# JubSteven/POEM-v2

Hardware: AMD Instinct MI355X
Metric: samples/sec (multi-view frames) POEM-medium 8-view (higher is better)
Workload: dtype f32

## Files before the change

### include/poem_hip.h

```cpp
#ifndef POEM_HIP_H
#define POEM_HIP_H

#include <stddef.h>
#include <stdint.h>

#ifdef __cplusplus
extern "C" {
#endif

#define POEM_OK 0
#define POEM_E_ARG (-1)
#define POEM_E_WORKSPACE (-2)
#define POEM_E_LAUNCH (-3)
#define POEM_E_UNSUPPORTED (-4)


#define POEM_ACT_NONE 0
#define POEM_ACT_RELU 1
#define POEM_ACT_GELU 2

typedef struct poem_config {
  int32_t embed;
  int32_t in_channels;
  int32_t nsample;
  int32_t nquery;
  int32_t heads;
  int32_t nblocks;
  int32_t knn;
  int32_t parametric;
  int32_t feat_h, feat_w;
  int32_t max_views;
  float radius;
  float ln_eps;
  int32_t pe_normalize;
  int32_t petr_embedding;
  int32_t depth_num;
  int32_t lid;
  int32_t reserved0;
  double depth_start, depth_end;
  double position_range[6];
} poem_config_t;

typedef struct poem_handle_s* poem_handle_t;

int poem_abi_version(void);
int poem_last_hip_error(void);
const char* poem_error_string(int code);

int poem_num_weight_tensors(const poem_config_t* cfg);
int64_t poem_weight_tensor_numel(const poem_config_t* cfg, int index);
size_t poem_packed_bytes(const poem_config_t* cfg);
int poem_create(const poem_config_t* cfg, const void* const* raw_host, int n, const float* bps, const float* anchor,
                const int32_t* anchor_idx, const float* template_xyz, void* packed, size_t packed_bytes,
                void* stream, poem_handle_t* out);
void poem_destroy(poem_handle_t h);

size_t poem_workspace_bytes(poem_handle_t h, int batch, int total_views);
int poem_graph_stats(poem_handle_t h, int64_t* out, int n);
int poem_head_forward(poem_handle_t h, const float* mlvl_feat, const float* cam_intr, const float* cam_extr,
                      const int32_t* view_offsets_host, int batch, const float* reference_joints, int img_w,
                      int img_h, float* out_xyz, float* pose_aa, float* betas, void* workspace,
                      size_t workspace_bytes, void* stream);
int poem_decoder_forward(poem_handle_t h, const float* query_xyz, const float* query_feat, const float* pt_xyz,
                         const float* pt_feats, int batch, float* out_xyz_norm, float* pose_aa, float* betas,
                         void* workspace, size_t workspace_bytes, void* stream);
int poem_set_overlap(poem_handle_t h, int enable);
int poem_set_chains(poem_handle_t h, int enable);
int poem_set_option(poem_handle_t h, const char* name, int value);
int poem_set_anchor_tables(poem_handle_t h, int enable);
#define POEM_PRECISION_FP32 0
#define POEM_PRECISION_SPLIT_F16X3 1
#define POEM_PRECISION_SPLIT_F16X3_ALL 2
int poem_set_precision(poem_handle_t h, int mode);
int poem_cross_attention_merged(const float* q, const float* k, const float* v, float* ctx, int batch, int nq, int nk, int embed,
                                int heads, void* scratch, size_t scratch_bytes, void* stream);
int poem_cross_attention_split_f16x3(const float* q, const float* k, const float* v, float* ctx, int batch, int nq, int nk,
                                     int embed, int heads, void* scratch, size_t scratch_bytes, void* stream);
int poem_pack_split_gemm(const float* w, int out_features, int in_features, void* image, float* scales, void* stream);
int poem_gemm_split(const float* x, int ldx, const void* image, const float* scales, const float* bias, const float* residual,
                    int ldr, float* y, int ldy, int m, int n, int k, int act, void* stream);
int poem_finalize_parametric(poem_handle_t h, const float* mano_verts, const float* mano_joints,
                             const float* reference_joints, int batch, float* out_xyz, void* stream);
int poem_profile_enable(poem_handle_t h, int max_launches);
int poem_profile_read(poem_handle_t h, int* launches, float* total_ms, int reset);
int poem_profile_read_anchored(poem_handle_t h, int* launches, float* total_ms);
#define POEM_PROF_VECATTN 0
#define POEM_PROF_VECATTN_ANCHORED 1
#define POEM_PROF_SAMPLING 2
int poem_profile_read_stage(poem_handle_t h, int stage, int* launches, float* total_ms);
int64_t poem_tap(poem_handle_t h, const char* name, void* dst, int64_t dst_elems, void* stream);
int poem_enable_taps(poem_handle_t h, int enable);

size_t poem_packed_linear_bytes(int out_features, int in_features);
int poem_pack_linear(const float* w, int out_features, int in_features, void* packed, void* stream);
int poem_gemm(const float* x, int ldx, const void* w_packed, const float* bias, const float* residual, int ldr,
              float* y, int ldy, int M, int N, int K, int act, void* stream);
#define POEM_LAYOUT_RM 0
#define POEM_LAYOUT_PA 1
int poem_gemm_ex(const float* x, int ldx, const void* w_packed, const float* bias, const float* residual, int ldr,
                 float* y, int ldy, int M, int N, int K, int act, int in_layout, int out_layout, void* stream);
int poem_pack_rows(const float* x, int rows, int cols, void* packed, void* stream);
int poem_unpack_rows(const void* packed, int rows, int cols, float* x, void* stream);
int poem_layernorm(const float* x, const float* gamma, const float* beta, float* y, int rows, int cols, float eps,
                   void* stream);
int poem_pe_table(const void* adapt_w_packed, const float* adapt_b, int embed, int h, int w, int max_views,
                  float* scratch_sine, float* table, void* stream);
int poem_pe_table_ex(const void* adapt_w_packed, const float* adapt_b, int embed, int h, int w, int max_views, int normalize,
                     float* scratch_sine, float* table, void* stream);
int poem_frustum_features(const poem_config_t* cfg, const float* cam_intr, const float* cam_extr, int views, int img0, int img1,
                          float* out, void* stream);
int poem_input_proj(const float* feat, const void* w_packed, const float* bias, const float* table,
                    const int32_t* pe_index, float* x, int views, int in_channels, int embed, int hw, void* stream);
int poem_project_sample(const float* x, const float* bps, const float* centre, const int32_t* view_sample,
                        const float* cam_intr, const float* cam_extr, float* uv_scratch, float* g, int views,
                        int embed, int fh, int fw, int nsample, int img_w, int img_h, void* stream);
int poem_merge_reduce(const float* h2, const int32_t* view_offsets, float* m, int batch, int nsample, int half,
                      void* stream);
int poem_merge_finalize(const float* g, const float* y, const int32_t* view_offsets, float* out, int batch,
                        int nsample, int embed, void* stream);
size_t poem_cross_attention_scratch_bytes(int batch, int nq, int nk, int embed, int heads);
int poem_cross_attention(const float* q, const float* k, const float* v, float* ctx, int batch, int nq, int nk,
                         int embed, int heads, void* scratch, size_t scratch_bytes, void* stream);
int poem_triangulate_dlt(const float* uv, const float* cam_intr, const float* cam_mat, const int32_t* view_offsets,
                         int batch, int njoints, int invert, float* out_xyz, void* stream);
int poem_heatmap_uv(const float* heatmaps, float* uv, int views, int njoints, int hm_h, int hm_w, float img_w, float img_h,
                    void* stream);
int poem_heatmap_uv_conf(const float* heatmaps, float* uv, float* conf, int views, int njoints, int hm_h, int hm_w,
                         float img_w, float img_h, void* stream);
#define POEM_DLT_THRESHOLD 1
#define POEM_DLT_WEIGHTED 2
int poem_dlt_confidence(const float* uv, const float* conf, const float* cam_intr, const float* cam_mat,
                        const int32_t* view_offsets, float* out_xyz, int32_t* sel_count, int batch, int njoints, int invert,
                        int mode, double threshold, void* stream);
size_t poem_conv3x3_packed_bytes(int cout, int cin);
int poem_pack_conv3x3(const float* w_oihw, int cout, int cin, void* packed, void* stream);
int poem_conv3x3(const float* in_padded, const void* w_packed, const float* scale, const float* shift,
                 const float* residual, float* out, int views, int cin, int cout, int h, int w, int stride, int relu,
                 int64_t out_view_stride, int out_ch_stride, int out_row_stride, int out_offset, void* stream);
typedef struct poem_fuse_term {
  const float* data;
  int64_t view_stride;
  int32_t ch_stride, row_stride, offset, shift;
} poem_fuse_term_t;
int poem_conv3x3_ex(const float* in_padded, const void* w_packed, const float* scale, const float* shift, const float* residual,
                    int64_t res_view_stride, int res_ch_stride, int res_row_stride, int res_offset, int res_before_act, float* out,
                    int views, int cin, int cout, int h, int w, int stride, int relu, int64_t out_view_stride, int out_ch_stride,
                    int out_row_stride, int out_offset, void* stream);
size_t poem_conv1x1_packed_bytes(int cout, int cin);
int poem_pack_conv1x1(const float* w_oi, int cout, int cin, void* packed, void* stream);
int poem_conv1x1(const float* in, int64_t in_view_stride, int in_ch_stride, int in_row_stride, int in_offset, const void* w_packed,
                 const float* shift, const float* residual, int64_t res_view_stride, int res_ch_stride, int res_row_stride,
                 int res_offset, float* out, int64_t out_view_stride, int out_ch_stride, int out_row_stride, int out_offset,
                 int views, int cin, int cout, int h, int w, int relu, void* stream);
int poem_hrnet_fuse(const poem_fuse_term_t* terms, int nterms, float* out, int64_t out_view_stride, int out_ch_stride,
                    int out_row_stride, int out_offset, int views, int channels, int h, int w, void* stream);
int poem_upsample2_concat_pad(const float* a, int ca, const float* b, int cb, float* out, int views, int h, int w, int pad,
                              void* stream);
size_t poem_conv7x7_packed_bytes(int cout);
int poem_pack_conv7x7(const float* w_oihw, int cout, void* packed, void* stream);
int poem_conv7x7_s2(const float* in, const void* w_packed, const float* scale, const float* shift, float* out,
                    int64_t out_view_stride, int out_ch_stride, int out_row_stride, int out_offset, int views, int cout, int h, int w,
                    void* stream);
int poem_maxpool3x3_s2(const float* in, int64_t in_view_stride, int in_ch_stride, int in_row_stride, int in_offset, float* out,
                       int64_t out_view_stride, int out_ch_stride, int out_row_stride, int out_offset, int views, int channels, int h,
                       int w, void* stream);
int poem_conv1x1_s2(const float* in, int64_t in_view_stride, int in_ch_stride, int in_row_stride, int in_offset, const void* w_packed,
                    const float* shift, float* out, int64_t out_view_stride, int out_ch_stride, int out_row_stride, int out_offset,
                    int views, int cin, int cout, int h, int w, void* stream);
int poem_maxpool2_conv1x1(const float* x, const void* w_packed, const float* bias, float* out, int views, int cin, int cout, int h,
                          int w, int act, void* stream);
int poem_upsample2_concat_pad_staged(const float* a, int ca, const float* b, int cb, float* out, int views, int h, int w, void* stream);
int poem_conv3x3_down2(const float* in, const void* w_packed, const float* scale, const float* shift, const float* residual,
                       float* out, int views, int cin, int cout, int h, int w, int relu, int64_t out_view_stride,
                       int out_ch_stride, int out_row_stride, int out_offset, void* stream);
int poem_set_decode_option(const char* name, int value);
int poem_conv1x1_upsample2(const float* in, const void* w_packed, const float* bias, float* out, int views, int cin, int cout,
                           int h, int w, void* stream);
int poem_upcat_conv3x3(const float* a_half, int ca, const float* b_full, int cb, const void* w_packed, const float* scale,
                       const float* shift, float* out, int views, int cout, int h, int w, int relu, int64_t out_view_stride,
                       int out_ch_stride, int out_row_stride, int out_offset, void* stream);
int poem_pool_conv1x1_sigmoid(const float* x, const float* w, const float* bias, float* heatmaps, int views, int c, int j,
                              int h, int w_, void* stream);
int poem_upcat_conv3x3_pool_head(const float* a_half, int ca, const float* b_full, int cb, const void* w_packed, const float* scale,
// ... 69 lines not shown
```

### poem-v2_amd/csrc/decoder.cpp

```cpp
#include "engine.h"

int build_anchor_tables(poem_handle_t h, Plan& p, hipStream_t s, bool at_create) {
  const poem_config_t& c = h->cfg;
  const int C = c.embed, Q = c.nquery;
  const bool ov = !at_create && h->overlap && h->bps_stream && h->knn_stream;
  hipStream_t sk = ov ? h->knn_stream : s;
  if (ov) {
    HIPCHK(hipEventRecord(h->ev_fork0, s));
    HIPCHK(hipStreamWaitEvent(sk, h->ev_fork0, 0));
  }
  const int bb0 = h->block_base(0);
  HIPCHK(poem_launch_canon_xyz(h->tmpl, p.canon_xyz, Q * 3, c.radius, sk));
  for (int k = 0; k < 2; ++k) {
    const int vb = bb0 + (k == 0 ? B_VS : B_VC);
    HIPCHK(poem_launch_vector_attention_tables(p.canon_xyz, h->anchor, h->anchor_idx, h->R(vb + 4), h->R(vb + 5),
                                               h->P(vb + 6), h->R(vb + 7), h->fused[0].w[5 + k], p.tab_g[k], p.tab_p[k],
                                               Q, C, sk));
  }
  if (ov) HIPCHK(hipEventRecord(h->ev_tab, sk));
  h->tables_pending = ov;
  return POEM_OK;
}

namespace {

struct DecoderRun {
  poem_handle_t h;
  Plan& p;
  const poem_config_t& c;
  const float *pt_xyz, *pt_feats;
  float *pose_aa, *betas;
  const int B, C, S, Q, BS, BQ;
  const int SP, BSP;
  const float* pt_xyz_rows;
  const bool ov;
  hipStream_t s, sb, sk;
  const bool tables;
  const bool chain;
  const float* feats;
  const float* hidden;
  int ldh = 0, hidden_mod = 0, q_batch = 0;
  const float* q0 = nullptr;
  const int *idx_s = nullptr, *idx_c = nullptr;
  const float* anchor = nullptr;
  int shared = 0;
  bool knn_issued[9] = {};
  bool wmerge = false;
  int wmask = 0;
  bool side_rest_pending = false;
  bool bps_waited[9] = {}, knn_waited[9] = {};
  bool anchor_from_y3 = false;

  DecoderRun(poem_handle_t h_, Plan& p_, const float* feats_in, const float* pt_xyz_, const float* pt_feats_, int B_, float* pose,
             float* bet, hipStream_t s_, bool template_queries)
      : h(h_), p(p_), c(h_->cfg), pt_xyz(pt_xyz_), pt_feats(pt_feats_), pose_aa(pose), betas(bet), B(B_), C(c.embed), S(c.nsample),
        Q(c.nquery), BS(B_ * c.nsample), BQ(B_ * c.nquery), SP(padded_samples(c)), BSP(B_ * padded_samples(c)), pt_xyz_rows(pt_xyz_), ov(h_->overlap && h_->bps_stream && h_->knn_stream), s(s_),
        sb(ov ? h_->bps_stream : s_), sk(ov ? h_->knn_stream : s_),
        tables(template_queries && h_->anchor_tables && h_->precision == POEM_PRECISION_FP32),
        chain(h_->chains && h_->precision == POEM_PRECISION_FP32 && poem_chain_supported(c.embed) != 0), feats(feats_in),
        hidden(nullptr) {}

  int gemm(const float* X, int ldx, int wi, int bi, const float* res, int ldr, float* Y, int ldy, int M, int N, int K, int act) {
    HIPCHK(poem_launch_gemm(X, ldx, h->P(wi), bi >= 0 ? h->R(bi) : nullptr, res, ldr, Y, ldy, M, N, K, act, s));
    return POEM_OK;
  }
  bool prof_begin() {
    const bool on = h->prof_on && (size_t)(2 * h->prof_used + 1) < h->prof_ev.size();
    if (on && hipEventRecord(h->prof_ev[2 * h->prof_used], s) != hipSuccess) return false;
    return on;
  }
  int prof_end(bool on, int kind) {
    if (on) { HIPCHK(hipEventRecord(h->prof_ev[2 * h->prof_used + 1], s)); h->prof_kind[h->prof_used++] = (char)kind; }
    return POEM_OK;
  }
  ChainArgs chain_args(int kind) const {
    ChainArgs a{};
    a.kind = kind; a.M = BQ; a.tile_p = h->chain_tile; a.eps = c.ln_eps;
    a.native_delta = h->native16 ? (long long)(h->native16 - h->packed_base) : 0;
    return a;
  }

  int fork() {
    if (!ov) return POEM_OK;
    HIPCHK(hipEventRecord(h->ev_fork, s));
    HIPCHK(hipStreamWaitEvent(sb, h->ev_fork, 0));
    HIPCHK(hipStreamWaitEvent(sk, h->ev_fork, 0));
    return POEM_OK;
  }
  int join() {
    if (!ov) return POEM_OK;
    HIPCHK(hipEventRecord(h->ev_join_bps, sb));
    HIPCHK(hipEventRecord(h->ev_join_knn, sk));
    HIPCHK(hipStreamWaitEvent(s, h->ev_join_bps, 0));
    HIPCHK(hipStreamWaitEvent(s, h->ev_join_knn, 0));
    return POEM_OK;
  }

  int basis_point_side(int i) {
    const auto& f = h->fused[i];
    const size_t seg = (size_t)BSP * C;
    float* outs[6] = {p.y1[i], p.y1[i] + seg, p.y1[i] + 2 * seg, p.y1[i] + 3 * seg, p.y1[i] + 4 * seg, p.y1[i] + 5 * seg};
    const int modes[6] = {1, 2, 1, 2, 0, 0};
    h->kv_presplit[i] = poem_gemm_split_applies(f.w[0], BSP, C, C) != 0;
    const bool anchored = tables && i == 0;
    if (!anchored && h->f1_split && C % 128 == 0) {
      HIPCHK(poem_launch_gemm_segs(pt_feats, C, f.w[0], f.b[0], BSP, C, POEM_ACT_NONE, C, 4, outs, modes, sb));
      HIPCHK(poem_launch_gemm_segs(pt_feats, C, (const float*)f.w[0] + (size_t)4 * C * C, f.b[0] + 4 * C, BSP, C, POEM_ACT_NONE, C, 2, outs + 4,
                                   modes + 4, sb));
    } else {
      HIPCHK(poem_launch_gemm_segs(pt_feats, C, f.w[0], f.b[0], BSP, C, POEM_ACT_NONE, C, anchored ? 4 : 6, outs, modes, sb));
    }
    if (ov) HIPCHK(hipEventRecord(h->ev_bps[i], sb));
    if (anchored && !side_rest_pending) return basis_point_anchor_rows(f);
    return POEM_OK;
  }
  int basis_point_anchor_rows(const poem_handle_s::Fused& f) {
    {
      HIPCHK(poem_launch_gather_anchor_rows(pt_feats, C, h->anchor_idx, SP, p.anch_x[1], B, C, p.ident, sb));
      HIPCHK(poem_launch_gemm(p.anch_x[1], C, (const float*)f.w[0] + (size_t)4 * C * C, f.b[0] + 4 * C, nullptr, 0,
                              p.anch_kv[1], 2 * C, B * 32, 2 * C, C, POEM_ACT_NONE, sb));
      if (ov) HIPCHK(hipEventRecord(h->ev_xyz[0], sb));
    }
    return POEM_OK;
  }

  bool merge_in_attention() const { return h->xattn_merge >= 0 ? h->xattn_merge != 0 : B <= 2; }

  int defer_at() const {
    return (ov && chain) ? h->bps_defer : 0;
  }
  int deferred_basis_point_side(int i, int at) {
    if (defer_at() != at || i + 1 >= c.nblocks) return POEM_OK;
    HIPCHK(hipEventRecord(h->ev_def[i], s));
    HIPCHK(hipStreamWaitEvent(sb, h->ev_def[i], 0));
    return basis_point_side(i + 1);
  }

  int neighbour_searches(int i, bool recorded = false) {
    if (knn_issued[i]) return POEM_OK;
    if (ov) {
      if (!recorded) HIPCHK(hipEventRecord(h->ev_xyz[i], s));
      HIPCHK(hipStreamWaitEvent(sk, h->ev_xyz[i], 0));
    }
    if (p.idx_ld == 32) {
      HIPCHK(poem_launch_knn(p.xyz[i], pt_xyz, p.idx_cross[i], B, Q, S, h->knn_fma, sk));
      HIPCHK(poem_launch_knn(p.xyz[i], p.xyz[i], p.idx_self[i], B, Q, Q, h->knn_fma, sk));
    } else {
      HIPCHK(poem_launch_knn_k(p.xyz[i], pt_xyz, p.idx_cross[i], B, Q, S, c.knn, p.idx_ld, h->knn_fma, sk));
      HIPCHK(poem_launch_knn_k(p.xyz[i], p.xyz[i], p.idx_self[i], B, Q, Q, h->knn_query ? h->knn_query : c.knn, p.idx_ld, h->knn_fma, sk));
    }
    if (ov) HIPCHK(hipEventRecord(h->ev_knn[i], sk));
    knn_issued[i] = true;
    return POEM_OK;
  }

  int query_projection(int i) {
    hidden = p.qeqp;
    ldh = 2 * C; hidden_mod = 0; q_batch = Q;
    q0 = p.qeqp + C;
    if (tables && i == 0) {
      const float* qe0 = p.qeqp0;
      if (h->tables_cached && h->c_qeqp0 && h->precision == POEM_PRECISION_FP32)
        qe0 = h->c_qeqp0;
      else
        HIPCHK(poem_launch_gemm_split(h->R(T_QEMB), C, h->fused[i].w[1], h->fused[i].b[1], nullptr, 0, p.qeqp0, 2 * C, Q, 2 * C, C,
                                      POEM_ACT_NONE, 2 * C, POEM_ACT_NONE, s));
      if (chain) {
        hidden = qe0; hidden_mod = Q; q0 = qe0 + C; q_batch = 0;
      } else {
        HIPCHK(poem_launch_broadcast(qe0, p.qeqp, (long)Q * 2 * C, B, s));
      }
    } else if (!(chain && i > 0)) {
      HIPCHK(poem_launch_gemm_split(feats, C, h->fused[i].w[1], h->fused[i].b[1], nullptr, 0, p.qeqp, 2 * C, BQ, 2 * C, C,
                                    POEM_ACT_NONE, 2 * C, POEM_ACT_NONE, s));
    }
    return POEM_OK;
  }

  int anchor_rows_f3(int i) {
    HIPCHK(poem_launch_gather_anchor_rows(hidden, C, h->anchor_idx, Q, p.anch_x[0], B, C, nullptr, s));
    HIPCHK(poem_launch_gemm(p.anch_x[0], C, (const float*)h->fused[i].w[2] + (size_t)C * C, h->fused[i].b[2] + C, nullptr, 0,
                            p.anch_kv[0], 2 * C, B * 32, 2 * C, C, POEM_ACT_NONE, s));
    return POEM_OK;
  }

  int cross_attentions(int i) {
    const int bb = h->block_base(i);
    if (chain) {
      const int a1 = bb + B_A1, a2 = bb + B_A2;
      if (ov && !bps_waited[i]) HIPCHK(hipStreamWaitEvent(s, h->ev_bps[i], 0));
      if (ov && (wmask & 4) && h->knn_early && i > 0 && knn_issued[i] && !knn_waited[i]) {
        HIPCHK(hipStreamWaitEvent(s, h->ev_knn[i], 0));
        knn_waited[i] = true;
      }
      const void *part_o = nullptr, *part_ml = nullptr;
      int pchunks = 0;
      float pkc2 = 0.f;
      poem_cross_attention_partials(B, Q, S, C, c.heads, p.attn_scratch, &part_o, &part_ml, &pchunks, &pkc2);
      const bool merged = merge_in_attention() && poem_cross_attention_merges(S, C, c.heads) != 0;
      const bool comb = !merged && h->chain_combine && poem_chain_combines(C, c.heads, pchunks) != 0;
      auto attention = [&](const float* q, int ldq, int qb, const float* kimg, const float* vimg) -> hipError_t {
        if (merged) return poem_launch_cross_attention_merged(q, ldq, qb, kimg, vimg, p.ctx, B, Q, S, C, c.heads, s);
        return poem_launch_cross_attention_imgq(q, ldq, qb, kimg, vimg, comb ? nullptr : p.ctx, B, Q, S, C, c.heads, p.attn_scratch, s);
      };
      auto from_partials = [&](ChainArgs& a) {
        if (!comb) return;
        a.x = nullptr; a.part_o = (const float4*)part_o; a.part_ml = (const float2*)part_ml;
        a.pc_heads = c.heads; a.pc_chunks = pchunks; a.pc_nq = Q; a.pc_kc2 = pkc2;
      };
      HIPCHK(attention(q0, 2 * C, q_batch, p.y1[i], p.y1[i] + (size_t)BSP * C));
      if (side_rest_pending) {
        side_rest_pending = false;
        if (tables && i == 0)
          if (const int rc = basis_point_anchor_rows(h->fused[0]); rc != POEM_OK) return rc;
        for (int k = 1; k < c.nblocks; ++k)
          if (const int rc = basis_point_side(k); rc != POEM_OK) return rc;
      }
      if (const int rc = deferred_basis_point_side(i, 1); rc != POEM_OK) return rc;
      ChainArgs ca = chain_args(0);
      ca.x = p.ctx; ca.ldx = C;
      from_partials(ca);
      ca.w1 = (const float4*)h->P(a1 + 6); ca.b1 = h->R(a1 + 7); ca.res = hidden; ca.ldres = ldh; ca.res_mod = hidden_mod;
      ca.ln_g = h->R(a1 + 8); ca.ln_b = h->R(a1 + 9); ca.y1 = p.h_attn; ca.ldy1 = C;
      ca.w2 = (const float4*)h->P(a2 + 0); ca.b2 = h->R(a2 + 1); ca.n2 = 1; ca.y2 = p.qp; ca.ldy2 = C;
      HIPCHK(poem_launch_chain(&ca, C, s));
      HIPCHK(attention(p.qp, C, Q, p.y1[i] + (size_t)2 * BSP * C, p.y1[i] + (size_t)3 * BSP * C));
      if (const int rc = deferred_basis_point_side(i, 2); rc != POEM_OK) return rc;
      ChainArgs cb = chain_args(0);
      cb.x = p.ctx; cb.ldx = C;
      from_partials(cb);
      cb.w1 = (const float4*)h->P(a2 + 6); cb.b1 = h->R(a2 + 7); cb.res = p.h_attn; cb.ldres = C; cb.res_mod = 0;
      cb.ln_g = h->R(a2 + 8); cb.ln_b = h->R(a2 + 9); cb.y1 = p.h_cross[i]; cb.ldy1 = C;
      anchor_from_y3 = tables && i == 0 && (h->small_batch & 2) && (long)BQ <= 16L * poem_device_cu_count();
      cb.w2 = (const float4*)h->fused[i].w[2]; cb.b2 = h->fused[i].b[2]; cb.n2 = (tables && i == 0 && !anchor_from_y3) ? 1 : 3; cb.y2 = p.y3; cb.ldy2 = 3 * C;
      HIPCHK(poem_launch_chain(&cb, C, s));
// ... 16 lines not shown
      }
      if (ov && a == 0) HIPCHK(hipStreamWaitEvent(s, h->ev_bps[i], 0));
      if (h->precision == POEM_PRECISION_SPLIT_F16X3_ALL) poem_cross_attention_split(h->kv_presplit[i] ? 2 : 1);
      if (h->precision == POEM_PRECISION_FP32 && merge_in_attention() && poem_cross_attention_merges(S, C, c.heads))
        HIPCHK(poem_launch_cross_attention_merged(qptr, ldq, Q, p.y1[i] + (size_t)(2 * a) * BSP * C, p.y1[i] + (size_t)(2 * a + 1) * BSP * C,
                                                  p.ctx, B, Q, S, C, c.heads, s));
      else
        HIPCHK(poem_launch_cross_attention_img(qptr, ldq, p.y1[i] + (size_t)(2 * a) * BSP * C, p.y1[i] + (size_t)(2 * a + 1) * BSP * C,
                                               p.ctx, B, Q, S, C, c.heads, p.attn_scratch, s));
      const int rc = gemm(p.ctx, C, ab + 6, ab + 7, hidden, ldh, p.att, C, BQ, C, C, POEM_ACT_NONE);
      if (rc != POEM_OK) return rc;
      HIPCHK(poem_launch_layernorm(p.att, h->R(ab + 8), h->R(ab + 9), hout, BQ, C, c.ln_eps, s));
      hidden = hout;
      ldh = C;
    }
    if (tables && i == 0) {
      HIPCHK(poem_launch_gemm(hidden, C, h->fused[i].w[2], h->fused[i].b[2], nullptr, 0, p.y3, 3 * C, BQ, C, C, POEM_ACT_NONE, s));
      return anchor_rows_f3(i);
    }
    HIPCHK(poem_launch_gemm_split(hidden, C, h->fused[i].w[2], h->fused[i].b[2], nullptr, 0, p.y3, 3 * C, BQ, 3 * C, C, POEM_ACT_NONE,
                                  3 * C, POEM_ACT_NONE, s));
    return POEM_OK;
  }

  int vector_self(int i) {
    const int vsb = h->block_base(i) + B_VS;
    const float* xyz = p.xyz[i];
    if (ov && i > 0 && !knn_waited[i]) HIPCHK(hipStreamWaitEvent(s, h->ev_knn[i], 0));
    const bool prof = prof_begin();
    const int kq = shared ? 32 : (h->knn_query ? h->knn_query : c.knn);
    if (h->precision != POEM_PRECISION_FP32) {
      if (kq != 32) return POEM_E_UNSUPPORTED;
      const auto& sw = h->split[2 * i];
      HIPCHK(poem_launch_vector_attention_split(xyz, xyz, anchor, idx_s, shared, p.y3, p.y3 + C, p.y3 + 2 * C, Q, h->R(vsb + 4),
                                                h->R(vsb + 5), sw.w[0], h->R(vsb + 7), sw.w[1], sw.w[2], sw.scales, p.rs, B, Q, C,
                                                3 * C, 3 * C, 3 * C, s));
    } else if (tables && i == 0) {
      if (ov && h->tables_pending) HIPCHK(hipStreamWaitEvent(s, h->ev_tab, 0));
      if (anchor_from_y3)
        HIPCHK(poem_launch_vector_attention_anchored(h->anchor_idx, p.y3, p.y3 + C, p.y3 + 2 * C, Q, h->P(vsb + 10), p.tab_g[0], p.tab_p[0],
                                                     p.rs, B, Q, C, 3 * C, 3 * C, 3 * C, s));
      else {
      if (ov) HIPCHK(hipStreamWaitEvent(s, h->ev_xyz[0], 0));
      HIPCHK(poem_launch_vector_attention_anchored(p.ident, p.y3, p.anch_kv[0], p.anch_kv[0] + C, 32, h->P(vsb + 10), p.tab_g[0],
                                                   p.tab_p[0], p.rs, B, Q, C, 3 * C, 2 * C, 2 * C, s));
      }
    } else if (!shared && p.idx_ld != 32) {
      HIPCHK(poem_launch_vector_attention_k(xyz, xyz, idx_s, kq, p.idx_ld, p.y3, p.y3 + C, p.y3 + 2 * C, Q, h->R(vsb + 4), h->R(vsb + 5),
                                            h->P(vsb + 6), h->R(vsb + 7), h->fused[i].w[5], h->R(vsb + 9), h->P(vsb + 10), h->R(vsb + 11),
                                            p.rs, B, Q, C, 3 * C, 3 * C, 3 * C, 1, s));
    } else {
      poem_vecattn_one_query_blocks(h->va_p1);
      poem_vecattn_valid_neighbours(kq);
      const hipError_t ve = poem_launch_vector_attention(xyz, xyz, anchor, idx_s, shared, p.y3, p.y3 + C, p.y3 + 2 * C, Q, h->R(vsb + 4),
                                                         h->R(vsb + 5), h->P(vsb + 6), h->R(vsb + 7), h->fused[i].w[5], h->R(vsb + 9),
                                                         h->P(vsb + 10), h->R(vsb + 11), p.rs, B, Q, C, 3 * C, 3 * C, 3 * C, 1, s);
      poem_vecattn_valid_neighbours(32);
      poem_vecattn_one_query_blocks(0);
      HIPCHK(ve);
    }
    if (const int rc = prof_end(prof, tables && i == 0 ? 1 : 0); rc != POEM_OK) return rc;
    if (chain) {
      ChainArgs cc = chain_args(1);
      cc.x = p.rs; cc.ldx = C;
      cc.w1 = (const float4*)h->P(vsb + 2); cc.b1 = h->R(vsb + 3); cc.res = hidden; cc.ldres = C; cc.res_mod = 0;
      cc.y1 = p.f_self[i]; cc.ldy1 = C;
      cc.w2 = (const float4*)h->fused[i].w[4]; cc.b2 = h->fused[i].b[4]; cc.n2 = 1; cc.y2 = p.qc; cc.ldy2 = C;
      HIPCHK(poem_launch_chain(&cc, C, s));
      return POEM_OK;
    }
    if (const int rc = gemm(p.rs, C, vsb + 2, vsb + 3, hidden, C, p.f_self[i], C, BQ, C, C, POEM_ACT_NONE); rc != POEM_OK) return rc;
    HIPCHK(poem_launch_gemm(p.f_self[i], C, h->fused[i].w[4], h->fused[i].b[4], nullptr, 0, p.qc, C, BQ, C, C, POEM_ACT_NONE, s));
    return POEM_OK;
  }

  int vector_cross(int i) {
    const int vcb = h->block_base(i) + B_VC;
    const float* xyz = p.xyz[i];
    if (ov && (wmask & 2) && i == 0 && defer_at() == 0)
      for (int k = 1; k < c.nblocks; ++k) {
        HIPCHK(hipStreamWaitEvent(s, h->ev_bps[k], 0));
        bps_waited[k] = true;
      }
    const bool prof = prof_begin();
    const int kc = shared ? 32 : c.knn;
    if (h->precision != POEM_PRECISION_FP32) {
      if (kc != 32) return POEM_E_UNSUPPORTED;
      const auto& sw = h->split[2 * i + 1];
      HIPCHK(poem_launch_vector_attention_split(xyz, pt_xyz_rows, anchor, idx_c, shared, p.qc, p.y1[i] + 4 * (size_t)BSP * C,
                                                p.y1[i] + 5 * (size_t)BSP * C, SP, h->R(vcb + 4), h->R(vcb + 5), sw.w[0],
                                                h->R(vcb + 7), sw.w[1], sw.w[2], sw.scales, p.rc, B, Q, C, C, C, C, s));
    } else if (tables && i == 0) {
      if (ov) HIPCHK(hipStreamWaitEvent(s, h->ev_xyz[0], 0));
      HIPCHK(poem_launch_vector_attention_anchored(p.ident, p.qc, p.anch_kv[1], p.anch_kv[1] + C, 32, h->P(vcb + 10), p.tab_g[1],
                                                   p.tab_p[1], p.rc, B, Q, C, C, 2 * C, 2 * C, s));
    } else if (!shared && p.idx_ld != 32) {
      HIPCHK(poem_launch_vector_attention_k(xyz, pt_xyz_rows, idx_c, kc, p.idx_ld, p.qc, p.y1[i] + 4 * (size_t)BSP * C, p.y1[i] + 5 * (size_t)BSP * C,
                                            SP, h->R(vcb + 4), h->R(vcb + 5), h->P(vcb + 6), h->R(vcb + 7), h->fused[i].w[6], h->R(vcb + 9),
                                            h->P(vcb + 10), h->R(vcb + 11), p.rc, B, Q, C, C, C, C, 1, s));
    } else {
      poem_vecattn_one_query_blocks(h->va_p1);
      poem_vecattn_valid_neighbours(kc);
      const hipError_t ve = poem_launch_vector_attention(xyz, pt_xyz_rows, anchor, idx_c, shared, p.qc, p.y1[i] + 4 * (size_t)BSP * C,
                                                         p.y1[i] + 5 * (size_t)BSP * C, SP, h->R(vcb + 4), h->R(vcb + 5), h->P(vcb + 6),
                                                         h->R(vcb + 7), h->fused[i].w[6], h->R(vcb + 9), h->P(vcb + 10), h->R(vcb + 11), p.rc, B,
                                                         Q, C, C, C, C, 1, s);
      poem_vecattn_valid_neighbours(32);
      poem_vecattn_one_query_blocks(0);
      HIPCHK(ve);
    }
    return prof_end(prof, tables && i == 0 ? 1 : 0);
  }

  int parametric_tail(int i) {
    const int bb = h->block_base(i);
    HIPCHK(poem_launch_q3_flatten(feats, h->R(bb + B_FLAT_W), h->R(bb + B_FLAT_B), p.q3t, B, Q, C, s));
    HIPCHK(poem_launch_narrow_linear(p.q3t, C, h->R(bb + B_MANO_W), h->R(bb + B_MANO_B), nullptr, p.par, B, C, 106, s));
    HIPCHK(poem_launch_rot6d_to_aa(p.par, pose_aa, betas, B, s));
    if (h->mano_table) HIPCHK(poem_launch_mano_lbs(pose_aa, betas, h->mano_table, p.mano_verts, p.mano_joints, B, h->mano_center, s));
    return POEM_OK;
  }

  int tail(int i, bool* done) {
    const int bb = h->block_base(i), vcb = bb + B_VC;
    const float* xyz = p.xyz[i];
    const bool last = i == c.nblocks - 1;
    const bool feats_dead = last && !c.parametric && !h->taps;
    *done = feats_dead;
    if (chain) {
      ChainArgs cd = chain_args(2);
      cd.x = p.rc; cd.ldx = C;
      cd.w1 = (const float4*)h->P(vcb + 2); cd.b1 = h->R(vcb + 3); cd.res = p.f_self[i]; cd.ldres = C; cd.res_mod = 0;
      cd.y1 = p.f_cross[i]; cd.ldy1 = C;
      cd.wf4 = (const float4*)h->fused[i].w[3]; cd.bf4 = h->fused[i].b[3];
      cd.wreg2 = h->R(bb + B_REG2_W); cd.breg2 = h->R(bb + B_REG2_B); cd.xyz_in = xyz; cd.xyz_out = p.xyz[i + 1];
      HIPCHK(poem_launch_chain(&cd, C, s));
      if (feats_dead) return POEM_OK;
      const bool early = ov && h->knn_early && !last;
      const bool d2_first = early && h->d2_first != 0;
      if (early && d2_first) HIPCHK(hipEventRecord(h->ev_xyz[i + 1], s));
      if (early && !d2_first)
        if (const int rc = neighbour_searches(i + 1); rc != POEM_OK) return rc;
      ChainArgs ce = chain_args(3);
      ce.x = p.f_cross[i]; ce.ldx = C;
      ce.wf4 = (const float4*)h->fused[i].w[3]; ce.bf4 = h->fused[i].b[3];
      ce.wout = (const float4*)h->P(bb + B_OUT_W); ce.bout = h->R(bb + B_OUT_B);
      ce.ln2_g = h->R(bb + B_LN_W); ce.ln2_b = h->R(bb + B_LN_B); ce.y3 = p.feats[i]; ce.ldy3 = C;
      if (!last) {
        ce.w2 = (const float4*)h->fused[i + 1].w[1]; ce.b2 = h->fused[i + 1].b[1]; ce.n2 = 2; ce.y2 = p.qeqp; ce.ldy2 = 2 * C;
      }
      HIPCHK(poem_launch_chain(&ce, C, s));
      if (early && d2_first)
        if (const int rc = neighbour_searches(i + 1, true); rc != POEM_OK) return rc;
      feats = p.feats[i];
      return c.parametric && last ? parametric_tail(i) : POEM_OK;
    }
    if (const int rc = gemm(p.rc, C, vcb + 2, vcb + 3, p.f_self[i], C, p.f_cross[i], C, BQ, C, C, POEM_ACT_NONE); rc != POEM_OK) return rc;
    if (feats_dead) {
      HIPCHK(poem_launch_gemm(p.f_cross[i], C, h->fused[i].w[3], h->fused[i].b[3], nullptr, 0, p.y4, 5 * C, BQ, C, C, POEM_ACT_RELU, s));
      HIPCHK(poem_launch_narrow_linear(p.y4, 5 * C, h->R(bb + B_REG2_W), h->R(bb + B_REG2_B), xyz, p.xyz[i + 1], BQ, C, 3, s));
      return POEM_OK;
    }
    HIPCHK(poem_launch_gemm_split(p.f_cross[i], C, h->fused[i].w[3], h->fused[i].b[3], nullptr, 0, p.y4, 5 * C, BQ, 5 * C, C,
                                  POEM_ACT_RELU, C, POEM_ACT_GELU, s));
    HIPCHK(poem_launch_narrow_linear(p.y4, 5 * C, h->R(bb + B_REG2_W), h->R(bb + B_REG2_B), xyz, p.xyz[i + 1], BQ, C, 3, s));
    if (const int rc = gemm(p.y4 + C, 5 * C, bb + B_OUT_W, bb + B_OUT_B, p.f_cross[i], C, p.ffo, C, BQ, C, 4 * C, POEM_ACT_NONE); rc != POEM_OK)
// ... 49 lines not shown
```

### poem-v2_amd/csrc/engine.h

```cpp
#pragma once
#include "../../include/poem_hip.h"
#include "launchers.h"

#include <hip/hip_runtime.h>

#include <algorithm>
#include <cstdio>
#include <cstdlib>
#include <cstring>
#include <map>
#include <string>
#include <vector>

extern thread_local int g_last_hip_error;

#define HIPCHK(expr)                                 \
  do {                                               \
    (void)hipGetLastError();                         \
    hipError_t e_ = (expr);                          \
    if (e_ != hipSuccess) {                          \
      g_last_hip_error = (int)e_;                    \
      return POEM_E_LAUNCH;                          \
    }                                                \
  } while (0)
// ... 15 lines not shown
enum {
  T_INPROJ_W = 0, T_INPROJ_B, T_ADAPT_W, T_ADAPT_B, T_M00_W, T_M00_B, T_M02_W, T_M02_B, T_M10_W, T_M10_B, T_M12_W,
  T_M12_B, T_QEMB, T_HEAD_COUNT
};
enum {
  B_EMB_W = 0, B_EMB_B,
  B_A1 = 2,
  B_A2 = 12,
  B_VS = 22,
  B_VC = 37,
  B_REG0_W = 52, B_REG0_B, B_REG2_W, B_REG2_B, B_INT_W, B_INT_B, B_OUT_W, B_OUT_B, B_LN_W, B_LN_B,
  B_COUNT = 62,
  B_FLAT_W = 62, B_FLAT_B, B_MANO_W, B_MANO_B, B_COUNT_PARAM = 66
};

static inline int petr_slot(const poem_config_t& c) { return T_HEAD_COUNT + c.nblocks * (c.parametric ? B_COUNT_PARAM : B_COUNT); }
static inline size_t pe_views(int max_views) { return (size_t)max_views * (max_views + 1) / 2; }
std::vector<TensorSpec> tensor_table(const poem_config_t& c);
int check_config(const poem_config_t* c);

struct poem_handle_s {
  poem_config_t cfg;
  std::vector<TensorSpec> specs;
  std::vector<const float*> raw;
  std::vector<const void*> packed;
  const float* bps = nullptr;
  const float* anchor = nullptr;
  const int32_t* anchor_idx = nullptr;
  const float* tmpl = nullptr;
  float* pe_table = nullptr;
  struct Fused { const void* w[7]; const float* b[7]; };
  std::vector<Fused> fused;
  struct SplitW { const void* w[3]; const float* scales; };
  std::vector<SplitW> split;
  void* split_mem = nullptr;
  int precision = 0;
  bool kv_presplit[8] = {};
  const char* packed_base = nullptr;
  size_t packed_size = 0;
  char* native16 = nullptr;
  char* gemm_split = nullptr;
  float* gemm_scales = nullptr;
  bool taps = false;
  struct Tap { const void* p; int64_t elems; };
  std::map<std::string, Tap> tapmap;
  std::vector<hipEvent_t> prof_ev;
  int prof_used = 0;
  std::vector<char> prof_kind;
  bool prof_on = false;
  hipStream_t bps_stream = nullptr, knn_stream = nullptr;
  hipEvent_t ev_fork = nullptr, ev_join_bps = nullptr, ev_join_knn = nullptr, ev_tab = nullptr, ev_fork0 = nullptr;
  bool anchor_tables = true;
  bool chains = true;
  bool fused_sampling = true;
  bool tables_first = true;
  bool chain_combine = true;
  int xattn_merge = -1;
  bool knn_early = true;
  bool graphs = true;
  bool graph_broken = false;
  hipStream_t cap_stream = nullptr;
  int stream_device = 0;
  struct GraphEntry { std::vector<int64_t> key; hipGraphExec_t exec; uint64_t stamp; uint64_t shape; hipStream_t last_stream = nullptr; bool launched = false; };
  std::vector<GraphEntry> graph_cache;
  std::vector<std::vector<int64_t>> graph_seen;
  bool graph_eager = false;
  uint64_t graph_clock = 0;
  static constexpr size_t GRAPH_CAP = 12;
  int64_t graph_captures = 0, graph_instantiations = 0, graph_replays = 0, plain_forwards = 0, layout_uploads = 0;
  int small_batch = 3;
  int group_xcd = 1;
  int group_min_views = 0;
  const float* mano_table = nullptr;
  int mano_center = 9;
  int knn_query = 0;
  int knn_fma = 0;
  int chain_tile = 0;
  bool tables_cached = true;
  bool tables_pending = false;
  float* tab_mem = nullptr;
  float *c_canon_xyz = nullptr, *c_tab_g[2] = {}, *c_tab_p[2] = {};
  float* c_qeqp0 = nullptr;
  hipEvent_t ev_bps[8] = {}, ev_xyz[8] = {}, ev_knn[8] = {}, ev_def[8] = {};
  int bps_defer = 0;
  bool f1_split = true;
  int va_p1 = -1;
  int d2_first = 1;
  int wait_merge = -1;
  bool overlap = true;
  static constexpr int IDX_CAP = 32768;
  int32_t* idx_dev = nullptr;
  std::vector<int32_t> idx_host;
  int block_base(int b) const { return T_HEAD_COUNT + b * (cfg.parametric ? B_COUNT_PARAM : B_COUNT); }
  const float* R(int idx) const { return raw[idx]; }
  const void* P(int idx) const { return packed[idx]; }
};

struct Arena {
  char* base;
  size_t off = 0;
  explicit Arena(void* b) : base((char*)b) {}
  template <typename T>
  T* take(size_t n) {
    off = align_up(off, 256);
    T* p = base ? (T*)(base + off) : nullptr;
    off += n * sizeof(T);
    return p;
  }
};

struct Plan {
  int32_t *offs, *view_sample, *pe_index, *idx_self[8], *idx_cross[8];
  float *x, *uv, *g, *h1, *h2, *mm, *mh, *y, *bps_feat, *centre, *pt_xyz, *xyz[9];
  float *xt, *ptab, *q1;
  float *petr_f, *petr_h, *petr_tab;
  float *feats0, *qp, *ctx, *att, *h_attn, *y3, *rs, *qc, *rc, *y4, *ffo;
  float *y1[8];
  float *qeqp;
  float *h_cross[8], *f_self[8], *f_cross[8], *feats[8];
  float *q3t, *par, *attn_scratch, *g_pose, *g_betas;
  float *mano_verts, *mano_joints;
  float *canon_xyz, *tab_g[2], *tab_p[2];
  float *anch_x[2], *anch_kv[2], *qeqp0;
  int32_t* ident;
  float *feat_pad, *xyz_pad;
  int idx_ld;
  size_t bytes;
};

inline int padded_samples(const poem_config_t& c) { return (c.nsample + 31) / 32 * 32; }

inline int neighbour_ld(const poem_config_t& c, int knn_query) { return (c.knn > 32 || knn_query > 32) ? 64 : 32; }

Plan make_plan(const poem_config_t& c, int B, int BN, void* base, int idx_ld);
void register_taps(poem_handle_t h, const Plan& p, int B, int BN, bool sampling);

int poem_process_switches();
void poem_park_graph_exec(hipGraphExec_t e, uint64_t shape, int device, hipStream_t last_stream, bool launched);
hipGraphExec_t poem_reuse_graph_exec(hipGraph_t graph, uint64_t shape, int device);

int build_anchor_tables(poem_handle_t h, Plan& p, hipStream_t s, bool at_create = false);
int run_decoder(poem_handle_t h, Plan& p, const float* feats_in, const float* pt_xyz, const float* pt_feats, int B, float* pose_aa,
                float* betas, hipStream_t s, bool template_queries = false);
```

### poem-v2_amd/csrc/forward.cpp

```cpp
#include "engine.h"

namespace {

struct SplitContext {
  bool set = false;
  explicit SplitContext(poem_handle_t h) {
    if (h->precision != POEM_PRECISION_SPLIT_F16X3_ALL) return;
    set = true;
    poem_gemm_split_context(h->packed_base, h->packed_size, h->gemm_split, h->gemm_scales);
    poem_cross_attention_split(1);
    const int dh = h->cfg.embed / h->cfg.heads;
    poem_gemm_split_images(dh == 32 || dh == 64);
  }
  ~SplitContext() {
    if (!set) return;
    poem_gemm_split_context(nullptr, 0, nullptr, nullptr);
    poem_cross_attention_split(0);
    poem_gemm_split_images(0);
  }
};

struct HeadRun {
  poem_handle_t h;
  const poem_config_t& c;
// ... 76 lines not shown
      const int ps = petr_slot(c), K0 = 3 * c.depth_num;
      HIPCHK(poem_launch_frustum_features(cam_intr, cam_extr, p.petr_f, BN, c.feat_h, c.feat_w, c.depth_num, c.lid != 0, c.depth_start,
                                          c.depth_end, c.position_range, img_w, img_h, s));
      HIPCHK(poem_launch_conv1x1_ex(p.petr_f, h->P(ps), h->R(ps + 1), nullptr, nullptr, p.petr_h, nullptr, BN, K0, 2 * C, HW, 1, s));
      HIPCHK(poem_launch_conv1x1_ex(p.petr_h, h->P(ps + 2), h->R(ps + 3), h->pe_table, p.pe_index, p.petr_tab, nullptr, BN, 2 * C, C, HW, 0, s));
      table = p.petr_tab;
      table_index = nullptr;
    }
    HIPCHK(poem_launch_conv1x1(mlvl_feat, h->P(T_INPROJ_W), h->R(T_INPROJ_B), table, table_index,
                               (fused_fe && !h->taps) ? nullptr : p.x, fused_fe ? p.xt : nullptr, BN, c.in_channels, C, HW, s));
    if (fused_fe && (h->small_batch & 1)) {
      HIPCHK(poem_launch_input_tables(h->bps, reference_joints, h->tmpl, p.view_sample, cam_intr, cam_extr, p.ptab, p.ptab + (size_t)plan_views * S * 4, p.centre, p.pt_xyz,
                                      p.xyz[0], BN, B, S, Q, c.feat_h, c.feat_w, img_w, img_h, c.radius, s));
      return POEM_OK;
    }
    HIPCHK(poem_launch_prep_xyz(reference_joints, h->bps, h->tmpl, p.centre, p.pt_xyz, p.xyz[0], B, S, Q, c.radius, s));
    if (fused_fe) {
      float* inv = p.uv + (size_t)BN * S * 2;
      HIPCHK(poem_launch_invert_extr(cam_extr, inv, BN, s));
      HIPCHK(poem_launch_project_table(h->bps, p.centre, p.view_sample, cam_intr, inv, p.ptab, p.ptab + (size_t)plan_views * S * 4, nullptr, BN, C, c.feat_h, c.feat_w, S,
                                       img_w, img_h, s));
    } else {
      HIPCHK(poem_launch_project_uv(h->bps, p.centre, p.view_sample, cam_intr, cam_extr, p.uv + (size_t)BN * S * 2, p.uv, BN, c.feat_h,
                                    c.feat_w, S, img_w, img_h, s));
    }
    return POEM_OK;
  }

  int sampling(hipStream_t st) {
    if (fused_fe) {
      SampleMergeArgs sm{};
      sm.xt = p.xt; sm.tab = (const float4*)p.ptab; sm.tabo = (const uint2*)(p.ptab + (size_t)plan_views * S * 4);
      sm.view_sample = p.view_sample; sm.offs = p.offs;
      sm.w0 = (const float4*)h->P(T_M00_W); sm.b0 = h->R(T_M00_B); sm.w1 = (const float4*)h->P(T_M02_W); sm.b1 = h->R(T_M02_B);
      sm.h2 = p.h2; sm.q1 = p.q1; sm.S = S; sm.hw = HW; sm.h2_tiled = 1;
      sm.views = plan_views; sm.B = B; sm.views_dev = p.offs + B;
      const bool group_ok = h->group_min_views >= 0 && (S / C) % 8 == 0;
      sm.group_min_views = group_ok ? (h->group_min_views > 0 ? h->group_min_views : 2 * poem_device_cu_count() / ((C / (C == 512 ? 32 : 64)) * (S / C / 8)))
                                    : 0x7fffffff;
      if (h->tables_first && h->tables_pending) HIPCHK(hipStreamWaitEvent(st, h->ev_tab, 0));
      MergeTailArgs mt{};
      mt.h2 = p.h2; mt.q1 = p.q1; mt.offs = p.offs;
      mt.w0 = (const float4*)h->P(T_M10_W); mt.b0 = h->R(T_M10_B); mt.w1 = (const float4*)h->P(T_M12_W); mt.b1 = h->R(T_M12_B);
      mt.out = p.bps_feat; mt.B = B; mt.S = S; mt.h2_tiled = 1;
      mt.group_min_views = sm.group_min_views; mt.views_dev = sm.views_dev; mt.views = sm.views;
      sm.xcd_order = h->group_xcd;
      if (group_ok && plan_views >= sm.group_min_views) {
        SampleGroupArgs sg{};
        sg.sm = sm; sg.w2 = mt.w0; sg.b2 = mt.b0; sg.w3 = mt.w1; sg.b3 = mt.b1; sg.out = p.bps_feat;
        HIPCHK(poem_launch_sample_group(&sg, C, st));
      }
      HIPCHK(poem_launch_sample_merge(&sm, C, st));
      HIPCHK(poem_launch_merge_tail(&mt, C, st));
      return POEM_OK;
    }
    auto gemm = [&](const float* X, int ldx, int wi, int bi, float* Y, int ldy, int M, int N, int K, int act) -> int {
      HIPCHK(poem_launch_gemm(X, ldx, h->P(wi), h->R(bi), nullptr, 0, Y, ldy, M, N, K, act, st));
      return POEM_OK;
    };
    HIPCHK(poem_launch_grid_sample(p.x, p.uv, p.g, BN, C, c.feat_h, c.feat_w, S, st));
    int rc = gemm(p.g, C, T_M00_W, T_M00_B, p.h1, C, BN * S, C, C, POEM_ACT_RELU);
    if (rc == POEM_OK) rc = gemm(p.h1, C, T_M02_W, T_M02_B, p.h2, C / 2, BN * S, C / 2, C, POEM_ACT_NONE);
    if (rc != POEM_OK) return rc;
    HIPCHK(poem_launch_merge_reduce(p.h2, p.offs, p.mm, B, S, C / 2, st));
    rc = gemm(p.mm, C / 2, T_M10_W, T_M10_B, p.mh, C / 2, BS, C / 2, C / 2, POEM_ACT_RELU);
    if (rc == POEM_OK) rc = gemm(p.mh, C / 2, T_M12_W, T_M12_B, p.y, C, BS, C, C / 2, POEM_ACT_NONE);
    if (rc != POEM_OK) return rc;
    HIPCHK(poem_launch_merge_finalize(p.g, p.y, p.offs, p.bps_feat, B, S, C, st));
    return POEM_OK;
  }

  int body(hipStream_t st, float* pose_dst, float* betas_dst) {
    if (const int rc = sampling(st); rc != POEM_OK) return rc;
    if (prof_fe) HIPCHK(hipEventRecord(h->prof_ev[2 * prof_slot + 1], st));
    if (!(h->anchor_tables && h->precision == POEM_PRECISION_FP32 && (h->small_batch & 1)))
      HIPCHK(poem_launch_broadcast(h->R(T_QEMB), p.feats0, (long)Q * C, B, st));
    return run_decoder(h, p, p.feats0, p.pt_xyz, p.bps_feat, B, pose_dst, betas_dst, st, true);
  }

  int replay(void* workspace, float* pose_aa, float* betas) {
    if (!h->graphs || h->graph_broken || h->prof_on || h->tables_pending || !h->cap_stream) return 0;
    const std::vector<int64_t> key = {B, plan_views, fused_fe ? -1 : BN, (int64_t)(uintptr_t)workspace, h->precision, h->anchor_tables, h->chains,
                                      h->fused_sampling, h->tables_first, h->chain_combine, h->knn_early, h->overlap, h->chain_tile,
                                      h->tables_cached, h->knn_fma, h->knn_query, h->taps, c.parametric, h->xattn_merge, h->small_batch, h->bps_defer, poem_process_switches(), h->f1_split, h->va_p1, h->group_min_views, h->group_xcd, h->d2_first, h->wait_merge,
                                      (int64_t)(uintptr_t)h->mano_table, h->mano_center};
    poem_handle_s::GraphEntry* hit = nullptr;
    for (auto& g : h->graph_cache)
      if (g.key == key) { hit = &g; break; }
    if (!hit) {
      if (!h->graph_eager) {
        bool seen = false;
        for (auto& k : h->graph_seen) seen = seen || k == key;
        if (!seen) {
          if (h->graph_seen.size() >= 64) h->graph_seen.erase(h->graph_seen.begin());
          h->graph_seen.push_back(key);
          return 0;
        }
      }
      hipGraph_t graph = nullptr;
      hipGraphExec_t exec = nullptr;
      POEM_TRACE("capture begin h=%p B=%d cached=%zu", (void*)h, B, h->graph_cache.size());
      bool ok = hipStreamBeginCapture(h->cap_stream, hipStreamCaptureModeRelaxed) == hipSuccess;
      if (ok) {
        const int rc = body(h->cap_stream, p.g_pose, p.g_betas);
        POEM_TRACE("capture body rc=%d", rc);
        const hipError_t e = hipStreamEndCapture(h->cap_stream, &graph);
        POEM_TRACE("capture end e=%d graph=%p", (int)e, (void*)graph);
        ok = rc == POEM_OK && e == hipSuccess && graph != nullptr;
      }
      ++h->graph_captures;
      if (ok) {
        exec = poem_reuse_graph_exec(graph, graph_shape_of(c, key), h->stream_device);
        if (!exec) {
          ok = hipGraphInstantiate(&exec, graph, nullptr, nullptr, 0) == hipSuccess;
          ++h->graph_instantiations;
        }
      }
      POEM_TRACE("instantiate ok=%d exec=%p", (int)ok, (void*)exec);
      if (graph) (void)hipGraphDestroy(graph);
      POEM_TRACE("graph destroyed");
      if (!ok) {
        (void)hipGetLastError();
        h->graph_broken = true;
        return 0;
      }
      if (h->graph_cache.size() >= poem_handle_s::GRAPH_CAP) {
        size_t lru = 0;
        for (size_t i = 1; i < h->graph_cache.size(); ++i)
          if (h->graph_cache[i].stamp < h->graph_cache[lru].stamp) lru = i;
        poem_park_graph_exec(h->graph_cache[lru].exec, h->graph_cache[lru].shape, h->stream_device, h->graph_cache[lru].last_stream,
                             h->graph_cache[lru].launched);
        h->graph_cache.erase(h->graph_cache.begin() + lru);
      }
      h->graph_cache.push_back({key, exec, 0, graph_shape_of(c, key), nullptr, false});
      hit = &h->graph_cache.back();
    }
    hit->stamp = ++h->graph_clock;
    POEM_TRACE("graph launch exec=%p", (void*)hit->exec);
    HIPCHK(hipGraphLaunch(hit->exec, s));
    hit->last_stream = s; hit->launched = true;
    ++h->graph_replays;
    POEM_TRACE("graph launched");
    if (c.parametric) {
      HIPCHK(hipMemcpyAsync(pose_aa, p.g_pose, (size_t)B * 48 * sizeof(float), hipMemcpyDeviceToDevice, s));
      HIPCHK(hipMemcpyAsync(betas, p.g_betas, (size_t)B * 10 * sizeof(float), hipMemcpyDeviceToDevice, s));
    }
    return 1;
  }

  static uint64_t graph_shape_of(const poem_config_t& c, const std::vector<int64_t>& key) {
    uint64_t v = 1469598103934665603ull;
    auto mix = [&](uint64_t x) { v = (v ^ x) * 1099511628211ull; };
    mix((uint64_t)c.embed); mix((uint64_t)c.nblocks); mix((uint64_t)c.heads); mix((uint64_t)c.nsample); mix((uint64_t)c.nquery);
    mix((uint64_t)c.in_channels); mix((uint64_t)c.feat_h * 65536u + (uint64_t)c.feat_w); mix((uint64_t)c.max_views);
    for (size_t i = 0; i < key.size(); ++i)
      if (i != 3) mix((uint64_t)key[i]);
    return v ? v : 1;
  }
};

}

extern "C" {

int poem_head_forward(poem_handle_t h, const float* mlvl_feat, const float* cam_intr, const float* cam_extr,
                      const int32_t* view_offsets_host, int batch, const float* reference_joints, int img_w, int img_h,
                      float* out_xyz, float* pose_aa, float* betas, void* workspace, size_t workspace_bytes,
// ... 71 lines not shown
```

### poem-v2_amd/csrc/gemm.hip

```cpp
#include "common.h"
#include <algorithm>
#include <cstdlib>

typedef _Float16 h8 __attribute__((ext_vector_type(8)));
#ifndef POEM_GS_WAVES
#define POEM_GS_WAVES 12
#endif
#define POEM_GEMM_SX 16.0f
__global__ __launch_bounds__(256) void pack_split_tiles_kernel(const float* __restrict__ W, int N, int K,
                                                              h8* __restrict__ img, float* __restrict__ scales,
                                                              int scale_stride) {
  __shared__ float red[256];
  const int nt = blockIdx.x, KC = K / 16;
  float m = 0.f;
  for (int i = threadIdx.x; i < 32 * K; i += 256) {
    const int row = 32 * nt + i / K;
    if (row < N) m = fmaxf(m, fabsf(W[(size_t)row * K + i % K]));
  }
  red[threadIdx.x] = m;
  __syncthreads();
  for (int o = 128; o > 0; o >>= 1) {
    if ((int)threadIdx.x < o) red[threadIdx.x] = fmaxf(red[threadIdx.x], red[threadIdx.x + o]);
    __syncthreads();
  }
// ... 362 lines not shown
    const int col = col0 + n * 32 + r, ycol = ycol0 + n * 32 + r;
    const float bv = bias ? bias[col] : 0.f;
#pragma unroll
    for (int i = 0; i < MT; ++i) {
      const int row0 = (mt0 + i) * 32 + 4 * h;
      if (row0 >= M) continue;
      float v[16];
#pragma unroll
      for (int e = 0; e < 16; ++e) {
        v[e] = acc[i][n][e] + bv;
        if (pact == 1) v[e] = relu_nan(v[e]);
        if (pact == 2) v[e] = gelu_erf(v[e]);
      }
      if (row0 + 28 < M) {
        float* yl = Y + (size_t)row0 * ldy + ycol;
        if (R) {
          const float* rl = R + (size_t)row0 * ldr + col;
          float rr[16];
#pragma unroll
          for (int e = 0; e < 16; ++e) rr[e] = rl[(size_t)((e & 3) + 8 * (e >> 2)) * ldr];
#pragma unroll
          for (int e = 0; e < 16; ++e) yl[(size_t)((e & 3) + 8 * (e >> 2)) * ldy] = v[e] + rr[e];
        } else {
#pragma unroll
          for (int e = 0; e < 16; ++e) yl[(size_t)((e & 3) + 8 * (e >> 2)) * ldy] = v[e];
        }
      } else {
#pragma unroll
        for (int e = 0; e < 16; ++e) {
          const int row = row0 + (e & 3) + 8 * (e >> 2);
          if (row < M) Y[(size_t)row * ldy + ycol] = v[e] + (R ? R[(size_t)row * ldr + col] : 0.f);
        }
      }
    }
  }
}

template <int MT, int NT, int SKC>
__global__ __launch_bounds__(512, 2) void gemm_kslab_kernel(const float* __restrict__ X, int ldx, const float4* __restrict__ Wp,
                                                            const float* __restrict__ bias, const float* __restrict__ R, int ldr,
                                                            float* __restrict__ Y, int ldy, int M, int N, int K, int act,
                                                            int act_split, int act2, PanelSegs segs) {
  const int ncb = N / (32 * NT);
  const int nb = (int)gridDim.x;
  const int lb = (nb & 7) == 0 ? (int)(blockIdx.x & 7) * (nb >> 3) + (int)(blockIdx.x >> 3) : (int)blockIdx.x;
  const int cb = lb % ncb, rb = lb / ncb;
  const int col0 = cb * NT * 32;
  const int pact = (col0 >= act_split) ? act2 : act;
  if (segs.seg_cols == 0) {
    kslab_body<MT, NT, SKC, 0>(X, ldx, Wp, bias, R, ldr, Y, ldy, M, K, pact, cb, rb, col0);
    return;
  }
  const int sidx = col0 / segs.seg_cols, ycol0 = col0 - sidx * segs.seg_cols, mode = segs.mode[sidx];
  float* ys = segs.ptr[sidx];
  if (mode == 1) kslab_body<MT, NT, SKC, 1>(X, ldx, Wp, bias, nullptr, 0, ys, segs.seg_cols, M, K, pact, cb, rb, ycol0);
  else if (mode == 2) kslab_body<MT, NT, SKC, 2>(X, ldx, Wp, bias, nullptr, 0, ys, segs.seg_cols, M, K, pact, cb, rb, ycol0);
  else kslab_body<MT, NT, SKC, 0>(X, ldx, Wp, bias, nullptr, 0, ys, segs.seg_cols, M, K, pact, cb, rb, ycol0);
}

static bool kslab_applies(const float* X, int ldx, int M, int N, int K, int act_split) {
  return K >= 512 && K % 128 == 0 && N % 64 == 0 && (act_split >= N || act_split % 64 == 0) && !((uintptr_t)X & 15) && ldx % 4 == 0 &&
         (unsigned long long)M * ldx * 4ull < (1ull << 32) && M >= 512;
}

static hipError_t launch_gemm_kslab(const float* X, int ldx, const void* Wp, const float* bias, const float* R, int ldr, float* Y,
                                    int ldy, int M, int N, int K, int act, int act_split, int act2, const PanelSegs& segs, hipStream_t s) {
  constexpr int NT = 2, SKC = 16;
  const int mtiles = (M + 31) / 32, ncb = N / (32 * NT);
  const bool mt2 = (long)((mtiles + 15) / 16) * ncb >= 2 * poem_device_cus();
  const size_t lds = (size_t)2 * NT * SKC * 1024;
  if (mt2) {
    auto kern = gemm_kslab_kernel<2, NT, SKC>;
    hipLaunchKernelGGL(kern, dim3((unsigned)(((mtiles + 15) / 16) * ncb)), dim3(512), lds, s, X, ldx, (const float4*)Wp, bias, R, ldr, Y, ldy,
                       M, N, K, act, act_split, act2, segs);
  } else {
    auto kern = gemm_kslab_kernel<1, NT, SKC>;
    hipLaunchKernelGGL(kern, dim3((unsigned)(((mtiles + 7) / 8) * ncb)), dim3(512), lds, s, X, ldx, (const float4*)Wp, bias, R, ldr, Y, ldy,
                       M, N, K, act, act_split, act2, segs);
  }
  return hipGetLastError();
}


template <int NT, int MT, bool GELU, int OMODE, bool SPLIT = false>
__device__ __forceinline__ void panel_rows(const float* __restrict__ X, int ldx, const float4* __restrict__ wl,
                                           const float* __restrict__ bias, const float* __restrict__ R, int ldr,
                                           float* __restrict__ Y, int ldy, int M, int K, int pact, int col0, int ycol0,
                                           int bip, int blocks_in_panel, const float* __restrict__ tile_scales = nullptr,
                                           int scale_stride = 0, int split_images = 0, int part = 0, int nparts = 1) {
  constexpr int NWV = (SPLIT && !GELU) ? POEM_GS_WAVES : 8;
  const int KC = K >> 3;
  const int tid = threadIdx.x, lane = tid & 63, wv = tid >> 6, r = lane & 31, h = lane >> 5;
  const int mtiles = (M + 31) / 32;
  const int rgroups = (mtiles + MT - 1) / MT;
  const __amdgpu_buffer_rsrc_t xrs = frag_rsrc(X, 0xffffffffu);
  float bv[NT];
#pragma unroll
  for (int n = 0; n < NT; ++n) bv[n] = (bias && OMODE != 1) ? bias[col0 + n * 32 + r] : 0.f;
  const size_t lane_yo = (size_t)(4 * h) * ldy + r, lane_ro = (size_t)(4 * h) * ldr + r;
  const int rg_lo = (int)((long)rgroups * part / nparts), rg_hi = (int)((long)rgroups * (part + 1) / nparts);
#ifndef POEM_PANEL_LAB
#define POEM_PANEL_LAB 0
#endif
#ifdef POEM_PANEL_SKEW
  if (wv >= NWV / 2) { const long long t0_ = wall_clock64(); while (wall_clock64() - t0_ < POEM_PANEL_SKEW) __builtin_amdgcn_s_sleep(32); }
#endif
  for (int rg = rg_lo + bip * NWV + wv; rg < rg_hi; rg += blocks_in_panel * NWV) {
#if POEM_PANEL_LAB & 4
    __builtin_amdgcn_s_setprio(0);
#endif
    const int mt0 = rg * MT;
    unsigned xo[MT];
#pragma unroll
    for (int i = 0; i < MT; ++i) xo[i] = (unsigned)min((mt0 + i) * 32 + r, M - 1) * (unsigned)(ldx * 4) + 16u * h;
    f32x16 acc[MT][NT];
#pragma unroll
    for (int i = 0; i < MT; ++i)
#pragma unroll
      for (int n = 0; n < NT; ++n) acc[i][n] = zero16();
    if constexpr (SPLIT) {
      const int KC16 = K >> 4;
      const h8* wl8 = reinterpret_cast<const h8*>(wl);
      unsigned xo8[MT];
#pragma unroll
      for (int i = 0; i < MT; ++i) xo8[i] = (unsigned)min((mt0 + i) * 32 + r, M - 1) * (unsigned)(ldx * 4) + 32u * h;
      float4 ra[2][MT][2];
#define POEM_LOADA8(S, KCI) { const int kq_ = min((KCI), KC16 - 1); _Pragma("unroll") for (int i = 0; i < MT; ++i) { \
        ra[S][i][0] = frag_load(xrs, (int)xo8[i], kq_ * 64); ra[S][i][1] = frag_load(xrs, (int)xo8[i], kq_ * 64 + 16); } }
      POEM_LOADA8(0, 0)
      h8 bh_next = wl8[lane], bl_next = wl8[64 + lane];
      for (int kc = 0; kc < KC16; ++kc) {
        const int cur = kc & 1;
        if (cur == 0) { POEM_LOADA8(1, kc + 1) } else { POEM_LOADA8(0, kc + 1) }
        h8 ah[MT], al[MT];
#pragma unroll
        for (int i = 0; i < MT; ++i) {
          const float4 lo4 = cur == 0 ? ra[0][i][0] : ra[1][i][0], hi4 = cur == 0 ? ra[0][i][1] : ra[1][i][1];
          const float xv[8] = {lo4.x, lo4.y, lo4.z, lo4.w, hi4.x, hi4.y, hi4.z, hi4.w};
#pragma unroll
          for (int t = 0; t < 8; ++t) {
#if defined(POEM_GS_LAB) && POEM_GS_LAB == 1
            ah[i][t] = __builtin_bit_cast(_Float16, (unsigned short)__float_as_uint(xv[t]));
            al[i][t] = ah[i][t];
#else
            const float v = __builtin_amdgcn_fmed3f(xv[t] * POEM_GEMM_SX, -60000.f, 60000.f);
            ah[i][t] = (_Float16)v;
            al[i][t] = (_Float16)(v - (float)ah[i][t]);
#endif
          }
        }
        __builtin_amdgcn_sched_barrier(0);
#pragma unroll
        for (int n = 0; n < NT; ++n) {
          const int nn = n + 1 < NT ? n + 1 : 0, kn = n + 1 < NT ? kc : min(kc + 1, KC16 - 1);
          const h8 bh = bh_next, bl = bl_next;
          bh_next = wl8[((size_t)(nn * KC16 + kn) * 2 + 0) * 64 + lane];
          bl_next = wl8[((size_t)(nn * KC16 + kn) * 2 + 1) * 64 + lane];
          __builtin_amdgcn_sched_barrier(0);
#define POEM_MMA8(XA, WB)                                                                                      \
          _Pragma("unroll") for (int i = 0; i < MT; ++i)                                                       \
            acc[i][n] = OMODE == 1 ? __builtin_amdgcn_mfma_f32_32x32x16_f16(WB, XA[i], acc[i][n], 0, 0, 0)     \
                                   : __builtin_amdgcn_mfma_f32_32x32x16_f16(XA[i], WB, acc[i][n], 0, 0, 0);
#if defined(POEM_GS_LAB) && POEM_GS_LAB == 2
#pragma unroll
          for (int i = 0; i < MT; ++i) acc[i][n][0] += (float)al[i][0] * (float)bh[0] + (float)ah[i][1] * (float)bl[1];
#else
          POEM_MMA8(al, bh) POEM_MMA8(ah, bh) POEM_MMA8(ah, bl)
#endif
#undef POEM_MMA8
          __builtin_amdgcn_sched_barrier(0);
        }
      }
#undef POEM_LOADA8
#pragma unroll
      for (int n = 0; n < NT; ++n) {
        const float inv = 1.0f / (tile_scales[(size_t)(col0 / 32 + n) * scale_stride] * POEM_GEMM_SX);
#pragma unroll
        for (int i = 0; i < MT; ++i)
#pragma unroll
          for (int e = 0; e < 16; ++e) acc[i][n][e] *= inv;
      }
    } else {
    float4 a0[MT], a1[MT], b0[NT], b1[NT];
#define POEM_LOADA(A, KCI) { const int kq_ = min((KCI), KC - 1); _Pragma("unroll") for (int i = 0; i < MT; ++i) A[i] = frag_load(xrs, (int)xo[i], kq_ * 32); }
#define POEM_LOADB(B, KCI) { const int kq_ = min((KCI), KC - 1); _Pragma("unroll") for (int n = 0; n < NT; ++n) B[n] = wl[(n * KC + kq_) * 64 + lane]; }
#define POEM_MMA(A, B)                                                          \
  _Pragma("unroll") for (int t = 0; t < 4; ++t) {                               \
    _Pragma("unroll") for (int n = 0; n < NT; ++n) {                            \
      const float bw = (&B[n].x)[t];                                            \
      _Pragma("unroll") for (int i = 0; i < MT; ++i)                            \
        acc[i][n] = OMODE == 1 ? mfma32(bw, (&A[i].x)[t], acc[i][n]) : mfma32((&A[i].x)[t], bw, acc[i][n]); \
    }                                                                           \
  }
    POEM_LOADA(a0, 0) POEM_LOADB(b0, 0)
    int kc = 0;
    for (; kc + 1 < KC; kc += 2) {
      POEM_LOADA(a1, kc + 1) POEM_LOADB(b1, kc + 1)
      __builtin_amdgcn_sched_barrier(0);
      POEM_MMA(a0, b0)
      __builtin_amdgcn_sched_barrier(0);
      POEM_LOADA(a0, kc + 2) POEM_LOADB(b0, kc + 2)
      __builtin_amdgcn_sched_barrier(0);
      POEM_MMA(a1, b1)
      __builtin_amdgcn_sched_barrier(0);
    }
    if (kc < KC) { POEM_MMA(a0, b0) }
#if POEM_PANEL_LAB & 4
    __builtin_amdgcn_s_setprio(3);
#endif
#undef POEM_LOADA
#undef POEM_LOADB
#undef POEM_MMA
    }
    if (OMODE == 1) {
#pragma unroll
      for (int i = 0; i < MT; ++i) {
        if ((mt0 + i) * 32 >= M) break;
        float4* yp = reinterpret_cast<float4*>(Y) + ((size_t)(mt0 + i) * (ldy >> 3) + (ycol0 >> 3)) * 64 + lane;
        float4 vprev = make_float4(0.f, 0.f, 0.f, 0.f);
        (void)vprev;
#pragma unroll
        for (int n = 0; n < NT; ++n)
#pragma unroll
          for (int g = 0; g < 4; ++g) {
            float4 v = make_float4(acc[i][n][4 * g], acc[i][n][4 * g + 1], acc[i][n][4 * g + 2], acc[i][n][4 * g + 3]);
            if (bias) {
              const float4 bb = *reinterpret_cast<const float4*>(reinterpret_cast<const float*>(wl + NT * KC * 64) + n * 32 + 8 * g + 4 * h);
              v.x += bb.x; v.y += bb.y; v.z += bb.z; v.w += bb.w;
            }
            if (pact == 1) { v.x = relu_nan(v.x); v.y = relu_nan(v.y); v.z = relu_nan(v.z); v.w = relu_nan(v.w); }
            if (GELU && pact == 2) { v.x = gelu_erf(v.x); v.y = gelu_erf(v.y); v.z = gelu_erf(v.z); v.w = gelu_erf(v.w); }
            if (SPLIT && split_images) {
              if (g & 1) {
                h8 hi, lo;
                split_pair(vprev, v, hi, lo);
                yp[(size_t)(n * 4 + g - 1) * 64] = __builtin_bit_cast(float4, hi);
                yp[(size_t)(n * 4 + g) * 64] = __builtin_bit_cast(float4, lo);
              }
              vprev = v;
            } else {
#if POEM_PANEL_LAB & 1
              asm volatile("" :: "v"(v.x), "v"(v.y), "v"(v.z), "v"(v.w));
#else
              yp[(size_t)(n * 4 + g) * 64] = v;
#endif
            }
          }
      }
      continue;
    }
#pragma unroll
    for (int i = 0; i < MT; ++i) {
      const int trow0 = (mt0 + i) * 32;
      if (trow0 >= M) break;
      float* yl = Y + (size_t)trow0 * ldy + (size_t)ycol0 + lane_yo;
      const float* rl = R ? R + (size_t)trow0 * ldr + (size_t)col0 + lane_ro : nullptr;
      const bool full = trow0 + 32 <= M;
#pragma unroll
      for (int n = 0; n < NT; ++n) {
        float v[16];
        if (GELU && pact == 2) {
#pragma unroll
          for (int e = 0; e < 16; ++e) v[e] = gelu_erf(acc[i][n][e] + bv[n]);
        } else if (pact == 1) {
#pragma unroll
          for (int e = 0; e < 16; e += 2) {
            const f32x2 t = f32x2{acc[i][n][e], acc[i][n][e + 1]} + f32x2{bv[n], bv[n]};
            v[e] = relu_nan(t[0]); v[e + 1] = relu_nan(t[1]);
          }
        } else {
#pragma unroll
          for (int e = 0; e < 16; e += 2) {
            const f32x2 t = f32x2{acc[i][n][e], acc[i][n][e + 1]} + f32x2{bv[n], bv[n]};
            v[e] = t[0]; v[e + 1] = t[1];
          }
        }
        if (OMODE == 2) {
          float4* yp = reinterpret_cast<float4*>(Y) + ((size_t)(mt0 + i) * (ldy >> 5) + (ycol0 >> 5) + n) * 256 + lane;
          if (SPLIT && split_images) {
#pragma unroll
            for (int c = 0; c < 2; ++c) {
              h8 hi, lo;
              split_pair(make_float4(v[8 * c], v[8 * c + 1], v[8 * c + 2], v[8 * c + 3]),
                         make_float4(v[8 * c + 4], v[8 * c + 5], v[8 * c + 6], v[8 * c + 7]), hi, lo);
              yp[(size_t)(2 * c) * 64] = __builtin_bit_cast(float4, hi);
              yp[(size_t)(2 * c + 1) * 64] = __builtin_bit_cast(float4, lo);
            }
          } else {
#pragma unroll
          for (int g = 0; g < 4; ++g) {
#if POEM_PANEL_LAB & 1
            asm volatile("" :: "v"(v[4 * g]), "v"(v[4 * g + 1]), "v"(v[4 * g + 2]), "v"(v[4 * g + 3]));
#else
            yp[(size_t)g * 64] = make_float4(v[4 * g], v[4 * g + 1], v[4 * g + 2], v[4 * g + 3]);
#endif
          }
          }
        } else if (full) {
          if (rl) {
            float rr[16];
// ... 100 lines not shown
  int NT = 0;
  const long wave_slots = 8L * poem_num_cus(), row_tiles = (M + 31) / 32;
  for (int c : {4, 2, 1})
    if (N % (32 * c) == 0 && (size_t)c * K * 128 <= 128 * 1024 && (act_split >= N || act_split % (32 * c) == 0) &&
        (!seg || segs.seg_cols % (32 * c) == 0)) {
      NT = c;
      if (row_tiles * (N / (32 * c)) >= wave_slots || !g_panel_narrow || K > 256 || in_split_mode) break;
    }
  const bool split_mode = in_split_mode;
  if (NT <= 1 && !split_mode && g_kslab && kslab_applies(X, ldx, M, N, K, act_split) && (!seg || (segs.seg_cols % 64 == 0 && M % 32 == 0)))
    return launch_gemm_kslab(X, ldx, Wp, bias, R, ldr, Y, ldy, M, N, K, act, act_split, act2, segs, s);
  if (!seg && NT == 1 && N >= 64 && K >= 512 && !(act_split < N && act2 != act)) NT = 0;
  if (NT == 0 || K % 8 || ((uintptr_t)X & 15) || ldx % 4 || (unsigned long long)M * ldx * 4ull >= (1ull << 32)) {
    if (seg || (act_split < N && act2 != act) || g_explicit_split.img) return hipErrorInvalidValue;
    return poem_launch_gemm2(X, ldx, Wp, bias, R, ldr, Y, ldy, M, N, K, act, 0, 0, s);
  }
  const int mtiles = (M + 31) / 32, panels = N / (32 * NT);
  const int wpp = std::max(1, std::max(poem_num_cus(), panels) / panels) * 8;
  auto cost = [&](int mt) { return (long)(((mtiles + mt - 1) / mt + wpp - 1) / wpp) * mt; };
  const bool mt2_default = 5 * cost(2) <= 6 * cost(1);
  const bool mt2 = mt2_default;
  const bool gelu = act == 2 || (act_split < N && act2 == 2);
  if (seg && gelu) return hipErrorInvalidValue;
  const float* tsc = nullptr;
  int tstride = 0;
  const void* Wsplit = nullptr;
  if (g_explicit_split.img) {
    Wsplit = g_explicit_split.img; tsc = g_explicit_split.scales; tstride = 1;
  } else if (g_split_ctx.packed && (const char*)Wp >= g_split_ctx.packed && (const char*)Wp < g_split_ctx.packed + g_split_ctx.bytes) {
    const size_t off = (const char*)Wp - g_split_ctx.packed;
    Wsplit = g_split_ctx.split + off; tsc = g_split_ctx.scales + off / 256; tstride = K / 2;
  }
  if (g_explicit_split.img && K % 16) return hipErrorInvalidValue;
  if (Wsplit && K % 16 == 0 && (unsigned long long)M * ldx * 4ull + 64ull < (1ull << 32)) {
#ifdef POEM_LAB
    static const int force_mt = getenv("POEM_GS_MT") ? atoi(getenv("POEM_GS_MT")) : 1;
#else
    constexpr int force_mt = 1;
#endif
    const bool mt2 = force_mt == 2;
    (void)mt2_default;
#define POEM_PANEL_S(NTV)                                                                                                \
    if (gelu)                                                                                                            \
      return mt2 ? launch_panel_t<NTV, 2, true, true>(X, ldx, Wsplit, bias, R, ldr, Y, ldy, M, N, K, act, act_split, act2, segs, s, tsc, tstride)   \
                 : launch_panel_t<NTV, 1, true, true>(X, ldx, Wsplit, bias, R, ldr, Y, ldy, M, N, K, act, act_split, act2, segs, s, tsc, tstride);  \
    return mt2 ? launch_panel_t<NTV, 2, false, true>(X, ldx, Wsplit, bias, R, ldr, Y, ldy, M, N, K, act, act_split, act2, segs, s, tsc, tstride)    \
               : launch_panel_t<NTV, 1, false, true>(X, ldx, Wsplit, bias, R, ldr, Y, ldy, M, N, K, act, act_split, act2, segs, s, tsc, tstride)
    if (NT == 4) { POEM_PANEL_S(4); }
    if (NT == 2) { POEM_PANEL_S(2); }
    POEM_PANEL_S(1);
#undef POEM_PANEL_S
  }
#define POEM_PANEL(NTV)                                                                                                  \
  if (gelu)                                                                                                              \
    return mt2 ? launch_panel_t<NTV, 2, true>(X, ldx, Wp, bias, R, ldr, Y, ldy, M, N, K, act, act_split, act2, segs, s)   \
               : launch_panel_t<NTV, 1, true>(X, ldx, Wp, bias, R, ldr, Y, ldy, M, N, K, act, act_split, act2, segs, s);  \
  return mt2 ? launch_panel_t<NTV, 2, false>(X, ldx, Wp, bias, R, ldr, Y, ldy, M, N, K, act, act_split, act2, segs, s)    \
             : launch_panel_t<NTV, 1, false>(X, ldx, Wp, bias, R, ldr, Y, ldy, M, N, K, act, act_split, act2, segs, s)
  if (NT == 4) { POEM_PANEL(4); }
  if (NT == 2) { POEM_PANEL(2); }
  POEM_PANEL(1);
#undef POEM_PANEL
}

extern "C" hipError_t poem_launch_gemm_split(const float* X, int ldx, const void* Wp, const float* bias, const float* R,
                                             int ldr, float* Y, int ldy, int M, int N, int K, int act, int act_split,
                                             int act2, hipStream_t s) {
  PanelSegs none{};
  return launch_gemm_split_impl(X, ldx, Wp, bias, R, ldr, Y, ldy, M, N, K, act, act_split, act2, none, s);
}

extern "C" hipError_t poem_launch_gemm_segs(const float* X, int ldx, const void* Wp, const float* bias, int M, int K,
                                            int act, int seg_cols, int nsegs, float* const* outs, const int* modes,
                                            hipStream_t s) {
  if (nsegs < 1 || nsegs > 6 || seg_cols % 32 || M % 32) return hipErrorInvalidValue;
  PanelSegs segs{};
  segs.seg_cols = seg_cols;
  segs.split_images = g_split_images;
  for (int i = 0; i < nsegs; ++i) { segs.ptr[i] = outs[i]; segs.mode[i] = modes[i]; }
  const int N = seg_cols * nsegs;
  return launch_gemm_split_impl(X, ldx, Wp, bias, nullptr, 0, nullptr, 0, M, N, K, act, N, act, segs, s);
}

extern "C" hipError_t poem_launch_gemm(const float* X, int ldx, const void* Wp, const float* bias, const float* R,
                                       int ldr, float* Y, int ldy, int M, int N, int K, int act, hipStream_t s) {
  return poem_launch_gemm_split(X, ldx, Wp, bias, R, ldr, Y, ldy, M, N, K, act, N, act, s);
}

__global__ __launch_bounds__(256) void layernorm_kernel(const float* __restrict__ x, const float* __restrict__ g,
                                                        const float* __restrict__ b, float* __restrict__ y, int rows,
                                                        int cols, float eps) {
  const int lane = threadIdx.x & 63;
  const int row = blockIdx.x * 4 + (threadIdx.x >> 6);
  if (row >= rows) return;
  const float* xr = x + (size_t)row * cols;
  float s = 0.f;
  for (int c = lane; c < cols; c += 64) s += xr[c];
#pragma unroll
  for (int o = 32; o > 0; o >>= 1) s += __shfl_xor(s, o, 64);
  const float mean = s / (float)cols;
  float v = 0.f;
  for (int c = lane; c < cols; c += 64) { float d = xr[c] - mean; v += d * d; }
#pragma unroll
  for (int o = 32; o > 0; o >>= 1) v += __shfl_xor(v, o, 64);
  const float rstd = 1.0f / sqrtf(v / (float)cols + eps);
  float* yr = y + (size_t)row * cols;
  for (int c = lane; c < cols; c += 64) yr[c] = (xr[c] - mean) * rstd * g[c] + b[c];
}

extern "C" hipError_t poem_launch_layernorm(const float* x, const float* g, const float* b, float* y, int rows,
                                            int cols, float eps, hipStream_t s) {
  hipLaunchKernelGGL(layernorm_kernel, dim3((rows + 3) / 4), dim3(256), 0, s, x, g, b, y, rows, cols, eps);
  return hipGetLastError();
}

__global__ __launch_bounds__(256) void narrow_linear_kernel(const float* __restrict__ x, int ldx,
                                                            const float* __restrict__ w, const float* __restrict__ b,
                                                            const float* __restrict__ base, float* __restrict__ out,
                                                            int rows, int K, int N, int npb) {
  const int lane = threadIdx.x & 63;
  const int row = blockIdx.x * 4 + (threadIdx.x >> 6);
  if (row >= rows) return;
  const float* xr = x + (size_t)row * ldx;
  for (int n = blockIdx.y * npb, ne = min(N, n + npb); n < ne; ++n) {
    float s = 0.f;
    for (int c = lane; c < K; c += 64) s = fmaf(xr[c], w[(size_t)n * K + c], s);
#pragma unroll
    for (int o = 32; o > 0; o >>= 1) s += __shfl_xor(s, o, 64);
    if (lane == 0) out[(size_t)row * N + n] = (base ? base[(size_t)row * N + n] : 0.f) + (s + (b ? b[n] : 0.f));
  }
}

extern "C" hipError_t poem_launch_narrow_linear(const float* x, int ldx, const float* w, const float* b,
                                                const float* base, float* out, int rows, int K, int N,
                                                hipStream_t s) {
  const int npb = (long)((rows + 3) / 4) * N <= 65535 && (rows + 3) / 4 < 2048 ? 1 : N;
  hipLaunchKernelGGL(narrow_linear_kernel, dim3((rows + 3) / 4, (N + npb - 1) / npb), dim3(256), 0, s, x, ldx, w, b, base, out, rows, K, N, npb);
  return hipGetLastError();
}
```

### poem-v2_amd/csrc/handle.cpp

```cpp
#include "engine.h"

#include <atomic>
thread_local int g_last_hip_error = 0;

static std::atomic<int> g_proc_switches{15};
int poem_process_switches() { return g_proc_switches.load(); }

#include <mutex>
namespace {
struct CaptureKit {
  hipStream_t cap = nullptr, bps = nullptr, knn = nullptr;
  hipEvent_t ev[5 + 32] = {};
};
std::mutex g_pool_mutex;
std::map<int, std::vector<CaptureKit>> g_kit_pool;
struct ParkedExec { hipGraphExec_t exec; uint64_t shape; int device; hipEvent_t done; };
std::vector<ParkedExec> g_parked_execs;
std::map<int, std::vector<hipEvent_t>> g_idle_done_events;
int64_t g_exec_reuses = 0, g_exec_update_failures = 0, g_exec_busy_skips = 0;

hipEvent_t done_event_locked(hipStream_t last_stream, bool launched, int device, bool* ok) {
  *ok = true;
  if (!launched) return nullptr;
  int cur = -1;
  const bool switched = hipGetDevice(&cur) == hipSuccess && cur != device && hipSetDevice(device) == hipSuccess;
  hipEvent_t ev = nullptr;
  auto& idle = g_idle_done_events[device];
  if (!idle.empty()) { ev = idle.back(); idle.pop_back(); }
  else if (hipEventCreateWithFlags(&ev, hipEventDisableTiming) != hipSuccess) { (void)hipGetLastError(); ev = nullptr; }
  if (ev && hipEventRecord(ev, last_stream) != hipSuccess) {
    (void)hipGetLastError();
    idle.push_back(ev);
    ev = nullptr;
  }
  if (!ev) {
    *ok = hipDeviceSynchronize() == hipSuccess;
    (void)hipGetLastError();
  }
  if (switched) (void)hipSetDevice(cur);
  return ev;
}

hipEvent_t** kit_event_slots(poem_handle_t h, hipEvent_t** out) {
  int n = 0;
  out[n++] = &h->ev_fork; out[n++] = &h->ev_join_bps; out[n++] = &h->ev_join_knn; out[n++] = &h->ev_tab; out[n++] = &h->ev_fork0;
  for (int i = 0; i < 8; ++i) { out[n++] = &h->ev_bps[i]; out[n++] = &h->ev_xyz[i]; out[n++] = &h->ev_knn[i]; out[n++] = &h->ev_def[i]; }
  return out;
}

bool take_kit(poem_handle_t h) {
  int dev = 0;
  if (hipGetDevice(&dev) != hipSuccess) return false;
  h->stream_device = dev;
  hipEvent_t* slots[5 + 32];
  kit_event_slots(h, slots);
  {
    std::lock_guard<std::mutex> lock(g_pool_mutex);
    auto& pool = g_kit_pool[dev];
    if (!pool.empty()) {
      const CaptureKit k = pool.back();
      pool.pop_back();
      h->cap_stream = k.cap; h->bps_stream = k.bps; h->knn_stream = k.knn;
      for (int i = 0; i < 5 + 32; ++i) *slots[i] = k.ev[i];
      return true;
    }
  }
  bool ok = hipStreamCreateWithFlags(&h->bps_stream, hipStreamNonBlocking) == hipSuccess &&
            hipStreamCreateWithFlags(&h->knn_stream, hipStreamNonBlocking) == hipSuccess &&
            hipStreamCreateWithFlags(&h->cap_stream, hipStreamNonBlocking) == hipSuccess;
  for (int i = 0; i < 5 + 32; ++i) ok = ok && hipEventCreateWithFlags(slots[i], hipEventDisableTiming) == hipSuccess;
  return ok;
}

void return_kit(poem_handle_t h) {
  hipEvent_t* slots[5 + 32];
  kit_event_slots(h, slots);
  bool whole = h->cap_stream && h->bps_stream && h->knn_stream;
  for (int i = 0; i < 5 + 32; ++i) whole = whole && *slots[i] != nullptr;
  if (!whole) {
    if (h->cap_stream) (void)hipStreamDestroy(h->cap_stream);
    if (h->bps_stream) (void)hipStreamDestroy(h->bps_stream);
    if (h->knn_stream) (void)hipStreamDestroy(h->knn_stream);
    for (int i = 0; i < 5 + 32; ++i) if (*slots[i]) (void)hipEventDestroy(*slots[i]);
  } else {
    CaptureKit k;
    k.cap = h->cap_stream; k.bps = h->bps_stream; k.knn = h->knn_stream;
    for (int i = 0; i < 5 + 32; ++i) k.ev[i] = *slots[i];
    std::lock_guard<std::mutex> lock(g_pool_mutex);
    g_kit_pool[h->stream_device].push_back(k);
  }
  h->cap_stream = h->bps_stream = h->knn_stream = nullptr;
  for (int i = 0; i < 5 + 32; ++i) *slots[i] = nullptr;
}

void park_execs(poem_handle_t h) {
  std::lock_guard<std::mutex> lock(g_pool_mutex);
  for (auto& g : h->graph_cache) {
    bool ok = true;
    hipEvent_t ev = done_event_locked(g.last_stream, g.launched, h->stream_device, &ok);
    g_parked_execs.push_back({g.exec, ok ? g.shape : 0, h->stream_device, ev});
  }
  h->graph_cache.clear();
}
}

void poem_park_graph_exec(hipGraphExec_t e, uint64_t shape, int device, hipStream_t last_stream, bool launched) {
  std::lock_guard<std::mutex> lock(g_pool_mutex);
  bool ok = true;
  hipEvent_t ev = done_event_locked(last_stream, launched, device, &ok);
  g_parked_execs.push_back({e, ok ? shape : 0, device, ev});
}

hipGraphExec_t poem_reuse_graph_exec(hipGraph_t graph, uint64_t shape, int device) {
  ParkedExec cand{nullptr, 0, 0, nullptr};
  {
    std::lock_guard<std::mutex> lock(g_pool_mutex);
    for (size_t i = g_parked_execs.size(); i-- > 0;) {
      ParkedExec& pe = g_parked_execs[i];
      if (pe.shape != shape || pe.device != device) continue;
      if (pe.done) {
        if (hipEventQuery(pe.done) != hipSuccess) { (void)hipGetLastError(); ++g_exec_busy_skips; continue; }
        g_idle_done_events[pe.device].push_back(pe.done);
        pe.done = nullptr;
      }
      cand = pe;
      g_parked_execs.erase(g_parked_execs.begin() + i);
      break;
    }
  }
  if (!cand.exec) return nullptr;
  hipGraphNode_t err_node = nullptr;
  hipGraphExecUpdateResult res = hipGraphExecUpdateSuccess;
  const hipError_t e = hipGraphExecUpdate(cand.exec, graph, &err_node, &res);
  std::lock_guard<std::mutex> lock(g_pool_mutex);
  if (e == hipSuccess && res == hipGraphExecUpdateSuccess) {
    ++g_exec_reuses;
    return cand.exec;
  }
  (void)hipGetLastError();
  POEM_TRACE("exec update refused e=%d res=%d", (int)e, (int)res);
  ++g_exec_update_failures;
  g_parked_execs.insert(g_parked_execs.begin(), {cand.exec, 0, cand.device, nullptr});
  return nullptr;
}

std::vector<TensorSpec> tensor_table(const poem_config_t& c) {
  const int C = c.embed, Q = c.nquery;
  std::vector<TensorSpec> t;
  auto lin = [&](int o, int i, bool pack, bool bias = true) {
    t.push_back({o, i, pack});
    if (bias) t.push_back({o, 1, false});
  };
  lin(C, c.in_channels, true);
  lin(C, 3 * C / 2, true);
  lin(C, C, true);
  lin(C / 2, C, true);
  lin(C / 2, C / 2, true);
  lin(C, C / 2, true);
  t.push_back({Q, C, false});
  for (int b = 0; b < c.nblocks; ++b) {
    lin(C, C, true);
    for (int a = 0; a < 2; ++a) {
      lin(C, C, true); lin(C, C, true); lin(C, C, true); lin(C, C, true);
      t.push_back({C, 1, false}); t.push_back({C, 1, false});
    }
    for (int a = 0; a < 2; ++a) {
      lin(C, C, true); lin(C, C, true);
      lin(C, 3, false);
      lin(C, C, true); lin(C, C, true); lin(C, C, true);
      lin(C, C, true, false); lin(C, C, true, false); lin(C, C, true, false);
    }
    lin(C, C, true);
    lin(3, C, false);
    lin(4 * C, C, true);
    lin(C, 4 * C, true);
// ... 255 lines not shown
    const size_t tf = poem_vector_attention_table_floats(cfg->nquery, C);
    const size_t cx = align_up((size_t)cfg->nquery * 3, 64);
    const size_t qf = align_up((size_t)cfg->nquery * 2 * C, 64);
    if (hipMalloc((void**)&h->tab_mem, (cx + 4 * tf + qf) * sizeof(float)) != hipSuccess) {
      g_last_hip_error = (int)hipGetLastError(); poem_destroy(h); return POEM_E_LAUNCH;
    }
    h->c_canon_xyz = h->tab_mem;
    Plan tp{};
    tp.canon_xyz = h->c_canon_xyz;
    for (int k = 0; k < 2; ++k) {
      tp.tab_g[k] = h->c_tab_g[k] = h->tab_mem + cx + (size_t)(2 * k) * tf;
      tp.tab_p[k] = h->c_tab_p[k] = h->tab_mem + cx + (size_t)(2 * k + 1) * tf;
    }
    rc = build_anchor_tables(h, tp, s, true);
    if (rc != POEM_OK) { poem_destroy(h); return rc; }
    h->c_qeqp0 = h->tab_mem + cx + 4 * tf;
    if (poem_launch_gemm_split(h->R(T_QEMB), C, h->fused[0].w[1], h->fused[0].b[1], nullptr, 0, h->c_qeqp0, 2 * C, cfg->nquery, 2 * C, C,
                               POEM_ACT_NONE, 2 * C, POEM_ACT_NONE, s) != hipSuccess) {
      g_last_hip_error = (int)hipGetLastError(); poem_destroy(h); return POEM_E_LAUNCH;
    }
  }
  *out = h;
  return POEM_OK;
}

void poem_destroy(poem_handle_t h) {
  if (!h) return;
  POEM_TRACE("destroy h=%p graphs=%zu", (void*)h, h->graph_cache.size());
  for (auto e : h->prof_ev) (void)hipEventDestroy(e);
  if (h->tab_mem) (void)hipFree(h->tab_mem);
  if (h->split_mem) (void)hipFree(h->split_mem);
  if (h->gemm_split) (void)hipFree(h->gemm_split);
  if (h->native16) (void)hipFree(h->native16);
  if (h->gemm_scales) (void)hipFree(h->gemm_scales);
  park_execs(h);
  return_kit(h);
  delete h;
}

int poem_set_overlap(poem_handle_t h, int enable) {
  if (!h) return POEM_E_ARG;
  h->overlap = enable != 0;
  return POEM_OK;
}

int poem_set_chains(poem_handle_t h, int enable) {
  if (!h) return POEM_E_ARG;
  h->chains = enable != 0;
  return POEM_OK;
}

int poem_set_option(poem_handle_t h, const char* name, int value) {
  if (!h || !name) return POEM_E_ARG;
  const std::string k(name);
  if (k == "overlap") h->overlap = value != 0;
  else if (k == "anchor_tables") h->anchor_tables = value != 0;
  else if (k == "chains") h->chains = value != 0;
  else if (k == "knn_early") h->knn_early = value != 0;
  else if (k == "fused_sampling") h->fused_sampling = value != 0;
  else if (k == "chain_combine") h->chain_combine = value != 0;
  else if (k == "xattn_merge") { if (value < -1 || value > 1) return POEM_E_ARG; h->xattn_merge = value; }
  else if (k == "tables_first") h->tables_first = value != 0;
  else if (k == "tables_cached") h->tables_cached = value != 0;
  else if (k == "knn_fma") h->knn_fma = value != 0;
  else if (k == "knn_query") {
    if (value < 0 || value > 64 || value > h->cfg.nquery) return POEM_E_ARG;
    if (h->precision != POEM_PRECISION_FP32 && value != 0 && value != 32) return POEM_E_UNSUPPORTED;
    h->knn_query = value;
  }
  else if (k == "graphs") h->graphs = value != 0;
  else if (k == "graph_eager") h->graph_eager = value != 0;
  else if (k == "gemm_xcd_map") { poem_gemm_xcd_map(value != 0); g_proc_switches.fetch_and(~1); g_proc_switches.fetch_or(value ? 1 : 0); }
  else if (k == "f1_split") h->f1_split = value != 0;
  else if (k == "xattn_half") { poem_cross_attention_half(value != 0); g_proc_switches.fetch_and(~4); g_proc_switches.fetch_or(value ? 4 : 0); }
  else if (k == "xattn_tail") { poem_cross_attention_tail_halves(value != 0); g_proc_switches.fetch_and(~8); g_proc_switches.fetch_or(value ? 8 : 0); }
  else if (k == "wait_merge") { if (value < -1 || value > 7) return POEM_E_ARG; h->wait_merge = value; }
  else if (k == "d2_first") { if (value < 0 || value > 1) return POEM_E_ARG; h->d2_first = value; }
  else if (k == "va_p1") { if (value < -1 || value > 2) return POEM_E_ARG; h->va_p1 = value; }
  else if (k == "gemm_kslab") { poem_gemm_kslab(value != 0); g_proc_switches.fetch_and(~2); g_proc_switches.fetch_or(value ? 2 : 0); }
  else if (k == "small_batch") h->small_batch = value;
  else if (k == "group_xcd") h->group_xcd = value != 0;
  else if (k == "group_min_views") { if (value < -1) return POEM_E_ARG; h->group_min_views = value; }
  else if (k == "bps_defer") { if (value < 0 || value > 3) return POEM_E_ARG; h->bps_defer = value; }
  else if (k == "chain_tile") { if (value < 0 || value > 3) return POEM_E_ARG; h->chain_tile = value; }
  else return POEM_E_ARG;
  return POEM_OK;
}

int poem_graph_stats(poem_handle_t h, int64_t* out, int n) {
  if (!h || !out || n < 9) return POEM_E_ARG;
  out[0] = (int64_t)h->graph_cache.size();
  out[1] = h->graph_captures; out[2] = h->graph_instantiations; out[3] = h->graph_replays; out[4] = h->plain_forwards;
  out[5] = h->layout_uploads;
  std::lock_guard<std::mutex> lock(g_pool_mutex);
  out[6] = (int64_t)g_parked_execs.size(); out[7] = g_exec_reuses; out[8] = g_exec_update_failures;
  if (n >= 10) out[9] = g_exec_busy_skips;
  return POEM_OK;
}

int poem_attach_mano(poem_handle_t h, const void* table, int center_idx) {
  if (!h || center_idx < -1 || center_idx > 20) return POEM_E_ARG;
  if (table && !h->cfg.parametric) return POEM_E_UNSUPPORTED;
  h->mano_table = (const float*)table;
  h->mano_center = center_idx;
  return POEM_OK;
}

int poem_set_anchor_tables(poem_handle_t h, int enable) {
  if (!h) return POEM_E_ARG;
  h->anchor_tables = enable != 0;
  return POEM_OK;
}

int poem_set_precision(poem_handle_t h, int mode) {
  if (!h || mode < POEM_PRECISION_FP32 || mode > POEM_PRECISION_SPLIT_F16X3_ALL) return POEM_E_ARG;
  if (mode != POEM_PRECISION_FP32 && (!h->split_mem || !h->gemm_split)) return POEM_E_UNSUPPORTED;
  if (mode != POEM_PRECISION_FP32 && (h->cfg.knn != 32 || (h->knn_query && h->knn_query != 32)))
    return POEM_E_UNSUPPORTED;
  if (mode != POEM_PRECISION_FP32 && h->cfg.nsample % 32)
    return POEM_E_UNSUPPORTED;
  h->precision = mode;
  return POEM_OK;
}

int poem_enable_taps(poem_handle_t h, int enable) {
  if (!h) return POEM_E_ARG;
  h->taps = enable != 0;
  return POEM_OK;
}

int64_t poem_tap(poem_handle_t h, const char* name, void* dst, int64_t dst_elems, void* stream) {
  if (!h || !name) return POEM_E_ARG;
  auto it = h->tapmap.find(name);
  if (it == h->tapmap.end()) return POEM_E_ARG;
  if (dst) {
    if (dst_elems < it->second.elems) return POEM_E_ARG;
    HIPCHK(hipMemcpyAsync(dst, it->second.p, (size_t)it->second.elems * 4, hipMemcpyDeviceToDevice, (hipStream_t)stream));
  }
  return it->second.elems;
}
int poem_profile_enable(poem_handle_t h, int max_launches) {
  if (!h || max_launches < 0) return POEM_E_ARG;
  for (auto e : h->prof_ev) (void)hipEventDestroy(e);
  h->prof_ev.clear();
  h->prof_used = 0;
  h->prof_on = max_launches > 0;
  h->prof_kind.assign((size_t)max_launches, 0);
  for (int i = 0; i < 2 * max_launches; ++i) {
    hipEvent_t e;
    HIPCHK(hipEventCreate(&e));
    h->prof_ev.push_back(e);
  }
  return POEM_OK;
}

static int profile_sum(poem_handle_t h, int kind, int* launches, float* total_ms) {
  float tot = 0.f;
  int n = 0;
  for (int i = 0; i < h->prof_used; ++i) {
    if (h->prof_kind[i] != kind) continue;
    HIPCHK(hipEventSynchronize(h->prof_ev[2 * i + 1]));
    float ms = 0.f;
    HIPCHK(hipEventElapsedTime(&ms, h->prof_ev[2 * i], h->prof_ev[2 * i + 1]));
    tot += ms;
    ++n;
  }
// ... 23 lines not shown
```

### poem-v2_amd/csrc/launchers.h

```cpp
#pragma once
#include <hip/hip_runtime.h>

#include "chain.h"
#include "loss.h"
#include "merge.h"

extern "C" {
hipError_t poem_launch_pack_linear(const float* w, int N, int K, void* out, hipStream_t s);
hipError_t poem_launch_gemm(const float* X, int ldx, const void* Wp, const float* bias, const float* R, int ldr,
                            float* Y, int ldy, int M, int N, int K, int act, hipStream_t s);
hipError_t poem_launch_gemm2(const float* X, int ldx, const void* Wp, const float* bias, const float* R, int ldr,
                             float* Y, int ldy, int M, int N, int K, int act, int in_pa, int out_pa, hipStream_t s);
hipError_t poem_launch_unpack_rows(const void* pa, int N, int K, float* out, hipStream_t s);
hipError_t poem_launch_layernorm(const float* x, const float* g, const float* b, float* y, int rows, int cols,
                                 float eps, hipStream_t s);
hipError_t poem_launch_narrow_linear(const float* x, int ldx, const float* w, const float* b, const float* base,
                                     float* out, int rows, int K, int N, hipStream_t s);
hipError_t poem_launch_sine_pe(float* out, int F, int H, int W, int max_views, int normalize, hipStream_t s);
hipError_t poem_launch_frustum_features(const float* intr, const float* extr, float* out, int views, int H, int W, int D, int lid,
                                        double depth_start, double depth_end, const double* position_range, int img0, int img1,
                                        hipStream_t s);
hipError_t poem_launch_conv1x1_ex(const float* feat, const void* Wp, const float* bias, const float* table, const int* pe_index,
                                  float* x, float* xt, int views, int K, int C, int hw, int relu, hipStream_t s);
int poem_sample_merge_supported(int C, int S, int hw);
hipError_t poem_launch_project_table(const float* bps, const float* centre, const int* view_sample, const float* intr,
                                     const float* inv_extr, void* tabw, void* tabo, float* uv, int views, int C, int fh, int fw, int S,
                                     int img_w, int img_h, hipStream_t s);
hipError_t poem_launch_view_layout(const ViewLayoutArgs* a, hipStream_t s);
hipError_t poem_launch_input_tables(const float* bps, const float* ref_joints, const float* tmpl, const int* view_sample,
                                    const float* intr, const float* extr, void* tabw, void* tabo, float* centre, float* pt_xyz, float* query_xyz,
                                    int views, int B, int S, int Q, int fh, int fw, int img_w, int img_h, float radius, hipStream_t s);
hipError_t poem_launch_sample_merge(const SampleMergeArgs* a, int C, hipStream_t s);
hipError_t poem_launch_sample_group(const SampleGroupArgs* a, int C, hipStream_t s);
int poem_device_cu_count(void);
hipError_t poem_launch_merge_tail(const MergeTailArgs* a, int C, hipStream_t s);
hipError_t poem_launch_invert_extr(const float* extr, float* inv, int views, hipStream_t s);
hipError_t poem_launch_conv1x1(const float* feat, const void* Wp, const float* bias, const float* table,
                               const int* pe_index, float* x, float* xt, int views, int K, int C, int hw, hipStream_t s);
hipError_t poem_launch_project_sample(const float* x, const float* bps, const float* centre, const int* view_sample,
                                      const float* intr, const float* extr, float* inv_scratch, float* uv, float* g,
                                      int views, int C, int fh, int fw, int S, int img_w, int img_h, hipStream_t s);
hipError_t poem_launch_project_uv(const float* bps, const float* centre, const int* view_sample, const float* intr,
                                  const float* extr, float* inv_scratch, float* uv, int views, int fh, int fw, int S, int img_w,
                                  int img_h, hipStream_t s);
hipError_t poem_launch_grid_sample(const float* x, const float* uv, float* g, int views, int C, int fh, int fw, int S, hipStream_t s);
hipError_t poem_launch_grid_sample_ex(const float* x, const float* uv, float* g, int views, int C, int fh, int fw, int S, int staged,
                                      hipStream_t s);
hipError_t poem_launch_merge_reduce(const float* h2, const int* offs, float* m, int B, int S, int HALF, hipStream_t s);
hipError_t poem_launch_merge_finalize(const float* g, const float* y, const int* offs, float* out, int B, int S, int C,
                                      hipStream_t s);
hipError_t poem_launch_cross_attention(const float* q, const float* k, const float* v, float* ctx, int B, int NQ, int NK,
                                       int C, int heads, int ldkv, float* scratch, hipStream_t s);
size_t poem_cross_attention_scratch_floats(int B, int NQ, int NK, int C, int heads, int with_images);
hipError_t poem_launch_cross_attention_img(const float* q, int ldq, const void* kimg, const void* vimg, float* ctx, int B,
                                           int NQ, int NK, int C, int heads, float* scratch, hipStream_t s);
hipError_t poem_launch_gemm_segs(const float* X, int ldx, const void* Wp, const float* bias, int M, int K, int act,
                                 int seg_cols, int nsegs, float* const* outs, const int* modes, hipStream_t s);
hipError_t poem_launch_cross_attention_imgq(const float* q, int ldq, int q_batch_rows, const void* kimg, const void* vimg,
                                            float* ctx, int B, int NQ, int NK, int C, int heads, float* scratch, hipStream_t s);
int poem_chain_supported(int C);
int poem_chain_combines(int C, int heads, int chunks);
void poem_cross_attention_partials(int B, int NQ, int NK, int C, int heads, float* scratch, const void** part_o,
                                   const void** part_ml, int* chunks, float* kc2);
hipError_t poem_launch_chain(const ChainArgs* a, int C, hipStream_t s);
hipError_t poem_launch_native16(const void* packed, void* native, size_t bytes, hipStream_t s);
int poem_chain16_wants_native(int C);
hipError_t poem_launch_knn(const float* qxyz, const float* sxyz, int* idx, int B, int NQ, int NS, int fma, hipStream_t s);
hipError_t poem_launch_knn_k(const float* qxyz, const float* sxyz, int* idx, int B, int NQ, int NS, int K, int ld, int fma,
                             hipStream_t s);
hipError_t poem_launch_vector_attention(const float* query_xyz, const float* src_xyz, const float* anchor_xyz,
                                        const int* idx, int shared_idx, const float* q, const float* k, const float* v,
                                        int nsrc, const float* wd1, const float* bd1, const void* wd2, const float* bd2,
                                        const void* wg1, const float* bg1, const void* wg2, const float* bg2, float* out,
                                        int B, int Q, int C, int ldq, int ldk, int ldv, int composed, hipStream_t s);
hipError_t poem_launch_vector_attention_k(const float* query_xyz, const float* src_xyz, const int* idx, int K, int ld,
                                          const float* q, const float* k, const float* v, int nsrc, const float* wd1,
                                          const float* bd1, const void* wd2, const float* bd2, const void* wg1, const float* bg1,
                                          const void* wg2, const float* bg2, float* out, int B, int Q, int C, int ldq, int ldk,
                                          int ldv, int composed, hipStream_t s);
size_t poem_vector_attention_table_floats(int Q, int C);
hipError_t poem_launch_vector_attention_tables(const float* query_xyz, const float* anchor_xyz, const int* idx,
                                               const float* wd1, const float* bd1, const void* wd2, const float* bd2,
                                               const void* wg1d2, float* tab_g, float* tab_p, int Q, int C, hipStream_t s);
hipError_t poem_launch_vector_attention_anchored(const int* idx, const float* qg, const float* kg, const float* v, int nsrc,
                                                 const void* wg2, const float* tab_g, const float* tab_p, float* out, int B,
                                                 int Q, int C, int ldq, int ldk, int ldv, hipStream_t s);
hipError_t poem_launch_gather_anchor_rows(const float* src, int ld, const int* idx, int NS, float* dst, int B, int C,
                                          int* ident, hipStream_t s);
hipError_t poem_launch_pad_rows(const float* src, float* dst, int B, int S, int SP, int W, hipStream_t s);
hipError_t poem_launch_canon_xyz(const float* tmpl, float* out, int n, float radius, hipStream_t s);
hipError_t poem_launch_pack_split(const float* w, int C, void* img, float* scale_out, hipStream_t s);
hipError_t poem_launch_pack_split_tiles(const float* w, int N, int K, void* img, float* scales, int scale_stride, hipStream_t s);
void poem_gemm_split_context(const void* packed, size_t bytes, const void* split, const float* scales);
void poem_gemm_split_explicit(const void* img, const float* scales);
void poem_cross_attention_split(int on);
void poem_cross_attention_masked_form(int on);
void poem_cross_attention_half(int on);
void poem_cross_attention_tail_halves(int on);
int poem_cross_attention_merges(int NK, int C, int heads);
int poem_cross_attention_fits(int B, int NK, int C);
hipError_t poem_launch_cross_attention_merged_rm(const float* q, const float* k, const float* v, float* ctx, int B, int NQ, int NK,
                                                 int C, int heads, float* scratch, hipStream_t s);
hipError_t poem_launch_cross_attention_merged(const float* q, int ldq, int q_batch_rows, const void* kimg, const void* vimg, float* ctx,
                                              int B, int NQ, int NK, int C, int heads, hipStream_t s);
int poem_gemm_split_applies(const void* Wp, int M, int ldx, int K);
void poem_gemm_split_images(int on);
void poem_gemm_xcd_map(int on);
void poem_gemm_kslab(int on);
void poem_vecattn_one_query_blocks(int on);
void poem_vecattn_valid_neighbours(int k);
hipError_t poem_launch_vector_attention_split(const float* query_xyz, const float* src_xyz, const float* anchor_xyz,
                                              const int* idx, int shared_idx, const float* q, const float* k,
                                              const float* v, int nsrc, const float* wd1, const float* bd1,
                                              const void* wd2, const float* bd2, const void* wg1, const void* wg2,
                                              const float* scales, float* out, int B, int Q, int C, int ldq,
                                              int ldk, int ldv, hipStream_t s);
hipError_t poem_launch_dlt(const float* uv, const float* intr, const float* mat, const int* offs, float* out, int B, int J,
                           int invert, hipStream_t s);
hipError_t poem_launch_dlt_confidence(const float* uv, const float* conf, const float* intr, const float* mat,
                                      const int* offs, float* out, int* sel_count, int B, int J, int invert, int mode,
                                      double threshold, hipStream_t s);
hipError_t poem_launch_pa_epe(const float* pred, const float* gt, float* out, int B, int P, hipStream_t s);
hipError_t poem_launch_pck_accumulate(const float* pred, const float* gt, int B, int P, double vmin, double vmax, int steps,
                                      unsigned int* counts, double* sum, unsigned int* n, float* dist_out, hipStream_t s);
hipError_t poem_launch_mano_to_openpose(const float* jreg, const float* verts, float* joints, int B, int nverts,
                                        hipStream_t s);
hipError_t poem_launch_warp_affine(const unsigned char* src, const long long* src_off, const int* src_hw,
                                   const double* minv, const double* gain, float* out_f32, unsigned char* out_u8, int views,
                                   int OH, int OW, hipStream_t s);
hipError_t poem_launch_heatmap_uv(const float* hmap, float* uv, int maps, int hh, int hw, float img_w, float img_h,
                                  hipStream_t s);
hipError_t poem_launch_heatmap_uv_conf(const float* hmap, float* uv, float* conf, int maps, int hh, int hw, float img_w,
                                       float img_h, hipStream_t s);
size_t poem_conv3x3_packed_floats(int Cout, int Cin);
hipError_t poem_launch_upcat_conv3x3(const float* a_half, int Ca, const float* b_full, int Cb, const void* wp, const float* scale,
                                     const float* shift, float* out, int views, int Cout, int H, int W, int relu, long out_ns,
                                     int out_cs, int out_rs, int out_off, hipStream_t s);
hipError_t poem_launch_pack_conv3x3(const float* w, int Cout, int Cin, void* out, hipStream_t s);
hipError_t poem_launch_conv3x3(const float* in, const void* wp, const float* scale, const float* shift, const float* res,
                               float* out, int views, int Cin, int Cout, int H, int W, int stride, int relu, long out_ns,
                               int out_cs, int out_rs, int out_off, hipStream_t s);
hipError_t poem_launch_conv3x3_ex(const float* in, const void* wp, const float* scale, const float* shift, const float* res,
                                  long res_ns, int res_cs, int res_rs, int res_off, int res_pre, float* out, int views, int Cin,
                                  int Cout, int H, int W, int stride, int relu, long out_ns, int out_cs, int out_rs, int out_off,
                                  hipStream_t s);
size_t poem_conv1x1_packed_floats(int Cout, int Cin);
hipError_t poem_launch_pack_conv1x1(const float* w, int Cout, int Cin, void* out, hipStream_t s);
hipError_t poem_launch_conv1x1_nchw(const float* in, long in_ns, int in_cs, int in_rs, int in_off, const void* wp,
                                    const float* shift, const float* res, long res_ns, int res_cs, int res_rs, int res_off,
                                    float* out, long out_ns, int out_cs, int out_rs, int out_off, int views, int Cin, int Cout,
                                    int H, int W, int relu, hipStream_t s);
hipError_t poem_launch_hrnet_fuse(const float* const* ptrs, const long* ns, const int* cs, const int* rs, const int* off,
                                  const int* shift, int nterms, float* out, long out_ns, int out_cs, int out_rs, int out_off,
                                  int views, int C, int H, int W, hipStream_t s);
size_t poem_conv7x7_packed_floats(int Cout);
hipError_t poem_launch_pack_conv7x7(const float* w, int Cout, void* out, hipStream_t s);
hipError_t poem_launch_conv7x7_s2(const float* in, const void* wp, const float* scale, const float* shift, float* out, long out_ns,
                                  int out_cs, int out_rs, int out_off, int views, int Cout, int H, int W, hipStream_t s);
hipError_t poem_launch_maxpool3x3_s2(const float* in, long in_ns, int in_cs, int in_rs, int in_off, float* out, long out_ns,
                                     int out_cs, int out_rs, int out_off, int views, int C, int H, int W, hipStream_t s);
hipError_t poem_launch_upcat_pad_staged(const float* a, int Ca, const float* b, int Cb, float* out, int views, int H, int W,
                                        hipStream_t s);
hipError_t poem_launch_sconv1x1(const float* in, long in_ns, int in_cs, int in_rs, int in_off, const void* wp, const float* shift,
                                float* out, long out_ns, int out_cs, int out_rs, int out_off, int views, int Cin, int Cout, int H,
                                int W, int pool, int act, hipStream_t s);
hipError_t poem_launch_conv3x3_down2(const float* in, const void* wp, const float* scale, const float* shift, const float* res,
                                     float* out, int views, int Cin, int Cout, int H, int W, int relu, long out_ns, int out_cs,
                                     int out_rs, int out_off, hipStream_t s);
void poem_decode_s2_staging_wave(int on);
void poem_decode_row_stager(int on);
void poem_decode_pin32(int on);
// ... 42 lines not shown
```

### poem-v2_amd/csrc/misc.hip

```cpp
#include "common.h"
#include <algorithm>
#include "merge.h"

__global__ void prep_xyz_kernel(const float* __restrict__ ref_joints, const float* __restrict__ bps,
                                const float* __restrict__ tmpl, float* __restrict__ centre, float* __restrict__ pt_xyz,
                                float* __restrict__ query_xyz, int B, int S, int Q, float radius) {
  poem_prep_xyz_elem((long)blockIdx.x * blockDim.x + threadIdx.x, ref_joints, bps, tmpl, centre, pt_xyz, query_xyz, B, S, Q, radius);
}

extern "C" hipError_t poem_launch_prep_xyz(const float* ref_joints, const float* bps, const float* tmpl, float* centre,
                                           float* pt_xyz, float* query_xyz, int B, int S, int Q, float radius,
                                           hipStream_t s) {
  const long total = (long)B * S * 3 + (long)B * Q * 3 + 3L * B;
  hipLaunchKernelGGL(prep_xyz_kernel, dim3((unsigned)((total + 255) / 256)), dim3(256), 0, s, ref_joints, bps, tmpl,
                     centre, pt_xyz, query_xyz, B, S, Q, radius);
  return hipGetLastError();
}

__global__ void canon_xyz_kernel(const float* __restrict__ tmpl, float* __restrict__ out, int n, float radius) {
  const int i = blockIdx.x * blockDim.x + threadIdx.x;
  if (i < n) out[i] = __fdiv_rn(tmpl[i], radius);
}

extern "C" hipError_t poem_launch_canon_xyz(const float* tmpl, float* out, int n, float radius, hipStream_t s) {
  hipLaunchKernelGGL(canon_xyz_kernel, dim3((unsigned)((n + 255) / 256)), dim3(256), 0, s, tmpl, out, n, radius);
  return hipGetLastError();
}

__global__ void gather_anchor_rows_kernel(const float* __restrict__ src, int ld, const int* __restrict__ idx, int NS,
                                          float* __restrict__ dst, int B, int C, int* __restrict__ ident) {
  const long i = (long)blockIdx.x * blockDim.x + threadIdx.x;
  const int c4 = C / 4;
  if (i < (long)B * 32 * c4) {
    const int c = (int)(i % c4), r = (int)(i / c4), b = r >> 5, j = r & 31;
    reinterpret_cast<float4*>(dst)[i] = *reinterpret_cast<const float4*>(src + ((size_t)b * NS + idx[j]) * ld + 4 * c);
  }
  if (ident && i < 32) ident[i] = (int)i;
}

extern "C" hipError_t poem_launch_gather_anchor_rows(const float* src, int ld, const int* idx, int NS, float* dst, int B,
                                                     int C, int* ident, hipStream_t s) {
  const long total = (long)B * 32 * (C / 4);
  hipLaunchKernelGGL(gather_anchor_rows_kernel, dim3((unsigned)((total + 255) / 256)), dim3(256), 0, s, src, ld, idx, NS,
                     dst, B, C, ident);
  return hipGetLastError();
}

__global__ void pad_rows_kernel(const float* __restrict__ src, float* __restrict__ dst, int S, int SP, int W, long total) {
  const long i = (long)blockIdx.x * blockDim.x + threadIdx.x;
  if (i >= total) return;
  const int w = (int)(i % W);
  const long r = i / W;
  const int row = (int)(r % SP);
  const long b = r / SP;
  dst[i] = row < S ? src[((size_t)b * S + row) * W + w] : 0.f;
}

extern "C" hipError_t poem_launch_pad_rows(const float* src, float* dst, int B, int S, int SP, int W, hipStream_t s) {
  const long total = (long)B * SP * W;
  hipLaunchKernelGGL(pad_rows_kernel, dim3((unsigned)((total + 255) / 256)), dim3(256), 0, s, src, dst, S, SP, W, total);
  return hipGetLastError();
}

__global__ void broadcast_rows_kernel(const float* __restrict__ src, float* __restrict__ dst, long per, long total) {
  const long i = (long)blockIdx.x * blockDim.x + threadIdx.x;
  if (i < total) dst[i] = src[i % per];
}

extern "C" hipError_t poem_launch_broadcast(const float* src, float* dst, long per, int copies, hipStream_t s) {
  const long total = per * copies;
  hipLaunchKernelGGL(broadcast_rows_kernel, dim3((unsigned)((total + 255) / 256)), dim3(256), 0, s, src, dst, per, total);
  return hipGetLastError();
}

__global__ void finalize_kernel(const float* __restrict__ xyz, const float* __restrict__ centre, float* __restrict__ out,
                                int L, int B, int Q, float radius, const float* __restrict__ mano_verts,
                                const float* __restrict__ mano_joints) {
  const long i = (long)blockIdx.x * blockDim.x + threadIdx.x;
  if (i >= (long)L * B * Q * 3) return;
  const int d = (int)(i % 3);
  const int b = (int)((i / (3L * Q)) % B);
  if (mano_verts && i >= (long)(L - 1) * B * Q * 3) {
    const int qq = (int)((i / 3) % Q);
    float v = qq < 21 ? mano_joints[((size_t)b * 21 + qq) * 3 + d] : mano_verts[((size_t)b * (Q - 21) + (qq - 21)) * 3 + d];
    if (isnan(v)) v = 0.f;
    else if (isinf(v)) v = v > 0 ? 3.4028234663852886e38f : -3.4028234663852886e38f;
    out[i] = v + centre[b * 3 + d];
    return;
  }
  float v = xyz[i];
  if (isnan(v)) v = 0.f;
  else if (isinf(v)) v = v > 0 ? 3.4028234663852886e38f : -3.4028234663852886e38f;
  out[i] = v * radius + centre[b * 3 + d];
}

extern "C" hipError_t poem_launch_finalize(const float* xyz, const float* centre, float* out, int L, int B, int Q,
                                           float radius, const float* mano_verts, const float* mano_joints, hipStream_t s) {
  const long total = (long)L * B * Q * 3;
  hipLaunchKernelGGL(finalize_kernel, dim3((unsigned)((total + 255) / 256)), dim3(256), 0, s, xyz, centre, out, L, B, Q,
                     radius, mano_verts, mano_joints);
  return hipGetLastError();
}

__global__ void param_rows_kernel(const float* __restrict__ verts, const float* __restrict__ joints, float* __restrict__ out_last,
                                  int B, int Q) {
  const long i = (long)blockIdx.x * blockDim.x + threadIdx.x;
  if (i >= (long)B * Q * 3) return;
  const int d = (int)(i % 3), qq = (int)((i / 3) % Q), b = (int)(i / (3L * Q));
  out_last[i] = qq < 21 ? joints[((size_t)b * 21 + qq) * 3 + d] : verts[((size_t)b * (Q - 21) + (qq - 21)) * 3 + d];
}

extern "C" hipError_t poem_launch_param_rows(const float* verts, const float* joints, float* out_last, int B, int Q, hipStream_t s) {
  const long total = (long)B * Q * 3;
  hipLaunchKernelGGL(param_rows_kernel, dim3((unsigned)((total + 255) / 256)), dim3(256), 0, s, verts, joints, out_last, B, Q);
  return hipGetLastError();
}

__global__ void finalize_param_kernel(const float* __restrict__ verts, const float* __restrict__ joints,
                                      const float* __restrict__ ref_joints, float* __restrict__ out_last, int B, int Q) {
  const long i = (long)blockIdx.x * blockDim.x + threadIdx.x;
  if (i >= (long)B * Q * 3) return;
  const int d = (int)(i % 3), qq = (int)((i / 3) % Q), b = (int)(i / (3L * Q));
  const float c = ref_joints[((size_t)b * 21 + 9) * 3 + d];
  float v = qq < 21 ? joints[((size_t)b * 21 + qq) * 3 + d] : verts[((size_t)b * (Q - 21) + (qq - 21)) * 3 + d];
  if (isnan(v)) v = 0.f;
  else if (isinf(v)) v = v > 0 ? 3.4028234663852886e38f : -3.4028234663852886e38f;
  out_last[i] = v + c;
// ... 127 lines not shown
```

### poem-v2_amd/csrc/ops.cpp

```cpp
#include <cmath>
#include <cstring>
#include "engine.h"

extern "C" {

int poem_gemm(const float* x, int ldx, const void* w_packed, const float* bias, const float* residual, int ldr, float* y,
              int ldy, int M, int N, int K, int act, void* stream) {
  if (!x || !w_packed || !y || M <= 0 || N <= 0 || K <= 0 || K % 8 || ldx % 4 || ((uintptr_t)x & 15)) return POEM_E_ARG;
  if (act < 0 || act > 2) return POEM_E_ARG;
  HIPCHK(poem_launch_gemm(x, ldx, w_packed, bias, residual, ldr, y, ldy, M, N, K, act, (hipStream_t)stream));
  return POEM_OK;
}

int poem_gemm_ex(const float* x, int ldx, const void* w_packed, const float* bias, const float* residual, int ldr,
                 float* y, int ldy, int M, int N, int K, int act, int in_layout, int out_layout, void* stream) {
  if (!x || !w_packed || !y || M <= 0 || N <= 0 || K <= 0 || K % 8 || ((uintptr_t)x & 15) || ((uintptr_t)y & 15))
    return POEM_E_ARG;
  if (!in_layout && ldx % 4) return POEM_E_ARG;
  if (out_layout && N % 32) return POEM_E_ARG;
  if (act < 0 || act > 2 || (in_layout & ~1) || (out_layout & ~1)) return POEM_E_ARG;
  HIPCHK(poem_launch_gemm2(x, ldx, w_packed, bias, residual, ldr, y, ldy, M, N, K, act, in_layout, out_layout,
                           (hipStream_t)stream));
  return POEM_OK;
}

int poem_pack_rows(const float* x, int rows, int cols, void* packed, void* stream) {
  return poem_pack_linear(x, rows, cols, packed, stream);
}

int poem_unpack_rows(const void* packed, int rows, int cols, float* x, void* stream) {
  if (!packed || !x || rows <= 0 || cols % 8) return POEM_E_ARG;
  HIPCHK(poem_launch_unpack_rows(packed, rows, cols, x, (hipStream_t)stream));
  return POEM_OK;
}

int poem_layernorm(const float* x, const float* gamma, const float* beta, float* y, int rows, int cols, float eps,
                   void* stream) {
  if (!x || !gamma || !beta || !y || rows <= 0 || cols <= 0) return POEM_E_ARG;
  HIPCHK(poem_launch_layernorm(x, gamma, beta, y, rows, cols, eps, (hipStream_t)stream));
  return POEM_OK;
}

int poem_pe_table_ex(const void* adapt_w_packed, const float* adapt_b, int embed, int fh, int fw, int max_views, int normalize,
                     float* scratch_sine, float* table, void* stream) {
  if (!adapt_w_packed || !adapt_b || !scratch_sine || !table || embed % 2 || (fh * fw) % 32) return POEM_E_ARG;
  hipStream_t s = (hipStream_t)stream;
  HIPCHK(poem_launch_sine_pe(scratch_sine, embed / 2, fh, fw, max_views, normalize != 0, s));
  HIPCHK(poem_launch_conv1x1(scratch_sine, adapt_w_packed, adapt_b, nullptr, nullptr, table, nullptr, (int)pe_views(max_views),
                             3 * embed / 2, embed, fh * fw, s));
  return POEM_OK;
}

int poem_pe_table(const void* adapt_w_packed, const float* adapt_b, int embed, int fh, int fw, int max_views,
                  float* scratch_sine, float* table, void* stream) {
  return poem_pe_table_ex(adapt_w_packed, adapt_b, embed, fh, fw, max_views, 1, scratch_sine, table, stream);
}

int poem_frustum_features(const poem_config_t* cfg, const float* cam_intr, const float* cam_extr, int views, int img0, int img1,
                          float* out, void* stream) {
  if (!cfg || !cam_intr || !cam_extr || !out || views <= 0 || cfg->depth_num <= 0 || cfg->feat_h <= 0 || cfg->feat_w <= 0) return POEM_E_ARG;
  HIPCHK(poem_launch_frustum_features(cam_intr, cam_extr, out, views, cfg->feat_h, cfg->feat_w, cfg->depth_num, cfg->lid != 0,
                                      cfg->depth_start, cfg->depth_end, cfg->position_range, img0, img1, (hipStream_t)stream));
  return POEM_OK;
}

int poem_input_proj(const float* feat, const void* w_packed, const float* bias, const float* table,
                    const int32_t* pe_index, float* x, int views, int in_channels, int embed, int hw, void* stream) {
  if (!feat || !w_packed || !x || views <= 0 || in_channels % 8 || hw % 32) return POEM_E_ARG;
  if (table && !pe_index) return POEM_E_ARG;
  HIPCHK(poem_launch_conv1x1(feat, w_packed, bias, table, pe_index, x, nullptr, views, in_channels, embed, hw, (hipStream_t)stream));
  return POEM_OK;
}

int poem_project_sample(const float* x, const float* bps, const float* centre, const int32_t* view_sample,
                        const float* cam_intr, const float* cam_extr, float* uv_scratch, float* g, int views, int embed,
                        int fh, int fw, int nsample, int img_w, int img_h, void* stream) {
  if (!x || !bps || !centre || !view_sample || !cam_intr || !cam_extr || !uv_scratch || !g || views <= 0) return POEM_E_ARG;
  float* inv = uv_scratch + (size_t)views * nsample * 2;
  HIPCHK(poem_launch_project_sample(x, bps, centre, view_sample, cam_intr, cam_extr, inv, uv_scratch, g, views, embed, fh,
                                    fw, nsample, img_w, img_h, (hipStream_t)stream));
  return POEM_OK;
}

int poem_merge_reduce(const float* h2, const int32_t* view_offsets, float* m, int batch, int nsample, int half,
                      void* stream) {
  if (!h2 || !view_offsets || !m || half > 512 || batch <= 0) return POEM_E_ARG;
  HIPCHK(poem_launch_merge_reduce(h2, view_offsets, m, batch, nsample, half, (hipStream_t)stream));
  return POEM_OK;
}

int poem_merge_finalize(const float* g, const float* y, const int32_t* view_offsets, float* out, int batch, int nsample,
                        int embed, void* stream) {
  if (!g || !y || !view_offsets || !out || batch <= 0) return POEM_E_ARG;
  HIPCHK(poem_launch_merge_finalize(g, y, view_offsets, out, batch, nsample, embed, (hipStream_t)stream));
  return POEM_OK;
}

size_t poem_cross_attention_scratch_bytes(int batch, int nq, int nk, int embed, int heads) {
  if (batch <= 0 || nq <= 0 || nk <= 0 || heads <= 0 || embed % heads) return 0;
  return poem_cross_attention_scratch_floats(batch, nq, nk, embed, heads, 1) * sizeof(float);
}

int poem_cross_attention(const float* q, const float* k, const float* v, float* ctx, int batch, int nq, int nk, int embed,
                         int heads, void* scratch, size_t scratch_bytes, void* stream) {
  if (!q || !k || !v || !ctx || batch <= 0 || nq <= 0 || nk <= 0 || heads <= 0 || embed % heads) return POEM_E_ARG;
// ... 521 lines not shown
```

### poem-v2_amd/csrc/plan.cpp

```cpp
#include "engine.h"

Plan make_plan(const poem_config_t& c, int B, int BN, void* base, int idx_ld) {
  Plan p{};
  p.idx_ld = idx_ld;
  Arena a(base);
  const size_t C = c.embed, S = c.nsample, Q = c.nquery, HW = (size_t)c.feat_h * c.feat_w;
  const size_t BS = (size_t)B * S, BQ = (size_t)B * Q, VS = (size_t)BN * S;
  const size_t SP = (size_t)padded_samples(c), BSP = (size_t)B * SP;
  p.offs = a.take<int32_t>(B + 1);
  p.view_sample = a.take<int32_t>(BN);
  p.pe_index = a.take<int32_t>(BN);
  p.x = a.take<float>((size_t)BN * C * HW);
  p.uv = a.take<float>(VS * 2 + (size_t)BN * 16);
  p.h2 = a.take<float>(VS * C / 2);
  p.bps_feat = a.take<float>(BS * C);
  const size_t front = a.off;
  p.g = a.take<float>(VS * C);
  p.h1 = a.take<float>(VS * C);
  p.mm = a.take<float>(BS * C / 2);
  p.mh = a.take<float>(BS * C / 2);
  p.y = a.take<float>(BS * C);
  const size_t end_ops = a.off;
  a.off = front;
  p.xt = a.take<float>((size_t)BN * C * HW);
  p.ptab = a.take<float>(VS * 8);
  p.q1 = a.take<float>(BS * C);
  a.off = std::max(a.off, end_ops);
  p.centre = a.take<float>((size_t)B * 3);
  p.pt_xyz = a.take<float>(BS * 3);
  for (int i = 0; i <= c.nblocks; ++i) p.xyz[i] = nullptr;
  float* xyz_all = a.take<float>((size_t)(c.nblocks + 1) * BQ * 3);
  for (int i = 0; i <= c.nblocks; ++i) p.xyz[i] = xyz_all ? xyz_all + (size_t)i * BQ * 3 : nullptr;
  p.feats0 = a.take<float>(BQ * C);
  p.qeqp = a.take<float>(BQ * C * 2);
  p.qp = a.take<float>(BQ * C);
  p.ctx = a.take<float>(BQ * C);
  p.att = a.take<float>(BQ * C);
  p.h_attn = a.take<float>(BQ * C);
  p.y3 = a.take<float>(BQ * C * 3);
  p.rs = a.take<float>(BQ * C);
  p.qc = a.take<float>(BQ * C);
  p.rc = a.take<float>(BQ * C);
  p.y4 = a.take<float>(BQ * C * 5);
  p.ffo = a.take<float>(BQ * C);
  for (int i = 0; i < c.nblocks; ++i) {
    p.h_cross[i] = a.take<float>(BQ * C);
    p.f_self[i] = a.take<float>(BQ * C);
    p.f_cross[i] = a.take<float>(BQ * C);
    p.feats[i] = a.take<float>(BQ * C);
    p.idx_self[i] = a.take<int32_t>(BQ * idx_ld);
    p.idx_cross[i] = a.take<int32_t>(BQ * idx_ld);
    p.y1[i] = a.take<float>(BSP * C * 6);
  }
  p.q3t = a.take<float>((size_t)B * C);
  p.par = a.take<float>((size_t)B * 106);
  p.g_pose = a.take<float>((size_t)B * 48);
  p.g_betas = a.take<float>((size_t)B * 10);
  p.mano_verts = a.take<float>((size_t)B * 778 * 3);
  p.mano_joints = a.take<float>((size_t)B * 21 * 3);
  p.attn_scratch = a.take<float>(poem_cross_attention_scratch_floats(B, (int)Q, (int)S, (int)C, c.heads, 0) + 4);
  p.canon_xyz = a.take<float>(Q * 3);
  for (int k = 0; k < 2; ++k) {
    p.anch_x[k] = a.take<float>((size_t)B * 32 * C);
    p.anch_kv[k] = a.take<float>((size_t)B * 32 * C * 2);
  }
  p.qeqp0 = a.take<float>(Q * C * 2);
  p.ident = a.take<int32_t>(32);
  for (int k = 0; k < 2; ++k) {
    p.tab_g[k] = a.take<float>(poem_vector_attention_table_floats((int)Q, (int)C));
    p.tab_p[k] = a.take<float>(poem_vector_attention_table_floats((int)Q, (int)C));
  }
  if (c.petr_embedding) {
    p.petr_f = a.take<float>((size_t)BN * 3 * c.depth_num * HW);
    p.petr_h = a.take<float>((size_t)BN * 2 * C * HW);
    p.petr_tab = a.take<float>((size_t)BN * C * HW);
  }
  p.feat_pad = p.xyz_pad = nullptr;
  if (SP != S) {
    p.feat_pad = a.take<float>(BSP * C);
    p.xyz_pad = a.take<float>(BSP * 3);
  }
  p.bytes = align_up(a.off, 256);
  return p;
}
void register_taps(poem_handle_t h, const Plan& p, int B, int BN, bool sampling) {
  const poem_config_t& c = h->cfg;
  const int64_t C = c.embed, S = c.nsample, Q = c.nquery, HW = c.feat_h * c.feat_w;
  const int64_t BS = B * S, BQ = B * Q;
  h->tapmap.clear();
  if (!h->taps) return;
  auto put = [&](const std::string& k, const void* ptr, int64_t n) { h->tapmap[k] = {ptr, n}; };
  if (sampling) {
    put("x", p.x, (int64_t)BN * C * HW);
    if (!(h->fused_sampling && h->precision == POEM_PRECISION_FP32 && poem_sample_merge_supported((int)C, (int)S, (int)HW)))
      put("g", p.g, (int64_t)BN * C * S);
    put("bps_feat", p.bps_feat, BS * C);
    put("pt_xyz", p.pt_xyz, BS * 3);
  }
  put("query_xyz", p.xyz[0], BQ * 3);
  for (int i = 0; i < c.nblocks; ++i) {
    const std::string pre = "b" + std::to_string(i) + ".";
    put(pre + "h_cross", p.h_cross[i], BQ * C);
    put(pre + "f_self", p.f_self[i], BQ * C);
    put(pre + "f_cross", p.f_cross[i], BQ * C);
    put(pre + "feats", p.feats[i], BQ * C);
    put(pre + "xyz", p.xyz[i + 1], BQ * 3);
    if (i > 0) {
      put(pre + "idx_self", p.idx_self[i], BQ * p.idx_ld);
      put(pre + "idx_cross", p.idx_cross[i], BQ * p.idx_ld);
    }
  }
}

extern "C" {

size_t poem_workspace_bytes(poem_handle_t h, int batch, int total_views) {
  if (!h || batch <= 0 || total_views < batch || h->cfg.nblocks > 8) return 0;
  return make_plan(h->cfg, batch, total_views, nullptr, neighbour_ld(h->cfg, h->knn_query)).bytes;
}
}
```

### poem-v2_amd/hip.py

```python
import ctypes
import os
import subprocess

import numpy as np
import torch

_HERE = os.path.dirname(os.path.abspath(__file__))
CSRC = os.path.join(_HERE, "csrc")
LIB_PATH = os.environ.get("POEM_HIP_LIB") or os.path.join(CSRC, "libpoem_hip.so")
ASSETS = os.path.join(_HERE, "assets")

ACT_NONE, ACT_RELU, ACT_GELU = 0, 1, 2
PRECISIONS = {"fp32": 0, "split_f16x3": 1, "split_f16x3_all": 2}


class PoemConfig(ctypes.Structure):
    _fields_ = [("embed", ctypes.c_int32), ("in_channels", ctypes.c_int32), ("nsample", ctypes.c_int32),
                ("nquery", ctypes.c_int32), ("heads", ctypes.c_int32), ("nblocks", ctypes.c_int32),
                ("knn", ctypes.c_int32), ("parametric", ctypes.c_int32), ("feat_h", ctypes.c_int32),
                ("feat_w", ctypes.c_int32), ("max_views", ctypes.c_int32), ("radius", ctypes.c_float),
                ("ln_eps", ctypes.c_float),
                ("pe_normalize", ctypes.c_int32), ("petr_embedding", ctypes.c_int32), ("depth_num", ctypes.c_int32),
                ("lid", ctypes.c_int32), ("reserved0", ctypes.c_int32), ("depth_start", ctypes.c_double),
                ("depth_end", ctypes.c_double), ("position_range", ctypes.c_double * 6)]


class PoemLossCfg(ctypes.Structure):
    _fields_ = [("joints_weight", ctypes.c_double), ("vertices_weight", ctypes.c_double), ("joints_2d_weight", ctypes.c_double),
                ("vertices_2d_weight", ctypes.c_double), ("heatmap_joints_weight", ctypes.c_double), ("pose_weight", ctypes.c_double),
                ("shape_weight", ctypes.c_double), ("joints_l2", ctypes.c_int32), ("vertices_l2", ctypes.c_int32),
                ("parametric", ctypes.c_int32), ("center_idx", ctypes.c_int32), ("img_h", ctypes.c_int32), ("img_w", ctypes.c_int32)]


class PoemFuseTerm(ctypes.Structure):
    _fields_ = [("data", ctypes.c_void_p), ("view_stride", ctypes.c_int64), ("ch_stride", ctypes.c_int32),
                ("row_stride", ctypes.c_int32), ("offset", ctypes.c_int32), ("shift", ctypes.c_int32)]


LOSS_NTERMS = 10

_vp, _i, _f, _sz, _i64 = ctypes.c_void_p, ctypes.c_int, ctypes.c_float, ctypes.c_size_t, ctypes.c_int64
_cfgp = ctypes.POINTER(PoemConfig)

SIGNATURES = {
    "poem_abi_version": (_i, []),
    "poem_last_hip_error": (_i, []),
    "poem_error_string": (ctypes.c_char_p, [_i]),
    "poem_num_weight_tensors": (_i, [_cfgp]),
    "poem_weight_tensor_numel": (_i64, [_cfgp, _i]),
    "poem_packed_bytes": (_sz, [_cfgp]),
    "poem_create": (_i, [_cfgp, ctypes.POINTER(_vp), _i, _vp, _vp, _vp, _vp, _vp, _sz, _vp, ctypes.POINTER(_vp)]),
    "poem_destroy": (None, [_vp]),
    "poem_workspace_bytes": (_sz, [_vp, _i, _i]),
    "poem_graph_stats": (_i, [_vp, ctypes.POINTER(ctypes.c_int64), _i]),
    "poem_head_forward": (_i, [_vp, _vp, _vp, _vp, ctypes.POINTER(ctypes.c_int32), _i, _vp, _i, _i, _vp, _vp, _vp, _vp,
                               _sz, _vp]),
    "poem_decoder_forward": (_i, [_vp, _vp, _vp, _vp, _vp, _i, _vp, _vp, _vp, _vp, _sz, _vp]),
    "poem_finalize_parametric": (_i, [_vp, _vp, _vp, _vp, _i, _vp, _vp]),
    "poem_tap": (_i64, [_vp, ctypes.c_char_p, _vp, _i64, _vp]),
    "poem_enable_taps": (_i, [_vp, _i]),
    "poem_profile_enable": (_i, [_vp, _i]),
    "poem_profile_read": (_i, [_vp, ctypes.POINTER(_i), ctypes.POINTER(_f), _i]),
    "poem_profile_read_anchored": (_i, [_vp, ctypes.POINTER(_i), ctypes.POINTER(_f)]),
    "poem_packed_linear_bytes": (_sz, [_i, _i]),
    "poem_pack_linear": (_i, [_vp, _i, _i, _vp, _vp]),
    "poem_set_overlap": (_i, [_vp, _i]),
    "poem_set_anchor_tables": (_i, [_vp, _i]),
    "poem_set_chains": (_i, [_vp, _i]),
    "poem_set_option": (_i, [_vp, ctypes.c_char_p, _i]),
    "poem_set_precision": (_i, [_vp, _i]),
    "poem_pack_split_linear": (_i, [_vp, _i, _vp, _vp, _vp]),
    "poem_pack_split_gemm": (_i, [_vp, _i, _i, _vp, _vp, _vp]),
    "poem_gemm_split": (_i, [_vp, _i, _vp, _vp, _vp, _vp, _i, _vp, _i, _i, _i, _i, _i, _vp]),
    "poem_vector_attention_split": (_i, [_vp, _vp, _vp, _vp, _i, _vp, _vp, _vp, _i, _vp, _vp, _vp, _vp, _vp, _vp, _vp, _vp,
                                         _i, _i, _i, _vp]),
    "poem_gemm": (_i, [_vp, _i, _vp, _vp, _vp, _i, _vp, _i, _i, _i, _i, _i, _vp]),
    "poem_gemm_ex": (_i, [_vp, _i, _vp, _vp, _vp, _i, _vp, _i, _i, _i, _i, _i, _i, _i, _vp]),
    "poem_pack_rows": (_i, [_vp, _i, _i, _vp, _vp]),
    "poem_unpack_rows": (_i, [_vp, _i, _i, _vp, _vp]),
    "poem_layernorm": (_i, [_vp, _vp, _vp, _vp, _i, _i, _f, _vp]),
    "poem_pe_table": (_i, [_vp, _vp, _i, _i, _i, _i, _vp, _vp, _vp]),
    "poem_pe_table_ex": (_i, [_vp, _vp, _i, _i, _i, _i, _i, _vp, _vp, _vp]),
    "poem_frustum_features": (_i, [_cfgp, _vp, _vp, _i, _i, _i, _vp, _vp]),
    "poem_input_proj": (_i, [_vp, _vp, _vp, _vp, _vp, _vp, _i, _i, _i, _i, _vp]),
    "poem_project_sample": (_i, [_vp, _vp, _vp, _vp, _vp, _vp, _vp, _vp, _i, _i, _i, _i, _i, _i, _i, _vp]),
    "poem_merge_reduce": (_i, [_vp, _vp, _vp, _i, _i, _i, _vp]),
    "poem_merge_finalize": (_i, [_vp, _vp, _vp, _vp, _i, _i, _i, _vp]),
    "poem_cross_attention_scratch_bytes": (_sz, [_i, _i, _i, _i, _i]),
    "poem_cross_attention": (_i, [_vp, _vp, _vp, _vp, _i, _i, _i, _i, _i, _vp, _sz, _vp]),
    "poem_cross_attention_merged": (_i, [_vp, _vp, _vp, _vp, _i, _i, _i, _i, _i, _vp, _sz, _vp]),
    "poem_cross_attention_split_f16x3": (_i, [_vp, _vp, _vp, _vp, _i, _i, _i, _i, _i, _vp, _sz, _vp]),
    "poem_triangulate_dlt": (_i, [_vp, _vp, _vp, _vp, _i, _i, _i, _vp, _vp]),
    "poem_heatmap_uv": (_i, [_vp, _vp, _i, _i, _i, _i, _f, _f, _vp]),
    "poem_heatmap_uv_conf": (_i, [_vp, _vp, _vp, _i, _i, _i, _i, _f, _f, _vp]),
    "poem_dlt_confidence": (_i, [_vp, _vp, _vp, _vp, _vp, _vp, _vp, _i, _i, _i, _i, ctypes.c_double, _vp]),
    "poem_conv3x3_packed_bytes": (_sz, [_i, _i]),
    "poem_pack_conv3x3": (_i, [_vp, _i, _i, _vp, _vp]),
    "poem_conv3x3": (_i, [_vp, _vp, _vp, _vp, _vp, _vp, _i, _i, _i, _i, _i, _i, _i, _i64, _i, _i, _i, _vp]),
    "poem_conv3x3_ex": (_i, [_vp, _vp, _vp, _vp, _vp, _i64, _i, _i, _i, _i, _vp, _i, _i, _i, _i, _i, _i, _i, _i64, _i, _i, _i, _vp]),
    "poem_conv1x1_packed_bytes": (_sz, [_i, _i]),
    "poem_pack_conv1x1": (_i, [_vp, _i, _i, _vp, _vp]),
    "poem_conv1x1": (_i, [_vp, _i64, _i, _i, _i, _vp, _vp, _vp, _i64, _i, _i, _i, _vp, _i64, _i, _i, _i, _i, _i, _i, _i, _i, _i, _vp]),
    "poem_hrnet_fuse": (_i, [_vp, _i, _vp, _i64, _i, _i, _i, _i, _i, _i, _i, _vp]),
    "poem_conv7x7_packed_bytes": (_sz, [_i]),
    "poem_pack_conv7x7": (_i, [_vp, _i, _vp, _vp]),
    "poem_conv7x7_s2": (_i, [_vp, _vp, _vp, _vp, _vp, _i64, _i, _i, _i, _i, _i, _i, _i, _vp]),
    "poem_maxpool3x3_s2": (_i, [_vp, _i64, _i, _i, _i, _vp, _i64, _i, _i, _i, _i, _i, _i, _i, _vp]),
    "poem_conv1x1_s2": (_i, [_vp, _i64, _i, _i, _i, _vp, _vp, _vp, _i64, _i, _i, _i, _i, _i, _i, _i, _i, _vp]),
    "poem_maxpool2_conv1x1": (_i, [_vp, _vp, _vp, _vp, _i, _i, _i, _i, _i, _i, _vp]),
    "poem_upsample2_concat_pad_staged": (_i, [_vp, _i, _vp, _i, _vp, _i, _i, _i, _vp]),
    "poem_set_decode_option": (_i, [ctypes.c_char_p, _i]),
    "poem_conv3x3_down2": (_i, [_vp, _vp, _vp, _vp, _vp, _vp, _i, _i, _i, _i, _i, _i, _i64, _i, _i, _i, _vp]),
    "poem_upsample2_concat_pad": (_i, [_vp, _i, _vp, _i, _vp, _i, _i, _i, _i, _vp]),
    "poem_conv1x1_upsample2": (_i, [_vp, _vp, _vp, _vp, _i, _i, _i, _i, _i, _vp]),
    "poem_upcat_conv3x3": (_i, [_vp, _i, _vp, _i, _vp, _vp, _vp, _vp, _i, _i, _i, _i, _i, _i64, _i, _i, _i, _vp]),
    "poem_pool_conv1x1_sigmoid": (_i, [_vp, _vp, _vp, _vp, _i, _i, _i, _i, _i, _vp]),
    "poem_upcat_conv3x3_pool_head": (_i, [_vp, _i, _vp, _i, _vp, _vp, _vp, _vp, _vp, _vp, _i, _i, _i, _i, _i, _i, _vp]),
    "poem_pa_epe": (_i, [_vp, _vp, _vp, _i, _i, _vp]),
    "poem_mano_to_openpose": (_i, [_vp, _vp, _vp, _i, _i, _vp]),
    "poem_rot6d_to_axis_angle": (_i, [_vp, _vp, _vp, _i, _vp]),
    "poem_mano_table_bytes": (_sz, []),
    "poem_mano_prepare": (_i, [_vp, _vp, _vp, _vp, _vp, _vp, _vp]),
    "poem_mano_lbs": (_i, [_vp, _vp, _vp, _i, _i, _vp, _vp, _vp]),
    "poem_attach_mano": (_i, [_vp, _vp, _i]),
    "poem_profile_read_stage": (_i, [_vp, _i, ctypes.POINTER(_i), ctypes.POINTER(_f)]),
    "poem_warp_affine": (_i, [_vp, _vp, _vp, _vp, _vp, _vp, _vp, _i, _i, _i, _vp]),
    "poem_pck_accumulate": (_i, [_vp, _vp, _i, _i, ctypes.c_double, ctypes.c_double, _i, _vp, _vp, _vp, _vp, _vp]),
    "poem_knn": (_i, [_vp, _vp, _vp, _i, _i, _i, _vp]),
    "poem_knn_ex": (_i, [_vp, _vp, _vp, _i, _i, _i, _i, _vp]),
    "poem_knn_k": (_i, [_vp, _vp, _vp, _i, _i, _i, _i, _i, _i, _vp]),
    "poem_vector_attention_k": (_i, [_vp, _vp, _vp, _i, _i, _vp, _vp, _vp, _i, _vp, _vp, _vp, _vp, _vp, _vp, _vp, _vp, _vp,
                                     _i, _i, _i, _vp]),
    "poem_vector_attention": (_i, [_vp, _vp, _vp, _vp, _i, _vp, _vp, _vp, _i, _vp, _vp, _vp, _vp, _vp, _vp, _vp, _vp, _vp,
                                   _i, _i, _i, _vp]),
    "poem_reg_update": (_i, [_vp, _vp, _vp, _vp, _vp, _i, _i, _vp]),
    "poem_render_workspace_bytes": (_sz, [_i, _i, _i]),
    "poem_render_mesh": (_i, [_vp, _vp, _vp, _vp, _vp, _vp, _vp, _vp, _vp, _i, _vp, _f, _vp, _vp, _vp, _i, _i, _i, _i, _i, _i, _vp, _sz,
                              _vp]),
    "poem_project_points": (_i, [_vp, _vp, _vp, _vp, _vp, _i, _i, _i, _vp]),
    "poem_draw_skeleton": (_i, [_vp, _vp, _vp, _vp, _i, _i, _i, _vp]),
    "poem_loss_workspace_bytes": (_sz, [_i, _i]),
    "poem_loss_terms": (_i, [_vp, _vp, _vp, _vp, _vp, _vp, _vp, _vp, _vp, _vp, _vp, _vp, _vp, ctypes.POINTER(PoemLossCfg), _i, _i, _vp,
                             _vp, _sz, _vp]),
}

_LIB = None


def build(verbose=False):
    out = subprocess.run(["make", "-C", CSRC, "-j8"], capture_output=True, text=True)
    if verbose or out.returncode != 0:
        print(out.stdout[-4000:])
        print(out.stderr[-4000:])
    if out.returncode != 0:
        raise RuntimeError("building libpoem_hip.so failed")
    return LIB_PATH


def lib():
    global _LIB
# ... 184 lines not shown
    def profile_read_stage(self, stage):
        n, ms = _i(0), _f(0.0)
        check(lib().poem_profile_read_stage(self.handle, int(stage), ctypes.byref(n), ctypes.byref(ms)), "poem_profile_read_stage")
        return n.value, ms.value

    def profile_read_anchored(self):
        n, ms = _i(0), _f(0.0)
        check(lib().poem_profile_read_anchored(self.handle, ctypes.byref(n), ctypes.byref(ms)), "poem_profile_read_anchored")
        return n.value, ms.value

    def head_forward(self, mlvl_feat, cam_intr, cam_extr, cam_view_num, reference_joints, inp_img_shape):
        c = self.cfg
        views = [int(v) for v in cam_view_num]
        B, BN = len(views), int(sum(views))
        if tuple(mlvl_feat.shape) != (BN, c.in_channels, c.feat_h, c.feat_w):
            raise RuntimeError(f"mlvl_feat shape {tuple(mlvl_feat.shape)} != {(BN, c.in_channels, c.feat_h, c.feat_w)}")
        for what, t, shape in (("cam_intr", cam_intr, (BN, 3, 3)), ("cam_extr", cam_extr, (BN, 4, 4)),
                               ("reference_joints", reference_joints, (B, 21, 3))):
            if tuple(t.shape) != shape:
                raise RuntimeError(f"{what} shape {tuple(t.shape)} != {shape} (cam_view_num sums to {BN} views, {B} samples)")
        offs = (ctypes.c_int32 * (B + 1))(*np.concatenate([[0], np.cumsum(views)]).astype(np.int32).tolist())
        ws, need = self._ws(B, max(BN, B * c.max_views))
        out = torch.empty(c.nblocks, B, c.nquery, 3, dtype=torch.float32, device=self.device)
        pose = torch.empty(B, 48, dtype=torch.float32, device=self.device) if c.parametric else None
        betas = torch.empty(B, 10, dtype=torch.float32, device=self.device) if c.parametric else None
        with torch.cuda.device(self.device):
            check(lib().poem_head_forward(self.handle, ptr(mlvl_feat), ptr(cam_intr), ptr(cam_extr), offs, B,
                                          ptr(reference_joints), int(inp_img_shape[0]), int(inp_img_shape[1]),
                                          ptr(out), ptr(pose), ptr(betas), ws.data_ptr(), need, stream()),
                  "poem_head_forward")
        return out, pose, betas

    def decoder_forward(self, query_xyz, query_feat, pt_xyz, pt_feats):
        c = self.cfg
        B = query_xyz.shape[0]
        ws, need = self._ws(B, B)
        out = torch.empty(c.nblocks, B, c.nquery, 3, dtype=torch.float32, device=self.device)
        pose = torch.empty(B, 48, dtype=torch.float32, device=self.device) if c.parametric else None
        betas = torch.empty(B, 10, dtype=torch.float32, device=self.device) if c.parametric else None
        with torch.cuda.device(self.device):
            check(lib().poem_decoder_forward(self.handle, ptr(query_xyz), ptr(query_feat), ptr(pt_xyz), ptr(pt_feats), B,
                                             ptr(out), ptr(pose), ptr(betas), ws.data_ptr(), need, stream()),
                  "poem_decoder_forward")
        return out, pose, betas

    def attach_mano(self, table, center_idx):
        check(lib().poem_attach_mano(self.handle, None if table is None else table.data_ptr(), int(center_idx)), "poem_attach_mano")
        self._mano = table
        self._mano_center = int(center_idx)

    def finalize_parametric(self, verts, joints, reference_joints, out):
        with torch.cuda.device(self.device):
            check(lib().poem_finalize_parametric(self.handle, ptr(verts), ptr(joints), ptr(reference_joints),
                                                 out.shape[1], ptr(out), stream()), "poem_finalize_parametric")
        return out

    def tap(self, name, shape, dtype=torch.float32):
        n = lib().poem_tap(self.handle, name.encode(), None, 0, None)
        check(n, f"poem_tap({name})")
        t = torch.empty(int(n), dtype=dtype, device=self.device)
        with torch.cuda.device(self.device):
            check(lib().poem_tap(self.handle, name.encode(), t.data_ptr(), int(n), stream()))
        return t.view(*shape)


def pack_linear(w):
    n, k = w.shape
    nbytes = lib().poem_packed_linear_bytes(n, k)
    if nbytes == 0:
        raise RuntimeError("in_features must be a multiple of 8")
    out = torch.empty(nbytes, dtype=torch.uint8, device=w.device)
    check(lib().poem_pack_linear(ptr(w), n, k, out.data_ptr(), stream()), "poem_pack_linear")
    return out


def gemm(x, w_packed, n_out, bias=None, residual=None, act=ACT_NONE):
    M, K = x.shape
    y = torch.empty(M, n_out, dtype=torch.float32, device=x.device)
    check(lib().poem_gemm(ptr(x), K, w_packed.data_ptr(), ptr(bias), ptr(residual), n_out, ptr(y), n_out, M, n_out, K,
                          act, stream()), "poem_gemm")
    return y


def pack_rows(x):
    return pack_linear(x)


def unpack_rows(pa, rows, cols):
    x = torch.empty(rows, cols, dtype=torch.float32, device=pa.device)
    check(lib().poem_unpack_rows(pa.data_ptr(), rows, cols, ptr(x), stream()), "poem_unpack_rows")
    return x


def gemm_ex(x, w_packed, M, n_out, K, bias=None, residual=None, act=ACT_NONE, in_pa=False, out_pa=False):
    if out_pa:
        y = torch.empty(lib().poem_packed_linear_bytes(M, n_out), dtype=torch.uint8, device=x.device)
    else:
        y = torch.empty(M, n_out, dtype=torch.float32, device=x.device)
    rptr = None if residual is None else residual.data_ptr()
    check(lib().poem_gemm_ex(x.data_ptr(), K, w_packed.data_ptr(), ptr(bias), rptr, n_out, y.data_ptr(), n_out, M, n_out,
                             K, act, int(in_pa), int(out_pa), stream()), "poem_gemm_ex")
    return y


def layernorm(x, g, b, eps):
    y = torch.empty_like(x)
    check(lib().poem_layernorm(ptr(x), ptr(g), ptr(b), ptr(y), x.shape[0], x.shape[1], eps, stream()), "poem_layernorm")
    return y


def cross_attention(q, k, v, heads, split=False, merged=False):
    B, NQ, C = q.shape
    ctx = torch.empty_like(q)
    need = lib().poem_cross_attention_scratch_bytes(B, NQ, k.shape[1], C, heads)
    scratch = torch.empty(max(need, 16), dtype=torch.uint8, device=q.device)
    fn = lib().poem_cross_attention_split_f16x3 if split else (lib().poem_cross_attention_merged if merged else lib().poem_cross_attention)
    check(fn(ptr(q), ptr(k), ptr(v), ptr(ctx), B, NQ, k.shape[1], C, heads, scratch.data_ptr(), need, stream()),
          "poem_cross_attention")
    return ctx


def knn(query_xyz, src_xyz, fma=False, k=32):
    B, NQ, _ = query_xyz.shape
    if k != 32:
        idx = torch.empty(B, NQ, k, dtype=torch.int32, device=query_xyz.device)
        check(lib().poem_knn_k(ptr(query_xyz), ptr(src_xyz), idx.data_ptr(), B, NQ, src_xyz.shape[1], k, k, int(bool(fma)),
                               stream()), "poem_knn_k")
        return idx
    idx = torch.empty(B, NQ, 32, dtype=torch.int32, device=query_xyz.device)
    if fma:
        check(lib().poem_knn_ex(ptr(query_xyz), ptr(src_xyz), idx.data_ptr(), B, NQ, src_xyz.shape[1], 1, stream()), "poem_knn_ex")
    else:
        check(lib().poem_knn(ptr(query_xyz), ptr(src_xyz), idx.data_ptr(), B, NQ, src_xyz.shape[1], stream()), "poem_knn")
    return idx


def vector_attention(query_xyz, src_xyz, anchor_xyz, idx, q, k, v, wd1, bd1, wd2p, bd2, wg1p, bg1, wg2p, bg2, nk=None):
    B, NQ, C = q.shape
    out = torch.empty_like(q)
    if nk is not None:
        assert idx.dim() == 3 and idx.stride(-1) == 1 and idx.stride(1) == idx.shape[2] and anchor_xyz is None
        check(lib().poem_vector_attention_k(ptr(query_xyz), ptr(src_xyz), idx.data_ptr(), int(nk), idx.shape[2], ptr(q), ptr(k),
                                            ptr(v), k.shape[1], ptr(wd1), ptr(bd1), wd2p.data_ptr(), ptr(bd2), wg1p.data_ptr(),
                                            ptr(bg1), wg2p.data_ptr(), ptr(bg2), ptr(out), B, NQ, C, stream()),
              "poem_vector_attention_k")
        return out
    shared = 1 if idx.dim() == 1 else 0
    check(lib().poem_vector_attention(ptr(query_xyz), ptr(src_xyz), ptr(anchor_xyz), idx.data_ptr(), shared, ptr(q), ptr(k),
                                      ptr(v), k.shape[1], ptr(wd1), ptr(bd1), wd2p.data_ptr(), ptr(bd2), wg1p.data_ptr(),
                                      ptr(bg1), wg2p.data_ptr(), ptr(bg2), ptr(out), B, NQ, C, stream()),
          "poem_vector_attention")
    return out



def gemm_split(x, w, bias=None, residual=None, act=ACT_NONE):
    N, K = w.shape
    M = x.shape[0]
    nt = (N + 31) // 32
    img = torch.empty(nt * 32 * K * 4, dtype=torch.uint8, device=w.device)
    sc = torch.empty(nt, dtype=torch.float32, device=w.device)
    check(lib().poem_pack_split_gemm(ptr(w), N, K, img.data_ptr(), sc.data_ptr(), stream()), "poem_pack_split_gemm")
    y = torch.empty(M, N, dtype=torch.float32, device=w.device)
    check(lib().poem_gemm_split(ptr(x), x.stride(0), img.data_ptr(), sc.data_ptr(), ptr(bias), ptr(residual),
                                residual.stride(0) if residual is not None else 0, ptr(y), N, M, N, K, act, stream()),
          "poem_gemm_split")
# ... 39 lines not shown
```

Measured before the change: 1474.

## Compute cross-attention K/V projection only for rows referenced by kNN indices

For decoder blocks after the first, the last two output segments of the fused basis-point projection (used by cross attention) are no longer computed for all padded sample rows. A new kernel marks which sample rows the cross-attention kNN index actually references and compacts them into a row list. A row-gathering variant of the panel GEMM then computes only those rows on the knn stream, with an event so the consumer waits. This trades a smaller GEMM for an extra mark/compact pass, a second launch, a serialisation dependency on the kNN result, and gathered row loads.

```diff
diff --git a/include/poem_hip.h b/include/poem_hip.h
--- a/include/poem_hip.h
+++ b/include/poem_hip.h
@@ -99,6 +99,10 @@
 #define POEM_LAYOUT_PA 1
 int poem_gemm_ex(const float* x, int ldx, const void* w_packed, const float* bias, const float* residual, int ldr,
                  float* y, int ldy, int M, int N, int K, int act, int in_layout, int out_layout, void* stream);
+int poem_mark_rows(const int32_t* idx, int batch, int nq, int k, int ld, int nsrc, int src_stride, int32_t* list, int32_t* count,
+                   int cap, int32_t* scratch, void* stream);
+int poem_gemm_rows(const float* x, int ldx, const void* w_packed, const float* bias, float* y, int nrows, int N, int K,
+                   const int32_t* rows, const int32_t* count, int cap, void* stream);
 int poem_pack_rows(const float* x, int rows, int cols, void* packed, void* stream);
 int poem_unpack_rows(const void* packed, int rows, int cols, float* x, void* stream);
 int poem_layernorm(const float* x, const float* gamma, const float* beta, float* y, int rows, int cols, float eps,
diff --git a/poem-v2_amd/csrc/decoder.cpp b/poem-v2_amd/csrc/decoder.cpp
--- a/poem-v2_amd/csrc/decoder.cpp
+++ b/poem-v2_amd/csrc/decoder.cpp
@@ -51,6 +51,11 @@
   bool bps_waited[9] = {}, knn_waited[9] = {};
   bool anchor_from_y3 = false;
 
+  bool vc_listed(int i) const {
+    return i >= 1 && h->vc_rows && h->precision == POEM_PRECISION_FP32 && p.vc_list[i] && S <= 8192 && poem_gemm_rows_supported(C, C, 2) != 0 &&
+           (unsigned long long)BSP * C * 4ull < (1ull << 32);
+  }
+
   DecoderRun(poem_handle_t h_, Plan& p_, const float* feats_in, const float* pt_xyz_, const float* pt_feats_, int B_, float* pose,
              float* bet, hipStream_t s_, bool template_queries)
       : h(h_), p(p_), c(h_->cfg), pt_xyz(pt_xyz_), pt_feats(pt_feats_), pose_aa(pose), betas(bet), B(B_), C(c.embed), S(c.nsample),
@@ -103,10 +108,11 @@
     const int modes[6] = {1, 2, 1, 2, 0, 0};
     h->kv_presplit[i] = poem_gemm_split_applies(f.w[0], BSP, C, C) != 0;
     const bool anchored = tables && i == 0;
-    if (!anchored && h->f1_split && C % 128 == 0) {
+    if (!anchored && (vc_listed(i) || (h->f1_split && C % 128 == 0))) {
       HIPCHK(poem_launch_gemm_segs(pt_feats, C, f.w[0], f.b[0], BSP, C, POEM_ACT_NONE, C, 4, outs, modes, sb));
-      HIPCHK(poem_launch_gemm_segs(pt_feats, C, (const float*)f.w[0] + (size_t)4 * C * C, f.b[0] + 4 * C, BSP, C, POEM_ACT_NONE, C, 2, outs + 4,
-                                   modes + 4, sb));
+      if (!vc_listed(i))
+        HIPCHK(poem_launch_gemm_segs(pt_feats, C, (const float*)f.w[0] + (size_t)4 * C * C, f.b[0] + 4 * C, BSP, C, POEM_ACT_NONE, C, 2, outs + 4,
+                                     modes + 4, sb));
     } else {
       HIPCHK(poem_launch_gemm_segs(pt_feats, C, f.w[0], f.b[0], BSP, C, POEM_ACT_NONE, C, anchored ? 4 : 6, outs, modes, sb));
     }
@@ -151,6 +157,15 @@
     }
     if (ov) HIPCHK(hipEventRecord(h->ev_knn[i], sk));
     knn_issued[i] = true;
+    if (vc_listed(i)) {
+      const auto& f = h->fused[i];
+      float* outs[2] = {p.y1[i] + 4 * (size_t)BSP * C, p.y1[i] + 5 * (size_t)BSP * C};
+      HIPCHK(poem_launch_mark_rows(p.idx_cross[i], B, Q, p.idx_ld == 32 ? 32 : c.knn, p.idx_ld, S, SP, p.vc_list[i], p.vc_count[i], BSP,
+                                   p.vc_scratch, sk));
+      HIPCHK(poem_launch_gemm_rows(pt_feats, C, (const float*)f.w[0] + (size_t)4 * C * C, f.b[0] + 4 * C, C, C, 2, outs, p.vc_list[i],
+                                   p.vc_count[i], BSP, BSP, sk));
+      if (ov) HIPCHK(hipEventRecord(h->ev_vc[i], sk));
+    }
     return POEM_OK;
   }
 
@@ -333,6 +348,7 @@
         HIPCHK(hipStreamWaitEvent(s, h->ev_bps[k], 0));
         bps_waited[k] = true;
       }
+    if (ov && vc_listed(i)) HIPCHK(hipStreamWaitEvent(s, h->ev_vc[i], 0));
     const bool prof = prof_begin();
     const int kc = shared ? 32 : c.knn;
     if (h->precision != POEM_PRECISION_FP32) {
diff --git a/poem-v2_amd/csrc/engine.h b/poem-v2_amd/csrc/engine.h
--- a/poem-v2_amd/csrc/engine.h
+++ b/poem-v2_amd/csrc/engine.h
@@ -121,6 +121,8 @@
   float *c_canon_xyz = nullptr, *c_tab_g[2] = {}, *c_tab_p[2] = {};
   float* c_qeqp0 = nullptr;
   hipEvent_t ev_bps[8] = {}, ev_xyz[8] = {}, ev_knn[8] = {}, ev_def[8] = {};
+  hipEvent_t ev_vc[8] = {};
+  bool vc_rows = true;
   int bps_defer = 0;
   bool f1_split = true;
   int va_p1 = -1;
@@ -150,6 +152,8 @@
 
 struct Plan {
   int32_t *offs, *view_sample, *pe_index, *idx_self[8], *idx_cross[8];
+  int32_t *vc_list[8], *vc_count[8];
+  int32_t *vc_scratch;
   float *x, *uv, *g, *h1, *h2, *mm, *mh, *y, *bps_feat, *centre, *pt_xyz, *xyz[9];
   float *xt, *ptab, *q1;
   float *petr_f, *petr_h, *petr_tab;
diff --git a/poem-v2_amd/csrc/forward.cpp b/poem-v2_amd/csrc/forward.cpp
--- a/poem-v2_amd/csrc/forward.cpp
+++ b/poem-v2_amd/csrc/forward.cpp
@@ -182,7 +182,7 @@
     if (!h->graphs || h->graph_broken || h->prof_on || h->tables_pending || !h->cap_stream) return 0;
     const std::vector<int64_t> key = {B, plan_views, fused_fe ? -1 : BN, (int64_t)(uintptr_t)workspace, h->precision, h->anchor_tables, h->chains,
                                       h->fused_sampling, h->tables_first, h->chain_combine, h->knn_early, h->overlap, h->chain_tile,
-                                      h->tables_cached, h->knn_fma, h->knn_query, h->taps, c.parametric, h->xattn_merge, h->small_batch, h->bps_defer, poem_process_switches(), h->f1_split, h->va_p1, h->group_min_views, h->group_xcd, h->d2_first, h->wait_merge,
+                                      h->tables_cached, h->knn_fma, h->knn_query, h->taps, c.parametric, h->xattn_merge, h->small_batch, h->bps_defer, poem_process_switches(), h->f1_split, h->va_p1, h->group_min_views, h->group_xcd, h->d2_first, h->wait_merge, h->vc_rows,
                                       (int64_t)(uintptr_t)h->mano_table, h->mano_center};
     poem_handle_s::GraphEntry* hit = nullptr;
     for (auto& g : h->graph_cache)
diff --git a/poem-v2_amd/csrc/gemm.hip b/poem-v2_amd/csrc/gemm.hip
--- a/poem-v2_amd/csrc/gemm.hip
+++ b/poem-v2_amd/csrc/gemm.hip
@@ -468,12 +468,14 @@
 }
 
 
-template <int NT, int MT, bool GELU, int OMODE, bool SPLIT = false>
+template <int NT, int MT, bool GELU, int OMODE, bool SPLIT = false, bool ROWS = false>
 __device__ __forceinline__ void panel_rows(const float* __restrict__ X, int ldx, const float4* __restrict__ wl,
                                            const float* __restrict__ bias, const float* __restrict__ R, int ldr,
                                            float* __restrict__ Y, int ldy, int M, int K, int pact, int col0, int ycol0,
                                            int bip, int blocks_in_panel, const float* __restrict__ tile_scales = nullptr,
-                                           int scale_stride = 0, int split_images = 0, int part = 0, int nparts = 1) {
+                                           int scale_stride = 0, int split_images = 0, int part = 0, int nparts = 1,
+                                           const int* __restrict__ rows = nullptr, int nrows = 0) {
+  static_assert(!ROWS || (OMODE == 1 && !SPLIT && !GELU), "the row-list form stores from the D[n][m] registers, fp32");
   constexpr int NWV = (SPLIT && !GELU) ? POEM_GS_WAVES : 8;
   const int KC = K >> 3;
   const int tid = threadIdx.x, lane = tid & 63, wv = tid >> 6, r = lane & 31, h = lane >> 5;
@@ -491,14 +493,29 @@
 #ifdef POEM_PANEL_SKEW
   if (wv >= NWV / 2) { const long long t0_ = wall_clock64(); while (wall_clock64() - t0_ < POEM_PANEL_SKEW) __builtin_amdgcn_s_sleep(32); }
 #endif
+  [[maybe_unused]] int rnext[MT];
+  if constexpr (ROWS) {
+#pragma unroll
+    for (int i = 0; i < MT; ++i) rnext[i] = rows[min(((rg_lo + bip * NWV + wv) * MT + i) * 32 + r, M - 1)];
+  }
   for (int rg = rg_lo + bip * NWV + wv; rg < rg_hi; rg += blocks_in_panel * NWV) {
 #if POEM_PANEL_LAB & 4
     __builtin_amdgcn_s_setprio(0);
 #endif
     const int mt0 = rg * MT;
     unsigned xo[MT];
-#pragma unroll
-    for (int i = 0; i < MT; ++i) xo[i] = (unsigned)min((mt0 + i) * 32 + r, M - 1) * (unsigned)(ldx * 4) + 16u * h;
+    [[maybe_unused]] int rid[MT];
+#pragma unroll
+    for (int i = 0; i < MT; ++i) {
+      if constexpr (ROWS) {
+        const bool inb = (unsigned)rnext[i] < (unsigned)nrows;
+        rid[i] = ((mt0 + i) * 32 + r < M && inb) ? rnext[i] : -1;
+        xo[i] = (unsigned)(inb ? rnext[i] : 0) * (unsigned)(ldx * 4) + 16u * h;
+        rnext[i] = rows[min(((rg + blocks_in_panel * NWV) * MT + i) * 32 + r, M - 1)];
+      } else {
+        xo[i] = (unsigned)min((mt0 + i) * 32 + r, M - 1) * (unsigned)(ldx * 4) + 16u * h;
+      }
+    }
     f32x16 acc[MT][NT];
 #pragma unroll
     for (int i = 0; i < MT; ++i)
@@ -602,6 +619,19 @@
 #pragma unroll
       for (int i = 0; i < MT; ++i) {
         if ((mt0 + i) * 32 >= M) break;
+        if constexpr (ROWS) {
+          if (rid[i] < 0) continue;
+          float4* yr = reinterpret_cast<float4*>(Y + (size_t)rid[i] * ldy + ycol0 + 4 * h);
+#pragma unroll
+          for (int n = 0; n < NT; ++n)
+#pragma unroll
+            for (int g = 0; g < 4; ++g) {
+              const float4 bb = *reinterpret_cast<const float4*>(reinterpret_cast<const float*>(wl + NT * KC * 64) + n * 32 + 8 * g + 4 * h);
+              yr[n * 8 + 2 * g] = make_float4(acc[i][n][4 * g] + bb.x, acc[i][n][4 * g + 1] + bb.y, acc[i][n][4 * g + 2] + bb.z,
+                                              acc[i][n][4 * g + 3] + bb.w);
+            }
+          continue;
+        }
         float4* yp = reinterpret_cast<float4*>(Y) + ((size_t)(mt0 + i) * (ldy >> 3) + (ycol0 >> 3)) * 64 + lane;
         float4 vprev = make_float4(0.f, 0.f, 0.f, 0.f);
         (void)vprev;
@@ -868,6 +898,75 @@
   return launch_gemm_split_impl(X, ldx, Wp, bias, nullptr, 0, nullptr, 0, M, N, K, act, N, act, segs, s);
 }
 
+template <int NT>
+__global__ __launch_bounds__(512, 2) void gemm_panel_rows_kernel(const float* __restrict__ X, int ldx, const float4* __restrict__ Wp,
+                                                                 const float* __restrict__ bias, int N, int K, PanelSegs segs,
+                                                                 const int* __restrict__ rows, const int* __restrict__ count, int cap,
+                                                                 int nrows) {
+  const int KC = K >> 3;
+  extern __shared__ __attribute__((aligned(16))) float4 wl[];
+  const int tid = threadIdx.x;
+  const int panels = N / (32 * NT);
+  const int xm = segs.xcd_map;
+  const int lb = xm ? (int)(blockIdx.x >> 3) : (int)blockIdx.x;
+  const int panel = lb % panels, bip = lb / panels;
+  const int blocks_in_panel = xm ? (int)(gridDim.x >> 3) / panels : ((int)gridDim.x - panel + panels - 1) / panels;
+  const int part = xm ? (int)(blockIdx.x & 7) : 0, nparts = xm ? 8 : 1;
+  const int M = min(max(*count, 0), cap);
+  if (M == 0) return;
+  {
+    const float4* src = Wp + (size_t)panel * NT * KC * 64;
+    for (int i = tid; i < NT * KC * 64; i += 512) wl[i] = src[i];
+    float* lbias = reinterpret_cast<float*>(wl + NT * KC * 64);
+    if (tid < NT * 32) lbias[tid] = bias ? bias[panel * NT * 32 + tid] : 0.f;
+  }
+  __syncthreads();
+  const int col0 = panel * NT * 32;
+  const int sidx = col0 / segs.seg_cols, ycol0 = col0 - sidx * segs.seg_cols;
+  float* ys = segs.ptr[sidx];
+  const int waves = blocks_in_panel * 8 * nparts;
+  const int m2 = (M + 31) / 32 / (2 * waves) * (2 * waves) * 32;
+  if (m2 > 0)
+    panel_rows<NT, 2, false, 1, false, true>(X, ldx, wl, bias, nullptr, 0, ys, segs.seg_cols, m2, K, 0, col0, ycol0, bip, blocks_in_panel,
+                                             nullptr, 0, 0, part, nparts, rows, nrows);
+  if (M > m2)
+    panel_rows<NT, 1, false, 1, false, true>(X, ldx, wl, bias, nullptr, 0, ys, segs.seg_cols, M - m2, K, 0, col0, ycol0, bip, blocks_in_panel,
+                                             nullptr, 0, 0, part, nparts, rows + m2, nrows);
+}
+
+static int gemm_rows_nt(int K, int seg_cols, int nsegs) {
+  if (K <= 0 || K % 8 || seg_cols <= 0 || nsegs < 1 || nsegs > 6) return 0;
+  for (int c : {4, 2})
+    if (seg_cols % (32 * c) == 0 && (size_t)c * K * 128 <= 128 * 1024) return c;
+  return 0;
+}
+extern "C" int poem_gemm_rows_supported(int K, int seg_cols, int nsegs) { return gemm_rows_nt(K, seg_cols, nsegs) != 0; }
+
+extern "C" hipError_t poem_launch_gemm_rows(const float* X, int ldx, const void* Wp, const float* bias, int K, int seg_cols, int nsegs,
+                                            float* const* outs, const int* rows, const int* count, int cap, int nrows, hipStream_t s) {
+  const int NT = gemm_rows_nt(K, seg_cols, nsegs);
+  if (!NT || !X || !Wp || !outs || !rows || !count || cap < 1 || nrows < 1 || ((uintptr_t)X & 15) || ldx % 4 || ldx < K ||
+      (unsigned long long)nrows * ldx * 4ull >= (1ull << 32))
+    return hipErrorInvalidValue;
+  PanelSegs segs{};
+  segs.seg_cols = seg_cols;
+  for (int i = 0; i < nsegs; ++i) {
+    if (!outs[i] || ((uintptr_t)outs[i] & 15)) return hipErrorInvalidValue;
+    segs.ptr[i] = outs[i];
+  }
+  const int N = seg_cols * nsegs, panels = N / (32 * NT);
+  const int grid = std::max(poem_num_cus(), panels);
+  segs.xcd_map = g_panel_xcd_map && grid % 8 == 0 && (grid / 8) % panels == 0;
+  const size_t lds = (size_t)NT * (K / 8) * 64 * 16 + (size_t)NT * 32 * sizeof(float);
+  auto launch = [&](auto kern, std::atomic<unsigned long long>& optin) -> hipError_t {
+    if (hipError_t e = poem_optin_lds(reinterpret_cast<const void*>(kern), 128 * 1024 + 512, optin); e != hipSuccess) return e;
+    hipLaunchKernelGGL(kern, dim3(grid), dim3(512), lds, s, X, ldx, (const float4*)Wp, bias, N, K, segs, rows, count, cap, nrows);
+    return hipGetLastError();
+  };
+  static std::atomic<unsigned long long> optin4{0}, optin2{0};
+  return NT == 4 ? launch(gemm_panel_rows_kernel<4>, optin4) : launch(gemm_panel_rows_kernel<2>, optin2);
+}
+
 extern "C" hipError_t poem_launch_gemm(const float* X, int ldx, const void* Wp, const float* bias, const float* R,
                                        int ldr, float* Y, int ldy, int M, int N, int K, int act, hipStream_t s) {
   return poem_launch_gemm_split(X, ldx, Wp, bias, R, ldr, Y, ldy, M, N, K, act, N, act, s);
diff --git a/poem-v2_amd/csrc/handle.cpp b/poem-v2_amd/csrc/handle.cpp
--- a/poem-v2_amd/csrc/handle.cpp
+++ b/poem-v2_amd/csrc/handle.cpp
@@ -10,7 +10,7 @@
 namespace {
 struct CaptureKit {
   hipStream_t cap = nullptr, bps = nullptr, knn = nullptr;
-  hipEvent_t ev[5 + 32] = {};
+  hipEvent_t ev[5 + 40] = {};
 };
 std::mutex g_pool_mutex;
 std::map<int, std::vector<CaptureKit>> g_kit_pool;
@@ -44,7 +44,7 @@
 hipEvent_t** kit_event_slots(poem_handle_t h, hipEvent_t** out) {
   int n = 0;
   out[n++] = &h->ev_fork; out[n++] = &h->ev_join_bps; out[n++] = &h->ev_join_knn; out[n++] = &h->ev_tab; out[n++] = &h->ev_fork0;
-  for (int i = 0; i < 8; ++i) { out[n++] = &h->ev_bps[i]; out[n++] = &h->ev_xyz[i]; out[n++] = &h->ev_knn[i]; out[n++] = &h->ev_def[i]; }
+  for (int i = 0; i < 8; ++i) { out[n++] = &h->ev_bps[i]; out[n++] = &h->ev_xyz[i]; out[n++] = &h->ev_knn[i]; out[n++] = &h->ev_def[i]; out[n++] = &h->ev_vc[i]; }
   return out;
 }
 
@@ -52,7 +52,7 @@
   int dev = 0;
   if (hipGetDevice(&dev) != hipSuccess) return false;
   h->stream_device = dev;
-  hipEvent_t* slots[5 + 32];
+  hipEvent_t* slots[5 + 40];
   kit_event_slots(h, slots);
   {
     std::lock_guard<std::mutex> lock(g_pool_mutex);
@@ -61,36 +61,36 @@
       const CaptureKit k = pool.back();
       pool.pop_back();
       h->cap_stream = k.cap; h->bps_stream = k.bps; h->knn_stream = k.knn;
-      for (int i = 0; i < 5 + 32; ++i) *slots[i] = k.ev[i];
+      for (int i = 0; i < 5 + 40; ++i) *slots[i] = k.ev[i];
       return true;
     }
   }
   bool ok = hipStreamCreateWithFlags(&h->bps_stream, hipStreamNonBlocking) == hipSuccess &&
             hipStreamCreateWithFlags(&h->knn_stream, hipStreamNonBlocking) == hipSuccess &&
             hipStreamCreateWithFlags(&h->cap_stream, hipStreamNonBlocking) == hipSuccess;
-  for (int i = 0; i < 5 + 32; ++i) ok = ok && hipEventCreateWithFlags(slots[i], hipEventDisableTiming) == hipSuccess;
+  for (int i = 0; i < 5 + 40; ++i) ok = ok && hipEventCreateWithFlags(slots[i], hipEventDisableTiming) == hipSuccess;
   return ok;
 }
 
 void return_kit(poem_handle_t h) {
-  hipEvent_t* slots[5 + 32];
+  hipEvent_t* slots[5 + 40];
   kit_event_slots(h, slots);
   bool whole = h->cap_stream && h->bps_stream && h->knn_stream;
-  for (int i = 0; i < 5 + 32; ++i) whole = whole && *slots[i] != nullptr;
+  for (int i = 0; i < 5 + 40; ++i) whole = whole && *slots[i] != nullptr;
   if (!whole) {
     if (h->cap_stream) (void)hipStreamDestroy(h->cap_stream);
     if (h->bps_stream) (void)hipStreamDestroy(h->bps_stream);
     if (h->knn_stream) (void)hipStreamDestroy(h->knn_stream);
-    for (int i = 0; i < 5 + 32; ++i) if (*slots[i]) (void)hipEventDestroy(*slots[i]);
+    for (int i = 0; i < 5 + 40; ++i) if (*slots[i]) (void)hipEventDestroy(*slots[i]);
   } else {
     CaptureKit k;
     k.cap = h->cap_stream; k.bps = h->bps_stream; k.knn = h->knn_stream;
-    for (int i = 0; i < 5 + 32; ++i) k.ev[i] = *slots[i];
+    for (int i = 0; i < 5 + 40; ++i) k.ev[i] = *slots[i];
     std::lock_guard<std::mutex> lock(g_pool_mutex);
     g_kit_pool[h->stream_device].push_back(k);
   }
   h->cap_stream = h->bps_stream = h->knn_stream = nullptr;
-  for (int i = 0; i < 5 + 32; ++i) *slots[i] = nullptr;
+  for (int i = 0; i < 5 + 40; ++i) *slots[i] = nullptr;
 }
 
 void park_execs(poem_handle_t h) {
@@ -512,6 +512,7 @@
   else if (k == "group_xcd") h->group_xcd = value != 0;
   else if (k == "group_min_views") { if (value < -1) return POEM_E_ARG; h->group_min_views = value; }
   else if (k == "bps_defer") { if (value < 0 || value > 3) return POEM_E_ARG; h->bps_defer = value; }
+  else if (k == "vc_rows") h->vc_rows = value != 0;
   else if (k == "chain_tile") { if (value < 0 || value > 3) return POEM_E_ARG; h->chain_tile = value; }
   else return POEM_E_ARG;
   return POEM_OK;
diff --git a/poem-v2_amd/csrc/launchers.h b/poem-v2_amd/csrc/launchers.h
--- a/poem-v2_amd/csrc/launchers.h
+++ b/poem-v2_amd/csrc/launchers.h
@@ -87,6 +87,11 @@
                                                  int Q, int C, int ldq, int ldk, int ldv, hipStream_t s);
 hipError_t poem_launch_gather_anchor_rows(const float* src, int ld, const int* idx, int NS, float* dst, int B, int C,
                                           int* ident, hipStream_t s);
+hipError_t poem_launch_mark_rows(const int* idx, int B, int Q, int K, int ld, int S, int SP, int* list, int* count, int cap,
+                                 int* scratch, hipStream_t s);
+int poem_gemm_rows_supported(int K, int seg_cols, int nsegs);
+hipError_t poem_launch_gemm_rows(const float* X, int ldx, const void* Wp, const float* bias, int K, int seg_cols, int nsegs,
+                                 float* const* outs, const int* rows, const int* count, int cap, int nrows, hipStream_t s);
 hipError_t poem_launch_pad_rows(const float* src, float* dst, int B, int S, int SP, int W, hipStream_t s);
 hipError_t poem_launch_canon_xyz(const float* tmpl, float* out, int n, float radius, hipStream_t s);
 hipError_t poem_launch_pack_split(const float* w, int C, void* img, float* scale_out, hipStream_t s);
diff --git a/poem-v2_amd/csrc/misc.hip b/poem-v2_amd/csrc/misc.hip
--- a/poem-v2_amd/csrc/misc.hip
+++ b/poem-v2_amd/csrc/misc.hip
@@ -43,6 +43,71 @@
   const long total = (long)B * 32 * (C / 4);
   hipLaunchKernelGGL(gather_anchor_rows_kernel, dim3((unsigned)((total + 255) / 256)), dim3(256), 0, s, src, ld, idx, NS,
                      dst, B, C, ident);
+  return hipGetLastError();
+}
+
+__global__ __launch_bounds__(1024) void mark_rows_kernel(const int* __restrict__ idx, int Q, int K, int ld, int S, int SP,
+                                                         int* __restrict__ part, int* __restrict__ counts) {
+  extern __shared__ int mr_flag[];
+  int* wtot = mr_flag + S;
+  const int tid = threadIdx.x, lane = tid & 63, wv = tid >> 6, b = blockIdx.x;
+  for (int i = tid; i < S; i += 1024) mr_flag[i] = 0;
+  __syncthreads();
+  const int* src = idx + (size_t)b * Q * ld;
+  for (int t = tid; t < Q * K; t += 1024) {
+    const int q = t / K, v = src[(size_t)q * ld + (t - q * K)];
+    if ((unsigned)v < (unsigned)S) mr_flag[v] = 1;
+  }
+  __syncthreads();
+  const int per = (S + 1023) / 1024, r0 = tid * per;
+  int mine = 0;
+  for (int k = 0; k < per; ++k) mine += (r0 + k < S) ? mr_flag[r0 + k] : 0;
+  int incl = mine;
+#pragma unroll
+  for (int o = 1; o < 64; o <<= 1) {
+    const int up = __shfl_up(incl, o, 64);
+    if (lane >= o) incl += up;
+  }
+  if (lane == 63) wtot[wv] = incl;
+  __syncthreads();
+  if (tid == 0) {
+    int run = 0;
+    for (int w = 0; w < 16; ++w) { const int t = wtot[w]; wtot[w] = run; run += t; }
+    counts[b] = run;
+  }
+  __syncthreads();
+  int pos = wtot[wv] + incl - mine;
+  for (int k = 0; k < per; ++k)
+    if (r0 + k < S && mr_flag[r0 + k]) part[(size_t)b * SP + pos++] = b * SP + r0 + k;
+}
+
+__global__ __launch_bounds__(256) void compact_rows_kernel(const int* __restrict__ part, const int* __restrict__ counts, int B, int SP,
+                                                           int* __restrict__ list, int* __restrict__ count, int cap) {
+  __shared__ int red[256];
+  const int tid = threadIdx.x, b = blockIdx.x;
+  int sum = 0;
+  for (int j = tid; j < b; j += 256) sum += counts[j];
+  red[tid] = sum;
+  __syncthreads();
+  for (int o = 128; o > 0; o >>= 1) {
+    if (tid < o) red[tid] += red[tid + o];
+    __syncthreads();
+  }
+  const int base = red[0], n = counts[b];
+  for (int t = tid; t < n; t += 256)
+    if (base + t < cap) list[base + t] = part[(size_t)b * SP + t];
+  if (b == B - 1 && tid == 0) *count = base + n;
+}
+
+extern "C" hipError_t poem_launch_mark_rows(const int* idx, int B, int Q, int K, int ld, int S, int SP, int* list, int* count, int cap,
+                                            int* scratch, hipStream_t s) {
+  if (!idx || !list || !count || !scratch || B < 1 || Q < 1 || K < 1 || ld < K || S < 1 || SP < S || cap < 1 || (long)Q * K >= (1l << 31) ||
+      (long)B * SP >= (1l << 31) || S > 8192)
+    return hipErrorInvalidValue;
+  int* counts = scratch + (size_t)B * SP;
+  hipLaunchKernelGGL(mark_rows_kernel, dim3((unsigned)B), dim3(1024), (size_t)(S + 16) * sizeof(int), s, idx, Q, K, ld, S, SP, scratch, counts);
+  if (hipError_t e = hipGetLastError(); e != hipSuccess) return e;
+  hipLaunchKernelGGL(compact_rows_kernel, dim3((unsigned)B), dim3(256), 0, s, scratch, counts, B, SP, list, count, cap);
   return hipGetLastError();
 }
 
diff --git a/poem-v2_amd/csrc/ops.cpp b/poem-v2_amd/csrc/ops.cpp
--- a/poem-v2_amd/csrc/ops.cpp
+++ b/poem-v2_amd/csrc/ops.cpp
@@ -21,6 +21,26 @@
   if (act < 0 || act > 2 || (in_layout & ~1) || (out_layout & ~1)) return POEM_E_ARG;
   HIPCHK(poem_launch_gemm2(x, ldx, w_packed, bias, residual, ldr, y, ldy, M, N, K, act, in_layout, out_layout,
                            (hipStream_t)stream));
+  return POEM_OK;
+}
+
+int poem_mark_rows(const int32_t* idx, int batch, int nq, int k, int ld, int nsrc, int src_stride, int32_t* list, int32_t* count,
+                   int cap, int32_t* scratch, void* stream) {
+  if (!idx || !list || !count || !scratch || batch <= 0 || nq <= 0 || k <= 0 || ld < k || nsrc <= 0 || nsrc > 8192 || src_stride < nsrc || cap <= 0 ||
+      (int64_t)batch * src_stride >= (1ll << 31) || (int64_t)nq * k >= (1ll << 31))
+    return POEM_E_ARG;
+  HIPCHK(poem_launch_mark_rows(idx, batch, nq, k, ld, nsrc, src_stride, list, count, cap, scratch, (hipStream_t)stream));
+  return POEM_OK;
+}
+
+int poem_gemm_rows(const float* x, int ldx, const void* w_packed, const float* bias, float* y, int nrows, int N, int K,
+                   const int32_t* rows, const int32_t* count, int cap, void* stream) {
+  if (!x || !w_packed || !y || !rows || !count || nrows <= 0 || N <= 0 || K <= 0 || K % 8 || ldx % 4 || ldx < K || cap <= 0 ||
+      ((uintptr_t)x & 15) || ((uintptr_t)y & 15))
+    return POEM_E_ARG;
+  if (N % 2 || !poem_gemm_rows_supported(K, N / 2, 2) || (uint64_t)nrows * ldx * 4ull >= (1ull << 32)) return POEM_E_UNSUPPORTED;
+  float* outs[2] = {y, y + (size_t)nrows * (N / 2)};
+  HIPCHK(poem_launch_gemm_rows(x, ldx, w_packed, bias, K, N / 2, 2, outs, rows, count, cap, nrows, (hipStream_t)stream));
   return POEM_OK;
 }
 
diff --git a/poem-v2_amd/csrc/plan.cpp b/poem-v2_amd/csrc/plan.cpp
--- a/poem-v2_amd/csrc/plan.cpp
+++ b/poem-v2_amd/csrc/plan.cpp
@@ -80,6 +80,11 @@
     p.feat_pad = a.take<float>(BSP * C);
     p.xyz_pad = a.take<float>(BSP * 3);
   }
+  for (int i = 0; i < c.nblocks; ++i) {
+    p.vc_list[i] = i ? a.take<int32_t>(BSP) : nullptr;
+    p.vc_count[i] = i ? a.take<int32_t>(1) : nullptr;
+  }
+  p.vc_scratch = a.take<int32_t>(BSP + (size_t)B);
   p.bytes = align_up(a.off, 256);
   return p;
 }
diff --git a/poem-v2_amd/hip.py b/poem-v2_amd/hip.py
--- a/poem-v2_amd/hip.py
+++ b/poem-v2_amd/hip.py
@@ -76,6 +76,8 @@
                                          _i, _i, _i, _vp]),
     "poem_gemm": (_i, [_vp, _i, _vp, _vp, _vp, _i, _vp, _i, _i, _i, _i, _i, _vp]),
     "poem_gemm_ex": (_i, [_vp, _i, _vp, _vp, _vp, _i, _vp, _i, _i, _i, _i, _i, _i, _i, _vp]),
+    "poem_mark_rows": (_i, [_vp, _i, _i, _i, _i, _i, _i, _vp, _vp, _i, _vp, _vp]),
+    "poem_gemm_rows": (_i, [_vp, _i, _vp, _vp, _vp, _i, _i, _i, _vp, _vp, _i, _vp]),
     "poem_pack_rows": (_i, [_vp, _i, _i, _vp, _vp]),
     "poem_unpack_rows": (_i, [_vp, _i, _i, _vp, _vp]),
     "poem_layernorm": (_i, [_vp, _vp, _vp, _vp, _i, _i, _f, _vp]),
@@ -426,6 +428,25 @@
     return y
 
 
+def mark_rows(idx, nsrc, src_stride=None, k=None):
+    B, NQ, ld = idx.shape
+    src_stride = nsrc if src_stride is None else src_stride
+    lst = torch.full((B * src_stride,), -1, dtype=torch.int32, device=idx.device)
+    cnt = torch.empty(1, dtype=torch.int32, device=idx.device)
+    scratch = torch.empty(B * src_stride + B, dtype=torch.int32, device=idx.device)
+    check(lib().poem_mark_rows(ptr(idx, torch.int32), B, NQ, ld if k is None else k, ld, nsrc, src_stride, lst.data_ptr(),
+                               cnt.data_ptr(), lst.numel(), scratch.data_ptr(), stream()), "poem_mark_rows")
+    return lst, cnt
+
+
+def gemm_rows(x, w_packed, n_out, rows, count, y, bias=None):
+    M, K = x.shape
+    assert tuple(y.shape) == (2, M, n_out // 2) and y.is_contiguous()
+    check(lib().poem_gemm_rows(ptr(x), K, w_packed.data_ptr(), ptr(bias), ptr(y), M, n_out, K, ptr(rows, torch.int32),
+                               ptr(count, torch.int32), rows.numel(), stream()), "poem_gemm_rows")
+    return y
+
+
 def pack_rows(x):
     return pack_linear(x)
 
```

Result: no change. 1488 (median of 6 runs) (+1.0%).
